# OpenPPL/ppq

Measured on AMD Instinct MI355X. Metric: calibration samples/sec (RuntimeCalibrationPass, KL 2048-bin, ResNet-50 INT8), higher is better.
Workload: dtype f32; 1 GPU; ResNet-50 topology (53 Conv + 1 Gemm, BN folded, seeded He init), RuntimeCalibrationPass kl 2048 bins, per-tensor INT8 activations, per-channel INT8 weights, 279 batches x 32 x 3x224x224 per GPU; samples=8928, batch=32, observed_tensors=72, rccl_ranks=1, async_observe=False, cache_params=False, channels_last=False, fuse_params=True, batch_observations=True, reuse_activations=False, replayed_batches=0, hip_graph=auto, graph_replays=0, miopen_find=False

## Files before the change

### include/ppq_hip.h

```cpp
#ifndef PPQ_HIP_H_
#define PPQ_HIP_H_

#include <stdint.h>

#ifdef __cplusplus
extern "C" {
#endif

typedef enum {
    PPQHIP_OK = 0,
    PPQHIP_ERR_INVALID_VALUE = -1,
    PPQHIP_ERR_UNSUPPORTED = -2,
    PPQHIP_ERR_HIP = -3
} ppqhip_status;

#define PPQHIP_ABI_VERSION 4

const char* ppqhip_last_error(void);
int ppqhip_version(void);
int ppqhip_device_arch(char* buf, int n);

int ppqhip_fq_linear_t(const float* x, const float* scale, const float* offset, float* out,
                       int64_t n, int clip_min, int clip_max, int rounding, void* stream);

int ppqhip_fq_linear_c(const float* x, const float* scale, const float* offset, float* out,
                       int64_t n, int64_t num_channel, int64_t elem_per_channel,
                       int clip_min, int clip_max, int rounding, void* stream);

int ppqhip_to_int_t(const float* x, const float* scale, const float* offset, void* out, int64_t n,
                    int clip_min, int clip_max, int rounding, int out_dtype, void* stream);
int ppqhip_to_int_c(const float* x, const float* scale, const float* offset, void* out, int64_t n,
                    int64_t num_channel, int64_t elem_per_channel, int clip_min, int clip_max,
                    int rounding, int out_dtype, void* stream);

typedef struct ppqhip_fq_job {
    const float* x;
    const float* scale;
    const float* offset;
    float* out;
    int64_t n, num_channel, elem_per_channel;
    int32_t clip_min, clip_max;
} ppqhip_fq_job;
int64_t ppqhip_fq_linear_multi_table_bytes(int num_jobs);
int ppqhip_fq_linear_multi(const ppqhip_fq_job* jobs, int num_jobs, int rounding, void* device_table,
                           int upload, void* stream);

int ppqhip_fq_linear_t_bwd(const float* x, const float* scale, const float* offset,
                           const float* grad_y, float* grad_x, float* grad_s, int64_t n,
                           int clip_min, int clip_max, int rounding, void* stream);

int ppqhip_fq_linear_c_bwd(const float* x, const float* scale, const float* offset,
                           const float* grad_y, float* grad_x, float* grad_s, int64_t n,
                           int64_t num_channel, int64_t elem_per_channel,
                           int clip_min, int clip_max, int rounding, void* stream);

int64_t ppqhip_fq_linear_t_bwd_partials(int64_t n);
int ppqhip_fq_linear_t_bwd_main(const float* x, const float* scale, const float* offset, const float* grad_y, float* grad_x,
                                float* partial, int64_t n, int clip_min, int clip_max, int rounding, void* stream);
typedef struct ppqhip_lsq_finish_job {
    const float* partial;
    float* grad_s;
    int64_t n;
    int32_t clip_min, clip_max;
} ppqhip_lsq_finish_job;
int ppqhip_lsq_finish_multi(const ppqhip_lsq_finish_job* jobs, int num_jobs, void* stream);

typedef struct ppqhip_lsq_job {
    const float* x;
    const float* scale;
    const float* offset;
    const float* grad_y;
    float* grad_x;
    float* grad_s;
    int64_t n, num_channel, elem_per_channel;
    int32_t clip_min, clip_max;
} ppqhip_lsq_job;
int ppqhip_fq_linear_c_bwd_multi(const ppqhip_lsq_job* jobs, int num_jobs, int rounding, void* stream);

int ppqhip_fq_float_t(const float* x, const float* scale, const float* offset, float* out,
                      int64_t n, int exponent, int mantissa, float clip_min, float clip_max,
                      int rounding, void* stream);

int ppqhip_fq_float_c(const float* x, const float* scale, const float* offset, float* out,
                      int64_t n, int64_t num_channel, int64_t elem_per_channel,
                      int exponent, int mantissa, float clip_min, float clip_max,
                      int rounding, void* stream);

typedef struct ppqhip_float_search_job {
    const float* x;
    int64_t rows, row_len;
    int32_t exponent, mantissa;
    float clip_min, clip_max;
} ppqhip_float_search_job;
int64_t ppqhip_float_scale_search_table_bytes(int num_jobs);
int ppqhip_float_scale_search(const ppqhip_float_search_job* jobs, int num_jobs, const float* candidates,
                              int num_candidates, int rounding, void* device_table, double* out, void* stream);

typedef struct ppqhip_fq_float_job {
    const float* x;
    const float* scale;
    const float* offset;
    float* out;
    int64_t n, num_channel, elem_per_channel;
    int32_t exponent, mantissa;
    float clip_min, clip_max;
} ppqhip_fq_float_job;
int64_t ppqhip_fq_float_multi_table_bytes(int num_jobs);
int ppqhip_fq_float_multi(const ppqhip_fq_float_job* jobs, int num_jobs, int rounding, void* device_table,
                          int upload, void* stream);

int ppqhip_fq_float_c_bwd(const float* x, const float* scale, const float* offset,
                          const float* grad_y, float* grad_x, float* grad_s, int64_t n,
                          int64_t num_channel, int64_t elem_per_channel,
                          int exponent, int mantissa, float clip_min, float clip_max,
                          int rounding, void* stream);

int64_t ppqhip_hist_workspace_bytes(int64_t n, int64_t num_bins);
int ppqhip_hist_sym_t(const float* x, int64_t n, float hist_scale, int clip_outliers,
                      int32_t* hist, int64_t num_bins, void* workspace, void* stream);

int ppqhip_hist_asym_t(const float* x, int64_t n, float min_value, float max_value,
                       int clip_outliers, int32_t* hist, int64_t num_bins, void* workspace,
                       void* stream);

int ppqhip_hist_sym_c(const float* x, int64_t n, int64_t num_channel, int64_t elem_per_channel,
                      float hist_scale, int clip_outliers, int32_t* hist, int64_t num_bins,
                      void* stream);

int ppqhip_hist_sym_c_scales(const float* x, int64_t n, int64_t num_channel, int64_t elem_per_channel,
                             const float* hist_scales, int clip_outliers, int32_t* hist,
                             int64_t num_bins, void* stream);
int ppqhip_hist_asym_c_ranges(const float* x, int64_t n, int64_t num_channel, int64_t elem_per_channel,
                              const float* mins, const float* maxs, int clip_outliers, int32_t* hist,
                              int64_t num_bins, void* stream);

int64_t ppqhip_quantile_workspace_bytes(int64_t n);
int ppqhip_quantile_t(const float* x, int64_t n, float q, float* dest, uint32_t* hint, void* workspace,
                      void* stream);

typedef struct ppqhip_quantile_job {
    const float* x;
    float* dest;
    uint32_t* hint;
    int64_t n;
} ppqhip_quantile_job;
int64_t ppqhip_quantile_multi_workspace_bytes(int num_jobs, int64_t total_elems);
int ppqhip_quantile_t_multi(const ppqhip_quantile_job* jobs, int num_jobs, float q, void* workspace,
                            void* stream);
void ppqhip_quantile_debug_layout(int64_t* out);
void ppqhip_quantile_hot_layout(int64_t* out);

int ppqhip_isotone_t(const float* x, int64_t n, float* dest, void* workspace, void* stream);

int64_t ppqhip_minmax_workspace_bytes(int64_t n);
int ppqhip_minmax_t(const float* x, int64_t n, float* minmax, void* workspace, void* stream);

int ppqhip_minmax_c(const float* x, int64_t n, int64_t num_channel, int64_t elem_per_channel,
                    float* mins, float* maxs, void* stream);

typedef struct ppqhip_minmax_c_job {
    const float* x;
    float* mins;
    float* maxs;
    int64_t n, num_channel, elem_per_channel;
    int32_t fresh, reserved;
} ppqhip_minmax_c_job;
int ppqhip_minmax_c_multi(const ppqhip_minmax_c_job* jobs, int num_jobs, void* stream);

int ppqhip_channel_sum(const float* x, int64_t n, int64_t num_channel, int64_t elem_per_channel,
                       double* sums, void* stream);

int64_t ppqhip_hist_rows(void);
int ppqhip_hist_sym_t_rows(const float* x, int64_t n, float hist_scale, int clip_outliers,
                           int32_t* rows, int64_t num_bins, void* stream);
int ppqhip_hist_asym_t_rows(const float* x, int64_t n, float min_value, float max_value,
                            int clip_outliers, int32_t* rows, int64_t num_bins, void* stream);
typedef struct ppqhip_minmax_job {
    const float* x;
    float* slots;
    int64_t n;
} ppqhip_minmax_job;
int ppqhip_minmax_t_slots_multi(const ppqhip_minmax_job* jobs, int num_jobs, void* stream);

typedef struct ppqhip_hist_job {
    const float* x;
    int32_t* rows;
    int64_t n;
    float p0, p1;
} ppqhip_hist_job;
int ppqhip_hist_t_rows_multi(const ppqhip_hist_job* jobs, int num_jobs, int asymmetric,
                             int clip_outliers, int64_t num_bins, void* stream);
int ppqhip_hist_rows_finish(const int32_t* rows, int64_t num_bins, int32_t* hist, void* stream);
int ppqhip_check_bin_rule(const float* x, int64_t n, float min_value, float hist_scale, int asymmetric, uint64_t* out, void* stream);
int64_t ppqhip_minmax_slots(void);
int ppqhip_minmax_t_slots(const float* x, int64_t n, float* slots, void* stream);
int ppqhip_minmax_slots_finish(const float* slots, float* minmax, void* stream);

float ppqhip_mse_loss_host(const int64_t* hist, int64_t num_bins, int start, int step, int end);

int64_t ppqhip_mse_search_workspace_bytes(int64_t num_hist);
int ppqhip_mse_search(const int32_t* hist, int64_t num_hist, int64_t num_bins,
                      const double* hist_scale, const double* min_value,
                      int quant_min, int quant_max, int symmetrical, int32_t* best,
                      void* workspace, void* stream);

int64_t ppqhip_kl_num_candidates(int64_t num_bins, int num_of_bits);
int ppqhip_kl_losses(const int32_t* hist, int64_t num_hist, int64_t num_bins, int num_of_bits,
                     double* losses, void* stream);

int ppqhip_tensor_clip_t(const float* value, const float* reference, const float* limit,
                         float* out, int64_t n, void* stream);
int ppqhip_tensor_clip_c(const float* value, const float* reference, const float* limit,
                         float* out, int64_t n, int64_t num_channel, int64_t elem_per_channel,
                         void* stream);
int ppqhip_rounding_loss(const float* x, const float* scale, const float* offset, float* out,
                         int64_t n, int64_t num_channel, int64_t elem_per_channel,
                         int clip_min, int clip_max, int rounding, void* stream);
int ppqhip_rounding_loss_bwd(const float* x, const float* dy, const float* scale,
                             const float* offset, float* dx, int64_t n, int64_t num_channel,
                             int64_t elem_per_channel, int clip_min, int clip_max, int rounding,
                             void* stream);

int ppqhip_bias_act(float* y, const float* bias, int64_t n, int64_t num_channel, int64_t elem_per_channel,
                    int relu, void* stream);
int ppqhip_bias_add_act(float* a, const float* bias_a, float* b, const float* bias_b, float* out,
                        int64_t n, int64_t num_channel, int64_t elem_per_channel, int relu, void* stream);

typedef struct ppqhip_adaround_job {
    const float* w;
    const float* v;
    const float* scale;
    const float* offset;
    float* out;
    const float* dy;
    int64_t n, num_channel, elem_per_channel;
    int32_t qmin, qmax;
} ppqhip_adaround_job;
int ppqhip_adaround_fwd_multi(const ppqhip_adaround_job* jobs, int num_jobs, void* stream);
int ppqhip_adaround_bwd_multi(const ppqhip_adaround_job* jobs, int num_jobs, const float* reg, void* stream);

typedef struct ppqhip_roundtune_job {
    const float* w;
    const float* r;
    const float* scale;
    const float* offset;
    float* out;
    int64_t n, num_channel, elem_per_channel;
    int32_t qmin, qmax;
} ppqhip_roundtune_job;
int ppqhip_roundtune_fwd_multi(const ppqhip_roundtune_job* jobs, int num_jobs, void* stream);

typedef struct ppqhip_fetch_rows_job {
    const float* x;
    const int32_t* index;
    float* out;
    int64_t rows, row_len, count;
} ppqhip_fetch_rows_job;
int ppqhip_fetch_rows_multi(const ppqhip_fetch_rows_job* jobs, int num_jobs, void* stream);
typedef struct ppqhip_measure_rows_job {
    const float* p;
    const float* r;
    const int32_t* index;
    double* sums;
    int64_t rows, row_len, count;
} ppqhip_measure_rows_job;
int ppqhip_measure_rows_multi(const ppqhip_measure_rows_job* jobs, int num_jobs, void* stream);
enum { PPQHIP_MEASURE_SNR = 0, PPQHIP_MEASURE_MSE = 1, PPQHIP_MEASURE_COSINE = 2 };
enum { PPQHIP_REDUCE_MEAN = 0, PPQHIP_REDUCE_MAX = 1 };
typedef struct ppqhip_measure_finish_job {
    const double* sums;
    double* acc;
    float* row_out;
    int64_t rows, count;
    int32_t method, reduce;
} ppqhip_measure_finish_job;
int ppqhip_measure_finish_multi(const ppqhip_measure_finish_job* jobs, int num_jobs, void* stream);

typedef struct ppqhip_equalize_segment {
    const float* base;
    int64_t extent;
    int64_t div, a, b;
    int64_t outer, stride, run;
    float multiplier;
    int32_t downstream;
} ppqhip_equalize_segment;
typedef struct ppqhip_equalize_scale_job {
    const ppqhip_equalize_segment* segments;
    float* scale;
    int32_t num_segments, num_channel;
    float value_threshold;
    int32_t reserved;
} ppqhip_equalize_scale_job;
int ppqhip_equalize_scale_multi(const ppqhip_equalize_scale_job* jobs, int num_jobs, void* stream);
typedef struct ppqhip_equalize_apply_job {
    float* x;
    const float* scale;
    int64_t n, run, inner, group_out;
    int64_t num_scale;
    int32_t divide, reserved;
} ppqhip_equalize_apply_job;
int ppqhip_equalize_apply_multi(const ppqhip_equalize_apply_job* jobs, int num_jobs, void* stream);

typedef struct ppqhip_split_plan_job {
    const ppqhip_equalize_segment* segments;
    int32_t* src_of;
    int32_t* count;
    int32_t num_segments, num_channel;
    float value_threshold;
    int32_t reserved;
} ppqhip_split_plan_job;
int ppqhip_split_plan_multi(const ppqhip_split_plan_job* jobs, int num_jobs, void* stream);
typedef struct ppqhip_split_apply_job {
    const float* x;
    float* out;
    const int32_t* src_of;
    int64_t n, run;
    int32_t num_channel, count;
} ppqhip_split_apply_job;
int ppqhip_split_apply_multi(const ppqhip_split_apply_job* jobs, int num_jobs, void* stream);

typedef struct ppqhip_ssd_scales_job {
    ppqhip_equalize_segment first, last;
    const float* act_range;
    float* scales;
    float* ranges;
    int32_t num_channel;
    float channel_ratio;
} ppqhip_ssd_scales_job;
int ppqhip_ssd_scales_multi(const ppqhip_ssd_scales_job* jobs, int num_jobs, void* stream);
typedef struct ppqhip_ssd_apply_job {
    const float* x;
    float* out;
    const float* scales;
    int64_t n, run, inner, group_out;
    int64_t num_channel;
    int32_t divide, reserved;
} ppqhip_ssd_apply_job;
int ppqhip_ssd_apply_multi(const ppqhip_ssd_apply_job* jobs, int num_jobs, void* stream);
typedef struct ppqhip_fq_measure_rows_job {
    const float* y;
    const float* r;
    const float* scale;
    const float* offset;
    double* sums;
    int64_t rows, count;
    int64_t num_channel, elem_per_channel;
    int32_t clip_min, clip_max, rounding, reserved;
} ppqhip_fq_measure_rows_job;
int ppqhip_fq_measure_rows_multi(const ppqhip_fq_measure_rows_job* jobs, int num_jobs, void* stream);

typedef struct ppqhip_stat_job {
    const float* p;
    const float* r;
    float* rec;
    int64_t n;
    int32_t bins, reserved;
} ppqhip_stat_job;
int ppqhip_stat_moments_multi(const ppqhip_stat_job* jobs, int num_jobs, void* stream);
int ppqhip_stat_shape_multi(const ppqhip_stat_job* jobs, int num_jobs, void* stream);

#define PPQHIP_PROF_MAX_KERNELS 40
typedef struct {
    char name[48];
    int64_t launches;
    double total_ms;
    double total_bytes;
} ppqhip_prof_entry;
int ppqhip_prof_enable(int on);
int ppqhip_prof_collect(ppqhip_prof_entry* entries, int max_entries);
double ppqhip_prof_event_overhead_us(void* stream, int pairs);

#ifdef __cplusplus
}
#endif
#endif
```

### ppq_amd/_lib.py

```python
import ctypes
import os

_HERE = os.path.dirname(os.path.abspath(__file__))
LIB_PATH = os.path.join(_HERE, 'libppq_hip.so')

c_f32p = ctypes.c_void_p
c_i32p = ctypes.c_void_p
c_f64p = ctypes.c_void_p
c_i64 = ctypes.c_int64
c_int = ctypes.c_int
c_flt = ctypes.c_float
c_vp = ctypes.c_void_p

ABI_VERSION = 4


class ProfEntry(ctypes.Structure):
    _fields_ = [('name', ctypes.c_char * 48), ('launches', ctypes.c_int64),
                ('total_ms', ctypes.c_double), ('total_bytes', ctypes.c_double)]


PROTOTYPES = {
    'ppqhip_last_error': (ctypes.c_char_p, []),
    'ppqhip_version': (c_int, []),
    'ppqhip_device_arch': (c_int, [ctypes.c_char_p, c_int]),
    'ppqhip_fq_linear_t': (c_int, [c_f32p, c_f32p, c_f32p, c_f32p, c_i64, c_int, c_int, c_int, c_vp]),
    'ppqhip_fq_linear_c': (c_int, [c_f32p, c_f32p, c_f32p, c_f32p, c_i64, c_i64, c_i64, c_int, c_int, c_int, c_vp]),
    'ppqhip_to_int_t': (c_int, [c_f32p, c_f32p, c_f32p, c_vp, c_i64, c_int, c_int, c_int, c_int, c_vp]),
    'ppqhip_to_int_c': (c_int, [c_f32p, c_f32p, c_f32p, c_vp, c_i64, c_i64, c_i64, c_int, c_int, c_int, c_int, c_vp]),
    'ppqhip_fq_linear_t_bwd': (c_int, [c_f32p, c_f32p, c_f32p, c_f32p, c_f32p, c_f32p, c_i64, c_int, c_int, c_int,
                                       c_vp]),
    'ppqhip_fq_linear_c_bwd': (c_int, [c_f32p, c_f32p, c_f32p, c_f32p, c_f32p, c_f32p, c_i64, c_i64, c_i64, c_int,
                                       c_int, c_int, c_vp]),
    'ppqhip_fq_linear_c_bwd_multi': (c_int, [c_vp, c_int, c_int, c_vp]),
    'ppqhip_fq_linear_t_bwd_partials': (c_i64, [c_i64]),
    'ppqhip_fq_linear_t_bwd_main': (c_int, [c_f32p, c_f32p, c_f32p, c_f32p, c_f32p, c_f32p, c_i64, c_int, c_int, c_int, c_vp]),
    'ppqhip_lsq_finish_multi': (c_int, [c_vp, c_int, c_vp]),
    'ppqhip_bias_act': (c_int, [c_f32p, c_f32p, c_i64, c_i64, c_i64, c_int, c_vp]),
    'ppqhip_bias_add_act': (c_int, [c_f32p, c_f32p, c_f32p, c_f32p, c_f32p, c_i64, c_i64, c_i64, c_int, c_vp]),
    'ppqhip_fq_float_t': (c_int, [c_f32p, c_f32p, c_f32p, c_f32p, c_i64, c_int, c_int, c_flt, c_flt, c_int, c_vp]),
    'ppqhip_fq_float_c': (c_int, [c_f32p, c_f32p, c_f32p, c_f32p, c_i64, c_i64, c_i64, c_int, c_int, c_flt, c_flt,
                                  c_int, c_vp]),
    'ppqhip_fq_float_c_bwd': (c_int, [c_f32p, c_f32p, c_f32p, c_f32p, c_f32p, c_f32p, c_i64, c_i64, c_i64, c_int,
                                      c_int, c_flt, c_flt, c_int, c_vp]),
    'ppqhip_hist_workspace_bytes': (c_i64, [c_i64, c_i64]),
    'ppqhip_hist_sym_t': (c_int, [c_f32p, c_i64, c_flt, c_int, c_i32p, c_i64, c_vp, c_vp]),
    'ppqhip_hist_asym_t': (c_int, [c_f32p, c_i64, c_flt, c_flt, c_int, c_i32p, c_i64, c_vp, c_vp]),
    'ppqhip_hist_sym_c': (c_int, [c_f32p, c_i64, c_i64, c_i64, c_flt, c_int, c_i32p, c_i64, c_vp]),
    'ppqhip_hist_sym_c_scales': (c_int, [c_f32p, c_i64, c_i64, c_i64, c_f32p, c_int, c_i32p, c_i64, c_vp]),
    'ppqhip_hist_asym_c_ranges': (c_int, [c_f32p, c_i64, c_i64, c_i64, c_f32p, c_f32p, c_int, c_i32p, c_i64, c_vp]),
    'ppqhip_quantile_workspace_bytes': (c_i64, [c_i64]),
    'ppqhip_quantile_t': (c_int, [c_f32p, c_i64, c_flt, c_f32p, c_vp, c_vp, c_vp]),
    'ppqhip_isotone_t': (c_int, [c_f32p, c_i64, c_f32p, c_vp, c_vp]),
    'ppqhip_minmax_workspace_bytes': (c_i64, [c_i64]),
    'ppqhip_minmax_t': (c_int, [c_f32p, c_i64, c_f32p, c_vp, c_vp]),
    'ppqhip_minmax_c': (c_int, [c_f32p, c_i64, c_i64, c_i64, c_f32p, c_f32p, c_vp]),
    'ppqhip_minmax_c_multi': (c_int, [c_vp, c_int, c_vp]),
    'ppqhip_fq_linear_multi_table_bytes': (c_i64, [c_int]),
    'ppqhip_fq_linear_multi': (c_int, [c_vp, c_int, c_int, c_vp, c_int, c_vp]),
    'ppqhip_float_scale_search_table_bytes': (c_i64, [c_int]),
    'ppqhip_float_scale_search': (c_int, [c_vp, c_int, c_vp, c_int, c_int, c_vp, c_vp, c_vp]),
    'ppqhip_fq_float_multi_table_bytes': (c_i64, [c_int]),
    'ppqhip_fq_float_multi': (c_int, [c_vp, c_int, c_int, c_vp, c_int, c_vp]),
    'ppqhip_quantile_multi_workspace_bytes': (c_i64, [c_int, c_i64]),
    'ppqhip_quantile_t_multi': (c_int, [c_vp, c_int, c_flt, c_vp, c_vp]),
    'ppqhip_quantile_debug_layout': (None, [c_vp]),
    'ppqhip_quantile_hot_layout': (None, [c_vp]),
    'ppqhip_minmax_t_slots_multi': (c_int, [c_vp, c_int, c_vp]),
    'ppqhip_hist_t_rows_multi': (c_int, [c_vp, c_int, c_int, c_int, c_i64, c_vp]),
    'ppqhip_channel_sum': (c_int, [c_f32p, c_i64, c_i64, c_i64, c_f64p, c_vp]),
    'ppqhip_hist_rows': (c_i64, []),
    'ppqhip_hist_sym_t_rows': (c_int, [c_f32p, c_i64, c_flt, c_int, c_i32p, c_i64, c_vp]),
    'ppqhip_hist_asym_t_rows': (c_int, [c_f32p, c_i64, c_flt, c_flt, c_int, c_i32p, c_i64, c_vp]),
    'ppqhip_hist_rows_finish': (c_int, [c_i32p, c_i64, c_i32p, c_vp]),
    'ppqhip_check_bin_rule': (c_int, [c_f32p, c_i64, c_flt, c_flt, c_int, c_vp, c_vp]),
    'ppqhip_minmax_slots': (c_i64, []),
    'ppqhip_minmax_t_slots': (c_int, [c_f32p, c_i64, c_f32p, c_vp]),
    'ppqhip_minmax_slots_finish': (c_int, [c_f32p, c_f32p, c_vp]),
    'ppqhip_mse_loss_host': (c_flt, [ctypes.POINTER(ctypes.c_int64), c_i64, c_int, c_int, c_int]),
    'ppqhip_mse_search_workspace_bytes': (c_i64, [c_i64]),
    'ppqhip_mse_search': (c_int, [c_i32p, c_i64, c_i64, c_f64p, c_f64p, c_int, c_int, c_int, c_i32p, c_vp, c_vp]),
    'ppqhip_kl_num_candidates': (c_i64, [c_i64, c_int]),
    'ppqhip_kl_losses': (c_int, [c_i32p, c_i64, c_i64, c_int, c_f64p, c_vp]),
    'ppqhip_tensor_clip_t': (c_int, [c_f32p, c_f32p, c_f32p, c_f32p, c_i64, c_vp]),
    'ppqhip_tensor_clip_c': (c_int, [c_f32p, c_f32p, c_f32p, c_f32p, c_i64, c_i64, c_i64, c_vp]),
    'ppqhip_rounding_loss': (c_int, [c_f32p, c_f32p, c_f32p, c_f32p, c_i64, c_i64, c_i64, c_int, c_int, c_int, c_vp]),
    'ppqhip_rounding_loss_bwd': (c_int, [c_f32p, c_f32p, c_f32p, c_f32p, c_f32p, c_i64, c_i64, c_i64, c_int, c_int,
                                         c_int, c_vp]),
    'ppqhip_adaround_fwd_multi': (c_int, [c_vp, c_int, c_vp]),
    'ppqhip_adaround_bwd_multi': (c_int, [c_vp, c_int, c_f32p, c_vp]),
    'ppqhip_roundtune_fwd_multi': (c_int, [c_vp, c_int, c_vp]),
    'ppqhip_equalize_scale_multi': (c_int, [c_vp, c_int, c_vp]),
    'ppqhip_equalize_apply_multi': (c_int, [c_vp, c_int, c_vp]),
    'ppqhip_split_plan_multi': (c_int, [c_vp, c_int, c_vp]),
    'ppqhip_split_apply_multi': (c_int, [c_vp, c_int, c_vp]),
    'ppqhip_ssd_scales_multi': (c_int, [c_vp, c_int, c_vp]),
    'ppqhip_ssd_apply_multi': (c_int, [c_vp, c_int, c_vp]),
    'ppqhip_fq_measure_rows_multi': (c_int, [c_vp, c_int, c_vp]),
    'ppqhip_fetch_rows_multi': (c_int, [c_vp, c_int, c_vp]),
    'ppqhip_measure_rows_multi': (c_int, [c_vp, c_int, c_vp]),
    'ppqhip_measure_finish_multi': (c_int, [c_vp, c_int, c_vp]),
    'ppqhip_stat_moments_multi': (c_int, [c_vp, c_int, c_vp]),
    'ppqhip_stat_shape_multi': (c_int, [c_vp, c_int, c_vp]),
    'ppqhip_prof_enable': (c_int, [c_int]),
    'ppqhip_prof_collect': (c_int, [ctypes.POINTER(ProfEntry), c_int]),
    'ppqhip_prof_event_overhead_us': (ctypes.c_double, [c_vp, c_int]),
}

if not os.path.exists(LIB_PATH):
    raise ImportError(
        f'{LIB_PATH} is missing: the HIP kernel library has not been built.  Run '
        '`python -c "import __graft_entry__ as g; g.build()"` or `make -C ppq_amd/csrc` (needs hipcc, '
        'targets gfx950).  ppq_amd has no CPU / PyTorch fallback by design.')

import torch

_torch_hip = os.path.join(os.path.dirname(torch.__file__), 'lib', 'libamdhip64.so')
if os.path.exists(_torch_hip):
    ctypes.CDLL(_torch_hip, mode=ctypes.RTLD_GLOBAL)

try:
    lib = ctypes.CDLL(LIB_PATH)
except OSError as e:
    raise ImportError(f'cannot load {LIB_PATH}: {e}') from e

for _name, (_res, _args) in PROTOTYPES.items():
    _fn = getattr(lib, _name)
    _fn.restype = _res
    _fn.argtypes = _args


if lib.ppqhip_version() != ABI_VERSION:
    raise ImportError(f'{LIB_PATH} has ABI version {lib.ppqhip_version()}, this package needs {ABI_VERSION}: rebuild it '
                      '(`make -C ppq_amd/csrc` or `python -c "import __graft_entry__ as g; g.build()"`)')


def last_error() -> str:
    msg = lib.ppqhip_last_error()
    return msg.decode('utf-8', 'replace') if msg else ''
```

### ppq_amd/calibration.py

```python
import time
from math import ceil
from typing import Callable, Dict, Iterable, List

from .core import QuantizationStates, state_value
from .distributed import merge_observers
from .observer import OperationObserver, TorchHistObserver, render_observers


class QuantizationOptimizationPass:
    def __init__(self, name: str = 'Default Quanzation Optim') -> None:
        self.name = name

    def apply(self, graph, **kwargs) -> None:
        self.optimize(graph, **kwargs)

    def optimize(self, graph, **kwargs) -> None:
        raise NotImplementedError('Implement this function first.')

    def __str__(self) -> str:
        return 'QuantizationOptimizationPass[' + self.name + ']'


class RuntimeCalibrationPass(QuantizationOptimizationPass):
    AUTO_GRAPH_ISSUE_FRACTION = 0.7
    AUTO_GRAPH_MIN_STEPS = 12

    def __init__(self, method: str = None, override: bool = False, calib_steps: int = 32,
                 process_group=None, check_steps: bool = True, async_observe: bool = False,
                 use_hip_graph: bool = False, batch_observations: bool = True,
                 reuse_activations: bool = False, reuse_budget_bytes: int = 64 << 30,
                 queue_bytes: int = None) -> None:
        super().__init__(name='PPQ Runtime Calibration Pass')
        self._method = method
        self._observers: Dict[str, OperationObserver] = {}
        self._collate_fn = None
        self._calib_steps = calib_steps
        self._override = override
        self._process_group = process_group
        self._check_steps = check_steps
        self._async_observe = async_observe
        self._use_hip_graph = use_hip_graph
        self._batch_observations = batch_observations
        self._queue = None
        self._reuse_activations = reuse_activations
        self._queue_bytes = queue_bytes
        self._reuse_budget = reuse_budget_bytes
        self._replay: list = []
        self._replay_bytes = 0
        self.replay_peak_bytes = 0
        self.replayed_batches = 0
        self._recording = False
        self.graph_replays = 0
        self.graph_decisions = []
        self.merge_stats = []
        self._side_stream = None

    def _batches(self, dataloader: Iterable) -> list:
        out = []
        for calib_epoch in range(ceil(self._calib_steps / len(dataloader))):
            for data in dataloader:
                if self._collate_fn is not None:
                    data = self._collate_fn(data)
                out.append(data)
                if len(out) >= self._calib_steps: return out
        return out

    def _graph_replayable(self, batches: list, hooks: Dict[str, object]) -> bool:
        import torch
        from .observer import ConstantObserver, TorchHistObserver, TorchMinMaxObserver, TorchMSEObserver
        if not self._use_hip_graph or len(batches) < 4: return False
        if not all(isinstance(b, torch.Tensor) and b.is_cuda and b.shape == batches[0].shape
                   and b.dtype == batches[0].dtype for b in batches): return False
        safe = (TorchMinMaxObserver, TorchHistObserver, TorchMSEObserver, ConstantObserver)
        return all(type(ob) in safe for hook in hooks.values() for ob in hook._observer_table.values())

    @ staticmethod
    def _forward_fn(executor):
        return executor.forward

    def _forward(self, executor, data, hooks, output_names):
        import torch
        recording = self._queue is not None and self._recording
        if recording: self._queue.recorder = []
        with torch.no_grad():
            self._forward_fn(executor)(inputs=data, hooks=hooks, output_names=output_names)
        if self._queue is not None: self._queue.flush()
        if recording:
            rec, self._queue.recorder = self._queue.recorder, None
            size = sum(v.numel() * 4 for _, v in rec)
            if self._replay_bytes + size <= self._reuse_budget:
                self._replay.append(rec); self._replay_bytes += size
                self.replay_peak_bytes = max(self.replay_peak_bytes, self._replay_bytes)
            else: self._recording = False

    def _replay_phase2(self, batches: list) -> int:
        n = min(len(self._replay), len(batches))
        for i in range(n):
            for ob, value in self._replay[i]: ob.observe(value)
            self._queue.flush()
            self._replay[i] = None
        self._replay, self._replay_bytes = [], 0
        self.replayed_batches += n
        return n

    def calibrate(self, desc: str, dataloader: Iterable, executor, hooks: Dict[str, object],
                  output_names: List[str] = None):
        import torch
        batches = self._batches(dataloader)
        if self._replay and not self._recording:
            batches = batches[self._replay_phase2(batches):]
            if not batches: return
        if not self._graph_replayable(batches, hooks):
            for data in batches:
                self._forward(executor, data, hooks, output_names)
            return
        self._forward(executor, batches[0], hooks, output_names)
        first = 1
        if self._use_hip_graph == 'auto':
            torch.cuda.synchronize()
            t0 = time.perf_counter()
            self._forward(executor, batches[1], hooks, output_names)
            t1 = time.perf_counter()
            torch.cuda.synchronize()
            t2 = time.perf_counter()
            first = 2
            launch_bound = (t1 - t0) > self.AUTO_GRAPH_ISSUE_FRACTION * (t2 - t0)
            self.graph_decisions.append({'phase': desc, 'issue_ms': (t1 - t0) * 1e3, 'total_ms': (t2 - t0) * 1e3,
                                         'graph': bool(launch_bound and len(batches) - first >= self.AUTO_GRAPH_MIN_STEPS)})
            if not self.graph_decisions[-1]['graph']:
                for data in batches[first:]:
                    self._forward(executor, data, hooks, output_names)
                return
        self._recording = False
        static_in = torch.empty_like(batches[0])
        torch.cuda.synchronize()
        graph = torch.cuda.CUDAGraph()
        with torch.cuda.graph(graph):
            self._forward(executor, static_in, hooks, output_names)
            if self._side_stream is not None:
                torch.cuda.current_stream().wait_stream(self._side_stream)
        for data in batches[first:]:
            static_in.copy_(data, non_blocking=True)
            graph.replay()
            self.graph_replays += 1

    def _all_tensor_observers(self):
        return [ob for op_ob in self._observers.values() for ob in op_ob.observers()]

    def _render(self):
        observers = self._all_tensor_observers()
        if self._queue is not None: self._queue.flush()
        if self._side_stream is not None:
            import torch
            torch.cuda.current_stream().wait_stream(self._side_stream)
        if merge_observers(observers, group=self._process_group):
            from . import distributed
            self.merge_stats.append(dict(distributed.last_merge_stats))
        render_observers(observers)

    def optimize(self, graph, dataloader: Iterable, executor, calib_steps: int = 32,
                 collate_fn: Callable = None, **kwargs) -> None:
        if collate_fn is not None: self._collate_fn = collate_fn
        if calib_steps is not None: self._calib_steps = calib_steps
        if self._check_steps:
            assert self._calib_steps >= 8, (
                'Insufficient Calibration Detected, to get a better quantization performance, '
                'more calibration steps is required, we strongly recommend you to prepare more calibration data '
                'and more calibration steps is preferred here. (at least 8)')
            assert self._calib_steps <= 512, (
                'Calibration steps is too large, ppq can quantize your network within 8-512 '
                'calibration steps. More calibration steps will greatly delay ppq\'s calibration procedure. '
                'Reset your calib_steps parameter please.')

        if self._override:
            for operation in graph.operations.values():
                if not hasattr(operation, 'config'): continue
                for config, var in operation.config_with_variable:
                    if (not var.is_parameter and state_value(config.state) == QuantizationStates.ACTIVATED.value
                            and config.dominated_by == config):
                        config.state = type(config.state).INITIAL

        self._observers = {}
        hooks = {}
        import torch
        if self._async_observe and torch.cuda.is_available():
            self._side_stream = torch.cuda.Stream()
        for op_name, operation in graph.operations.items():
            if not hasattr(operation, 'config'): continue
            for config, var in operation.config_with_variable:
                if not var.is_parameter and self._method is not None:
                    config.observer_algorithm = self._method
            observer = OperationObserver(operation=executor._graph.operations[op_name], monitor_parameter=False)
            observer.hook.stream = self._side_stream
            self._observers[op_name] = observer
            hooks[op_name] = observer.hook

        self._queue = None
        if self._batch_observations and self._side_stream is None:
            from .observer import ObservationQueue
            self._queue = ObservationQueue() if self._queue_bytes is None else ObservationQueue(self._queue_bytes)
        for ob in self._all_tensor_observers(): ob.queue = self._queue

        self._replay, self._replay_bytes = [], 0
        self._recording = bool(self._reuse_activations and self._queue is not None)
        self.calibrate(desc='Calibration Progress(Phase 1)', dataloader=dataloader, executor=executor,
                       hooks=hooks, output_names=None)
        self._recording = False
        self._render()
        if self._replay:
            for observer in self._observers.values():
                for cfg, ob in observer.hook._observer_table.items():
                    if (not getattr(ob._watch_on, 'is_parameter', False)
                            and QuantizationStates.is_activated(cfg.state)):
                        self._replay, self._replay_bytes = [], 0
                        break
                if not self._replay: break

        pop_list = []
        for op_name, observer in self._observers.items():
            if all([not isinstance(var_observer, TorchHistObserver)
                    for var_observer in observer.observers()]):
                pop_list.append(op_name)
        for op_name in pop_list:
            self._observers.pop(op_name)
            hooks.pop(op_name)

        if len(hooks) > 0:
            self.calibrate(desc='Calibration Progress(Phase 2)', dataloader=dataloader, executor=executor,
                           hooks=hooks, output_names=None)
            self._render()


class PPLDSPTIReCalibrationPass(RuntimeCalibrationPass):
    def __init__(self, method: str = None, override: bool = False) -> None:
        super().__init__(method, override)
        self.name = 'PPQ ReCalibration For Computing Op Pass'

    def optimize(self, graph, dataloader: Iterable, executor, calib_steps: int, collate_fn: Callable = None, **kwargs) -> None:
        from .blocks import COMPUTING_OP, downstream_operations
        from .core import QuantizationPolicy, QuantizationProperty as P, TensorQuantizationConfig
        from .observer import CalibrationHook, TensorObserverFactroy, TorchMinMaxObserver
        self._collate_fn, self._calib_steps = collate_fn, calib_steps
        assert calib_steps >= 8, ('Insufficient Calibration Detected, to better quantize your network, more calibration steps is '
                                  'demonded, we strongly recommend you to prepare more calibration data and more calibration '
                                  'steps is preferred here. (at least 8)')
        assert calib_steps <= 512, ('Calibration steps is too large, ppq is capable for quantizing your network within 32-128 '
                                    'calibration steps. More calibraiton steps will greatly delay ppq\'s calibration procedure. '
                                    'Reset your calib_steps parameter please.')

        def probe(like, per_channel: bool, consumer):
            bits = P.SYMMETRICAL.value + P.LINEAR.value + (P.PER_CHANNEL.value if per_channel else P.PER_TENSOR.value)
            return TensorQuantizationConfig(policy=QuantizationPolicy(bits), rounding=like.rounding, num_of_bits=like.num_of_bits,
                                            quant_min=like.quant_min, quant_max=like.quant_max, scale=None, offset=None,
                                            observer_algorithm='Minmax', state=QuantizationStates.INITIAL,
                                            channel_axis=1 if per_channel else None, detail={'consumer': consumer})
        hooks = {}
        for operation in graph.topological_sort():
            if not hasattr(operation, 'config') or operation.type not in COMPUTING_OP: continue
            output_cfg = operation.config.output_quantization_config[0]
            master_cfg, master_operation, master_var = output_cfg, operation, operation.outputs[0]
            table = {}
            if operation.inputs[0].name in graph.inputs:
                input_cfg = operation.config.input_quantization_config[0]
                table[input_cfg] = TensorObserverFactroy.build_observer(operation.inputs[0], probe(input_cfg, False, input_cfg))
            followers = downstream_operations(operation)
            if len(followers) == 1 and followers[0].type in {'Relu', 'Clip'} and hasattr(followers[0], 'config'):
                if table:
                    hooks[operation.name] = CalibrationHook(operation, table)
                    table = {}
                master_operation = followers[0]
                master_cfg = master_operation.config.output_quantization_config[0]
                master_var = master_operation.outputs[0]
            table[master_cfg] = TensorObserverFactroy.build_observer(master_var, probe(master_cfg, True, output_cfg))
            assert master_operation.name not in hooks, 'register an operation in calibration hooks twice'
            hooks[master_operation.name] = CalibrationHook(master_operation, table)

        self._queue = None
        self.calibrate(desc='ReCalibration For Computing Ops', dataloader=dataloader, executor=executor, hooks=hooks)

        for hook in hooks.values():
            for observer in hook._observer_table.values():
                cfg = observer._quant_cfg.detail['consumer']
                assert isinstance(observer, TorchMinMaxObserver)
                r = observer._range_on_host()
                if observer._quant_cfg.policy.has_property(P.PER_CHANNEL):
                    cfg.detail.update({'range_min': r[0].copy(), 'range_max': r[1].copy()})
                else:
                    cfg.detail.update({'range_min': (float(r[0]),), 'range_max': (float(r[1]),)})


class IsotoneCalibrationPass(RuntimeCalibrationPass):
    def __init__(self, variables: List[str] = None, axis: int = -1, verbose: bool = True, calib_steps: int = 32) -> None:
        super().__init__(calib_steps=calib_steps)
        self.name = 'Isotone Calibration Pass'
        self.variables = variables
        self.axis = axis
        self.verbose = verbose

    @ staticmethod
    def _mark(cfg, axis: int) -> None:
        from .core import OBSERVER_ISOTONE_OBSERVER_AXIS
        cfg.state = type(cfg.state).INITIAL
        cfg.observer_algorithm = 'Isotone'
        cfg.detail[OBSERVER_ISOTONE_OBSERVER_AXIS] = axis

    def optimize(self, graph, **kwargs) -> None:
        if self.variables is None:
            for op in graph.operations.values():
                if op.type != 'Softmax' or not hasattr(op, 'config'): continue
                cfg = op.config.output_quantization_config[0]
                if cfg.dominated_by != cfg: continue
                axis = op.attributes.get('axis', -1)
                self._mark(cfg, axis)
                if self.verbose: print(f'Calibration Method of Op {op.name} has been changed to Isotone[axis={axis}].')
        else:
            if not isinstance(self.variables, list):
                raise TypeError('Isotone Calibration Pass needs a list of variable name as its input.')
            for name in self.variables:
                if not isinstance(name, str):
                    raise TypeError('Isotone Calibration Pass needs a list of variable name as its input.')
                if name not in graph.variables: raise ValueError(f'Variable {name} not in current graph.')
                var = graph.variables[name]
                op = var.source_op
                if op is None or not hasattr(op, 'config'): continue
                self._mark(op.config.output_quantization_config[op.outputs.index(var)], self.axis)
                if self.verbose: print(f'Calibration Method of Variable {var.name} has been changed to Isotone[axis={self.axis}].')
        super().optimize(graph, **kwargs)
```

### ppq_amd/csrc/epilogue.hip

```cpp
#include "common.hpp"

namespace ppqhip {
namespace {

constexpr int kEpTileU = 2;
constexpr int kEpSmallU = 1;
constexpr long long kEpSmallElems = 1ll << 20;

struct EpArgs {
    float* a;
    const float* bias_a;
    float* b;
    const float* bias_b;
    float* out;
    uint32_t nvec;
    uint32_t tail;
    int ntail;
    FastDiv epc;
    FastDiv nc;
};

__device__ __forceinline__ uint32_t channel_of(uint32_t i, const FastDiv& epc, const FastDiv& nc) {
    const uint32_t row = fdiv(i, epc);
    return row - fdiv(row, nc) * nc.d;
}

__device__ __forceinline__ float act(float v, bool relu) {
    return (relu && !__builtin_isnan(v)) ? __builtin_fmaxf(v, 0.f) : v;
}

__device__ __forceinline__ float4 add4(const float4& x, const float4& y) {
    return make_float4(x.x + y.x, x.y + y.y, x.z + y.z, x.w + y.w);
}

template <bool RELU>
__device__ __forceinline__ float4 act4(const float4& v) {
    return make_float4(act(v.x, RELU), act(v.y, RELU), act(v.z, RELU), act(v.w, RELU));
}

template <bool PLANE>
__device__ __forceinline__ float4 bias4(const float* __restrict__ bias, uint32_t v, const FastDiv& epc, const FastDiv& nc) {
    if (PLANE) {
        const float t = bias[channel_of(v, epc, nc)];
        return make_float4(t, t, t, t);
    }
    const uint32_t i = v * 4u;
    return make_float4(bias[channel_of(i, epc, nc)], bias[channel_of(i + 1, epc, nc)], bias[channel_of(i + 2, epc, nc)],
                       bias[channel_of(i + 3, epc, nc)]);
}

template <bool RESID, bool BIAS_B, bool RELU>
__device__ __forceinline__ void epilogue_elem(const EpArgs& p, uint32_t i, const FastDiv& epc) {
    const uint32_t c = channel_of(i, epc, p.nc);
    const float x = p.a[i] + p.bias_a[c];
    if (!RESID) { p.a[i] = act(x, RELU); return; }
    p.a[i] = x;
    float y = p.b[i];
    if (BIAS_B) { y = y + p.bias_b[c]; p.b[i] = y; }
    p.out[i] = act(x + y, RELU);
}

template <int U, bool RESID, bool BIAS_B, bool RELU, bool PLANE>
__global__ __launch_bounds__(kBlock) void epilogue_kernel(EpArgs p) {
    const uint32_t base = blockIdx.x * (kBlock * U) + threadIdx.x;
    float4* a4 = reinterpret_cast<float4*>(p.a);
    float4* b4 = reinterpret_cast<float4*>(p.b);
    float4* o4 = reinterpret_cast<float4*>(p.out);
    float4 a[U], ba[U], b[U], bb[U];
#pragma unroll
    for (int k = 0; k < U; k++) {
        const uint32_t vv = min(base + k * kBlock, p.nvec - 1);
        a[k] = a4[vv];
        ba[k] = bias4<PLANE>(p.bias_a, vv, p.epc, p.nc);
        if (RESID) b[k] = b4[vv];
        if (BIAS_B) bb[k] = bias4<PLANE>(p.bias_b, vv, p.epc, p.nc);
    }
#pragma unroll
    for (int k = 0; k < U; k++) {
        const uint32_t vv = base + k * kBlock;
        if (vv >= p.nvec) continue;
        const float4 x = add4(a[k], ba[k]);
        if (!RESID) { a4[vv] = act4<RELU>(x); continue; }
        a4[vv] = x;
        float4 y = b[k];
        if (BIAS_B) { y = add4(y, bb[k]); b4[vv] = y; }
        o4[vv] = act4<RELU>(add4(x, y));
    }
    if (!PLANE && blockIdx.x == 0 && (int)threadIdx.x < p.ntail)
        epilogue_elem<RESID, BIAS_B, RELU>(p, p.tail + threadIdx.x, p.epc);
}

template <bool RESID, bool BIAS_B, bool RELU>
__global__ __launch_bounds__(kBlock) void epilogue_scalar_kernel(EpArgs p) {
    const uint32_t stride = gridDim.x * kBlock;
    for (uint32_t i = blockIdx.x * kBlock + threadIdx.x; i < (uint32_t)p.ntail; i += stride)
        epilogue_elem<RESID, BIAS_B, RELU>(p, i, p.epc);
}

template <bool RESID, bool BIAS_B, bool RELU>
void launch_epilogue(EpArgs p, int64_t n, int64_t C, int64_t epc, bool aligned, hipStream_t st) {
    p.nc = make_fastdiv((uint32_t)C);
    if (!aligned || n < 4) {
        p.nvec = 0; p.tail = 0; p.ntail = (int)n;
        p.epc = make_fastdiv((uint32_t)epc);
        hipLaunchKernelGGL((epilogue_scalar_kernel<RESID, BIAS_B, RELU>), dim3(stream_grid(n, kBlock)), dim3(kBlock), 0, st, p);
        return;
    }
    p.nvec = (uint32_t)(n >> 2);
    p.tail = p.nvec * 4u;
    p.ntail = (int)(n & 3);
    const bool plane = (epc % 4 == 0);
    p.epc = make_fastdiv((uint32_t)(plane ? epc / 4 : epc));
#define PPQ_LAUNCH_EP(U, PLANE)                                                                                          \
    hipLaunchKernelGGL((epilogue_kernel<U, RESID, BIAS_B, RELU, PLANE>), dim3((p.nvec + kBlock * U - 1) / (kBlock * U)),   \
                       dim3(kBlock), 0, st, p)
    if (n <= kEpSmallElems) {
        if (plane) PPQ_LAUNCH_EP(kEpSmallU, true); else PPQ_LAUNCH_EP(kEpSmallU, false);
    } else {
        if (plane) PPQ_LAUNCH_EP(kEpTileU, true); else PPQ_LAUNCH_EP(kEpTileU, false);
    }
#undef PPQ_LAUNCH_EP
}

int validate(int64_t n, int64_t C, int64_t epc, const char* what) {
    if (n <= 0 || n > 0x7fffffffLL) {
        set_error("%s: n=%lld is empty or has more than 2^31 - 1 elements", what, (long long)n);
        return PPQHIP_ERR_INVALID_VALUE;
    }
    if (C <= 0 || epc <= 0 || C > 0x7fffffffLL || epc > 0x7fffffffLL || n % (C * epc) != 0) {
        set_error("%s: n=%lld is not [outer, %lld channels, %lld elem/channel]", what, (long long)n, (long long)C,
                  (long long)epc);
        return PPQHIP_ERR_INVALID_VALUE;
    }
    return PPQHIP_OK;
}

}
}

using namespace ppqhip;

extern "C" {

int ppqhip_bias_act(float* y, const float* bias, int64_t n, int64_t num_channel, int64_t elem_per_channel, int relu,
                    void* stream) {
    if (int st = validate(n, num_channel, elem_per_channel, "bias_act")) return st;
    if (!y || !bias) { set_error("bias_act: null pointer"); return PPQHIP_ERR_INVALID_VALUE; }
    hipStream_t s = (hipStream_t)stream;
    EpArgs p{};
    p.a = y; p.bias_a = bias;
    const bool aligned = aligned16(y);
    if (relu) launch_epilogue<false, false, true>(p, n, num_channel, elem_per_channel, aligned, s);
    else launch_epilogue<false, false, false>(p, n, num_channel, elem_per_channel, aligned, s);
    return finish_launch("bias_act");
}

int ppqhip_bias_add_act(float* a, const float* bias_a, float* b, const float* bias_b, float* out, int64_t n,
                        int64_t num_channel, int64_t elem_per_channel, int relu, void* stream) {
    if (int st = validate(n, num_channel, elem_per_channel, "bias_add_act")) return st;
    if (!a || !bias_a || !b || !out) { set_error("bias_add_act: null pointer"); return PPQHIP_ERR_INVALID_VALUE; }
    hipStream_t s = (hipStream_t)stream;
    EpArgs p{};
    p.a = a; p.bias_a = bias_a; p.b = b; p.bias_b = bias_b; p.out = out;
    const bool aligned = aligned16(a) && aligned16(b) && aligned16(out);
    if (bias_b) {
        if (relu) launch_epilogue<true, true, true>(p, n, num_channel, elem_per_channel, aligned, s);
        else launch_epilogue<true, true, false>(p, n, num_channel, elem_per_channel, aligned, s);
    } else {
        if (relu) launch_epilogue<true, false, true>(p, n, num_channel, elem_per_channel, aligned, s);
        else launch_epilogue<true, false, false>(p, n, num_channel, elem_per_channel, aligned, s);
    }
    return finish_launch("bias_add_act");
}

}
```

### ppq_amd/csrc/hist.hip

```cpp
#include "common.hpp"

namespace ppqhip {

constexpr int kMaxLdsBins = 16384;
constexpr int kLdsBudgetInts = 2048;
constexpr int kHistBlock = 512;
constexpr int kHistWgPerCu = 2;
constexpr int kHistU = 2;
constexpr int kHistMinTiles = 2;
constexpr int kHistAtomicMaxWg = 128;
constexpr long long kHistNtElems = 48ll << 20;
constexpr int kHistRows = kNumCU * kHistWgPerCu;
constexpr uint32_t kTileVec = (uint32_t)kHistBlock * kHistU;
constexpr uint32_t kTileElems = kTileVec * 4;
static_assert(kHistBlock % 64 == 0 && kHistBlock >= 64 && kHistBlock <= 1024, "histogram workgroup: whole waves");

typedef float v2f __attribute__((ext_vector_type(2)));

struct BinRule {
    float a;
    float hs;
    float rcp;
    int bins;
    int clip;
    int asym;
};
static BinRule make_rule(float a, float hs, int bins, int clip, int asym) {
    BinRule r; r.a = a; r.hs = hs; r.rcp = 1.0f / hs; r.bins = bins; r.clip = clip; r.asym = asym;
    return r;
}

__device__ __forceinline__ bool quotient_is_safe(float t) {
    return __builtin_fabsf(t - __builtin_rintf(t)) >= __builtin_fabsf(t) * 0x1p-22f;
}

__device__ __forceinline__ int f2i_abs(float t) {
    int r;
    asm("v_cvt_i32_f32_e64 %0, |%1|" : "=v"(r) : "v"(t));
    return r;
}
__device__ __forceinline__ int f2i_floor(float t) {
    int r;
    asm("v_cvt_flr_i32_f32 %0, %1" : "=v"(r) : "v"(t));
    return r;
}

template <bool ASYM, bool CLIP, bool HOT>
struct Binner : WaveBinCounter<ASYM, CLIP, HOT> {
    using Base = WaveBinCounter<ASYM, CLIP, HOT>;
    using Base::h; using Base::last; using Base::hot_bin; using Base::hot_cnt;
    float a0, hs, rcp;

    __device__ __forceinline__ void set_rule(float a, float scale) { a0 = a; hs = scale; rcp = 1.0f / scale; }

    __device__ __forceinline__ void bins4(const float4& v, int (&b)[4]) const {
        v2f x01 = {v.x, v.y}, x23 = {v.z, v.w};
        if (ASYM) { x01 = x01 - a0; x23 = x23 - a0; }
        const v2f t01 = x01 * rcp, t23 = x23 * rcp;
        const v2f r01 = {__builtin_rintf(t01.x), __builtin_rintf(t01.y)};
        const v2f r23 = {__builtin_rintf(t23.x), __builtin_rintf(t23.y)};
        const v2f d01 = t01 - r01, d23 = t23 - r23;
        const v2f e01 = t01 * 0x1p-22f, e23 = t23 * 0x1p-22f;
        const bool u0 = !(__builtin_fabsf(d01.x) >= __builtin_fabsf(e01.x));
        const bool u1 = !(__builtin_fabsf(d01.y) >= __builtin_fabsf(e01.y));
        const bool u2 = !(__builtin_fabsf(d23.x) >= __builtin_fabsf(e23.x));
        const bool u3 = !(__builtin_fabsf(d23.y) >= __builtin_fabsf(e23.y));
        b[0] = ASYM ? f2i_floor(t01.x) : f2i_abs(t01.x);
        b[1] = ASYM ? f2i_floor(t01.y) : f2i_abs(t01.y);
        b[2] = ASYM ? f2i_floor(t23.x) : f2i_abs(t23.x);
        b[3] = ASYM ? f2i_floor(t23.y) : f2i_abs(t23.y);
        if (u0 | u1 | u2 | u3) {
            if (u0) b[0] = exact_bin(ASYM ? x01.x : __builtin_fabsf(v.x));
            if (u1) b[1] = exact_bin(ASYM ? x01.y : __builtin_fabsf(v.y));
            if (u2) b[2] = exact_bin(ASYM ? x23.x : __builtin_fabsf(v.z));
            if (u3) b[3] = exact_bin(ASYM ? x23.y : __builtin_fabsf(v.w));
        }
    }
    __device__ __forceinline__ int exact_bin(float a) const { return f2i_sat(__builtin_floorf(a / hs)); }

    __device__ __forceinline__ int bin1(float v) const {
        const float a = ASYM ? (v - a0) : __builtin_fabsf(v);
        const float t = a * rcp;
        if (quotient_is_safe(t)) return ASYM ? f2i_floor(t) : f2i_abs(t);
        return exact_bin(a);
    }

};

constexpr int kReduceBins = 32, kReduceSlices = 32, kReduceBlock = kReduceBins * kReduceSlices;
__global__ __launch_bounds__(kReduceBlock) void hist_reduce_kernel(const int* __restrict__ partial, int count, int bins,
                                                                   int* __restrict__ hist) {
    __shared__ int lds[kReduceSlices][kReduceBins];
    const int lane_bin = threadIdx.x % kReduceBins, slice = threadIdx.x / kReduceBins;
    const int b = blockIdx.x * kReduceBins + lane_bin;
    int total = 0;
    if (b < bins) {
        int i = slice;
        for (; i + 15 * kReduceSlices < count; i += 16 * kReduceSlices) {
            int v[16];
#pragma unroll
            for (int k = 0; k < 16; k++) v[k] = partial[(size_t)(i + k * kReduceSlices) * bins + b];
#pragma unroll
            for (int k = 0; k < 16; k++) total += v[k];
        }
        for (; i < count; i += kReduceSlices) total += partial[(size_t)i * bins + b];
    }
    lds[slice][lane_bin] = total;
    __syncthreads();
    if (slice == 0 && b < bins) {
        int t = 0;
#pragma unroll
        for (int k = 0; k < kReduceSlices; k++) t += lds[k][lane_bin];
        if (t) hist[b] += t;
    }
}

constexpr int kMultiMax = 96;
enum FlushMode : int {
    FLUSH_ROWS_ADD = 0,
    FLUSH_ROWS_STORE = 1,
    FLUSH_ATOMIC = 2
};
struct HistJob {
    const float* x;
    int* rows;
    uint32_t n;
    float a, hs;
    uint32_t first_tile;
};
struct HistJobs {
    HistJob job[kMultiMax];
    uint32_t count;
    uint32_t total_tiles;
    int bins, copies, mode;
};
__host__ __device__ inline uint32_t job_tiles(uint32_t n, bool vec_ok) {
    if (!vec_ok) return (n + kTileElems - 1) / kTileElems;
    const uint32_t full = (n >> 2) / kTileVec;
    return full + (n > full * kTileElems ? 1u : 0u);
}

__device__ __forceinline__ void lds_hist_flush(int* lds, int bins, int copies, int* __restrict__ dst, int mode) {
    asm volatile("s_waitcnt lgkmcnt(0)" ::: "memory");
    __syncthreads();
    for (int b = threadIdx.x; b < bins; b += kHistBlock) {
        int s = 0;
        for (int c = 0; c < copies; c++) { s += lds[c * bins + b]; lds[c * bins + b] = 0; }
        if (mode == FLUSH_ROWS_STORE) dst[b] = s;
        else if (s) {
            if (mode == FLUSH_ROWS_ADD) dst[b] += s;
            else atomicAdd(&dst[b], s);
        }
    }
    __syncthreads();
}

template <bool ASYM, bool CLIP, bool HOT, bool NT>
__global__ __launch_bounds__(kHistBlock, (kHistBlock * kHistWgPerCu + 255) / 256)
void hist_persistent_kernel(const HistJobs jobs) {
    extern __shared__ int lds[];
    const uint32_t G = gridDim.x, g = blockIdx.x;
    uint32_t t, t_end;
    even_split(jobs.total_tiles, G, g, t, t_end);
    const int bins = jobs.bins, copies = jobs.copies;
    bool zeroed = false;
    auto zero_lds = [&]() {
        if (zeroed) return;
        for (int i = threadIdx.x; i < copies * bins; i += kHistBlock) lds[i] = 0;
        asm volatile("s_waitcnt lgkmcnt(0)\n\ts_barrier" ::: "memory");
        zeroed = true;
    };
    if (t >= t_end) {
        if (jobs.mode == FLUSH_ROWS_STORE) for (int b = threadIdx.x; b < bins; b += kHistBlock) jobs.job[0].rows[(size_t)g * bins + b] = 0;
        return;
    }
    uint32_t lo = 0, hi = jobs.count;
    while (hi - lo > 1) {
        const uint32_t mid = (lo + hi) >> 1;
        if (jobs.job[mid].first_tile <= t) lo = mid; else hi = mid;
    }
    Binner<ASYM, CLIP, HOT> acc;
    acc.init(lds + ((threadIdx.x >> 6) % copies) * bins, bins);

    for (uint32_t j = lo; t < t_end; j++) {
        const HistJob& job = jobs.job[j];
        const uint32_t j_end = (j + 1 < jobs.count) ? jobs.job[j + 1].first_tile : jobs.total_tiles;
        uint32_t k = t - job.first_tile;
        const uint32_t k1 = min(t_end, j_end) - job.first_tile;
        t = min(t_end, j_end);
        acc.set_rule(job.a, job.hs);
        const float* __restrict__ x = job.x;
        const uint32_t n = job.n;
        const bool vec_ok = (reinterpret_cast<uintptr_t>(x) & 15u) == 0;
        const uint32_t full = vec_ok ? (n >> 2) / kTileVec : 0u;
        const uint32_t kf = min(k1, full);
        if (k < kf) {
            const float4* xv = reinterpret_cast<const float4*>(x) + threadIdx.x;
            float4 bufa[kHistU], bufb[kHistU];
            auto fetch = [&](float4 (&buf)[kHistU], uint32_t tile) {
                const float4* p = xv + (size_t)tile * kTileVec;
#pragma unroll
                for (int u = 0; u < kHistU; u++) buf[u] = load4<NT>(p + u * kHistBlock);
            };
            auto consume = [&](const float4 (&buf)[kHistU], uint32_t tile) {
#pragma unroll
                for (int u = 0; u < kHistU; u++) {
                    int b[4];
                    acc.bins4(buf[u], b);
                    if (u == 0) acc.elect(b[0], true);
                    if (CLIP && HOT) acc.commit4_exec(b);
                    else {
                        acc.template commit<true>(b[0], true); acc.template commit<true>(b[1], true);
                        acc.template commit<true>(b[2], true); acc.template commit<true>(b[3], true);
                    }
                }
            };
            fetch(bufa, k);
            zero_lds();
            for (;;) {
                fetch(bufb, min(k + 1, kf - 1));
                consume(bufa, k);
                if (++k >= kf) break;
                fetch(bufa, min(k + 1, kf - 1));
                consume(bufb, k);
                if (++k >= kf) break;
            }
        }
        zero_lds();
        for (; k < k1; k++) {
            const uint32_t e0 = k * kTileElems + threadIdx.x;
#pragma unroll 4
            for (int r = 0; r < 4 * kHistU; r++) {
                const uint32_t i = e0 + r * kHistBlock;
                const bool in = i < n;
                const float a = in ? x[i] : 0.f;
                const int b = acc.bin1(a);
                if ((r & 3) == 0) acc.elect(b, in);
                acc.template commit<false>(b, in);
            }
        }
        acc.flush_hot();
        acc.hot_bin = -1;
        int* dst = jobs.mode == FLUSH_ATOMIC ? job.rows : job.rows + (size_t)g * bins;
        lds_hist_flush(lds, bins, copies, dst, jobs.mode);
    }
}

template <bool ASYM, bool CLIP, int kSmallK, bool PING = false, bool NT = false>
__global__ __launch_bounds__(kHistBlock) void hist_small_kernel(const float* __restrict__ x, uint32_t n, float a, float hs, int bins,
                                                                 int copies, int* __restrict__ dst, uint32_t row_mod) {
    extern __shared__ int lds[];
    const uint32_t G = gridDim.x, g = blockIdx.x;
    const uint32_t nvec = n >> 2;
    const uint32_t full_rows = nvec / kHistBlock;
    uint32_t r0, r1;
    even_split(full_rows, G, g, r0, r1);
    const float4* xv = reinterpret_cast<const float4*>(x) + threadIdx.x;
    Binner<ASYM, CLIP, true> acc;
    acc.init(lds + ((threadIdx.x >> 6) % copies) * bins, bins);
    acc.set_rule(a, hs);
    bool zeroed = false;
    auto zero_lds = [&]() {
        if (zeroed) return;
        for (int i = threadIdx.x; i < copies * bins; i += kHistBlock) lds[i] = 0;
        asm volatile("s_waitcnt lgkmcnt(0)\n\ts_barrier" ::: "memory");
        zeroed = true;
    };
    auto fetch = [&](float4 (&buf)[kSmallK], uint32_t r) {
#pragma unroll
        for (int k = 0; k < kSmallK; k++) buf[k] = load4<NT>(xv + (size_t)min(r + (uint32_t)k, r1 - 1) * kHistBlock);
    };
    auto consume = [&](const float4 (&buf)[kSmallK], uint32_t cnt) {
#pragma unroll
        for (int k = 0; k < kSmallK; k++) {
            if ((uint32_t)k < cnt) {
                int b[4];
                acc.bins4(buf[k], b);
                if ((k & 1) == 0) acc.elect(b[0], true);
                if (CLIP) acc.commit4_exec(b);
                else {
                    acc.template commit<true>(b[0], true); acc.template commit<true>(b[1], true);
                    acc.template commit<true>(b[2], true); acc.template commit<true>(b[3], true);
                }
            }
        }
    };
    if (PING) {
        if (r0 < r1) {
            float4 bufa[kSmallK], bufb[kSmallK];
            uint32_t r = r0;
            fetch(bufa, r);
            zero_lds();
            for (;;) {
                fetch(bufb, r + kSmallK);
                consume(bufa, min((uint32_t)kSmallK, r1 - r));
                r += kSmallK;
                if (r >= r1) break;
                fetch(bufa, r + kSmallK);
                consume(bufb, min((uint32_t)kSmallK, r1 - r));
                r += kSmallK;
                if (r >= r1) break;
            }
        }
    } else {
        for (uint32_t r = r0; r < r1; r += kSmallK) {
            float4 buf[kSmallK];
            fetch(buf, r);
            zero_lds();
            consume(buf, min((uint32_t)kSmallK, r1 - r));
        }
    }
    zero_lds();
    if (g == G - 1) {
        const uint32_t e0 = full_rows * kHistBlock * 4;
        const uint32_t trips = (n - e0 + kHistBlock - 1) / kHistBlock;
        for (uint32_t t = 0; t < trips; t++) {
            const uint32_t i = e0 + t * kHistBlock + threadIdx.x;
            const bool in = i < n;
            const float v = in ? x[i] : 0.f;
            const int b = acc.bin1(v);
            if ((t & 3) == 0) acc.elect(b, in);
            acc.template commit<false>(b, in);
        }
    }
    acc.flush_hot();
    int* row = dst + (size_t)(row_mod ? g % row_mod : 0u) * bins;
    asm volatile("s_waitcnt lgkmcnt(0)" ::: "memory");
    __syncthreads();
    for (int b = threadIdx.x; b < bins; b += kHistBlock) {
        int sum = 0;
        for (int c = 0; c < copies; c++) sum += lds[c * bins + b];
        if (sum) atomicAdd(&row[b], sum);
    }
}

template <bool ASYM>
__global__ __launch_bounds__(kBlock) void check_bin_rule_kernel(const float4* __restrict__ x, uint32_t nvec, float a, float hs,
                                                                unsigned long long* __restrict__ out) {
    Binner<ASYM, true, false> acc;
    acc.init(nullptr, 1);
    acc.set_rule(a, hs);
    const uint32_t stride = gridDim.x * kBlock;
    for (uint32_t i = blockIdx.x * kBlock + threadIdx.x; i < nvec; i += stride) {
        const float4 v = x[i];
        int b[4];
        acc.bins4(v, b);
        const float e[4] = {v.x, v.y, v.z, v.w};
#pragma unroll
        for (int k = 0; k < 4; k++) {
            const int want = acc.exact_bin(ASYM ? (e[k] - a) : __builtin_fabsf(e[k]));
            if (b[k] != want) { atomicAdd(&out[0], 1ull); out[2] = __float_as_uint(e[k]); }
            if (acc.bin1(e[k]) != want) { atomicAdd(&out[1], 1ull); out[2] = __float_as_uint(e[k]); }
        }
    }
}

__device__ __forceinline__ bool bin_of(float v, const BinRule& r, int* b_out) {
    const float a = r.asym ? (v - r.a) : __builtin_fabsf(v);
    int b = f2i_sat(__builtin_floorf(a / r.hs));
    const int last = r.bins - 1;
    bool out = b > last;
    if (r.asym) out = out || (b < 0);
    *b_out = b < 0 ? 0 : (b > last ? last : b);
    return !(out && r.clip);
}

__global__ __launch_bounds__(kBlock) void hist_t_global_kernel(const float* __restrict__ x, uint32_t n, BinRule rule,
                                                               int* __restrict__ hist) {
    const uint32_t stride = gridDim.x * kBlock;
    for (uint32_t i = blockIdx.x * kBlock + threadIdx.x; i < n; i += stride) {
        int b;
        if (bin_of(x[i], rule, &b)) atomicAdd(&hist[b], 1);
    }
}

constexpr int kHistCWgPerCu = 1;
template <bool ASYM, bool CLIP, bool NT>
__global__ __launch_bounds__(kHistBlock, (kHistBlock * kHistWgPerCu + 255) / 256)
void hist_c_channel_kernel(const float* __restrict__ x, FastDiv vec_per_row, uint32_t C, uint32_t outer, uint32_t splits,
                           BinRule rule, int copies, int* __restrict__ hist, const float* __restrict__ scales,
                           const float* __restrict__ mins, const float* __restrict__ maxs, int flush_mode) {
    extern __shared__ int lds[];
    const int bins = rule.bins;
    bool zeroed = false;
    auto zero_lds = [&]() {
        if (zeroed) return;
        for (int i = threadIdx.x; i < copies * bins; i += kHistBlock) lds[i] = 0;
        asm volatile("s_waitcnt lgkmcnt(0)\n\ts_barrier" ::: "memory");
        zeroed = true;
    };
// ... 509 lines not shown
```

### ppq_amd/ffi.py

```python
import threading
import weakref
from typing import List

import numpy as np
import torch

from . import _lib
from ._lib import lib

_KERNEL_FAILURE = 'Kernel Failure, '


_raw_stream = torch._C._cuda_getCurrentRawStream
_get_device = torch._C._cuda_getDevice


def _stream() -> int:
    return _raw_stream(_get_device())


def _check(t: torch.Tensor, dtype: torch.dtype, name: str) -> None:
    if not isinstance(t, torch.Tensor):
        raise TypeError(f'{name}: expected a torch.Tensor, got {type(t)}')
    if t.dtype != dtype:
        raise RuntimeError(_KERNEL_FAILURE + 'Invalid dtype of Input tensor: ' + name)
    if t.numel() == 0:
        raise RuntimeError(_KERNEL_FAILURE + 'Tensor is empty: ' + name)
    if not t.is_cuda:
        raise RuntimeError(_KERNEL_FAILURE + f'{name} is not on the GPU (ppq_amd has no CPU path)')


_F32 = torch.float32


def _f32(t, name):
    try:
        if t.dtype is _F32 and t.is_cuda and t.numel() > 0: return
    except AttributeError:
        pass
    _check(t, torch.float32, name + '(Expect to be FP32)')


def _dense(t: torch.Tensor, channel_axis=None) -> torch.Tensor:
    if t.is_contiguous(): return t
    if channel_axis is None or channel_axis % t.dim() == 0:
        if t.dim() == 4 and t.is_contiguous(memory_format=torch.channels_last): return t
        if t.dim() == 5 and t.is_contiguous(memory_format=torch.channels_last_3d): return t
    return t.contiguous()


def _raise(status: int) -> None:
    if status != 0:
        raise RuntimeError(_KERNEL_FAILURE + _lib.last_error())


def _geometry(shape, channel_axis: int):
    ndim = len(shape)
    if channel_axis < 0: channel_axis += ndim
    if not 0 <= channel_axis < ndim:
        raise RuntimeError(_KERNEL_FAILURE + f'channel_axis {channel_axis} out of range for a {ndim}-d tensor')
    epc = 1
    for d in shape[channel_axis + 1:]:
        epc *= int(d)
    return int(shape[channel_axis]), epc


class _DeviceOf:
    __slots__ = ('idx', 'prev')

    def __init__(self, t: torch.Tensor):
        self.idx = t.device.index
        self.prev = None

    def __enter__(self):
        if self.idx is not None and self.idx != _get_device():
            self.prev = _get_device()
            torch.cuda.set_device(self.idx)

    def __exit__(self, *a):
        if self.prev is not None:
            torch.cuda.set_device(self.prev)


_workspaces = {}
_MAX_WORKSPACES = 16


def _workspace(device: torch.device, nbytes: int) -> torch.Tensor:
    key = (device.index, _stream())
    ws = _workspaces.pop(key, None)
    if ws is None or ws.numel() < nbytes:
        ws = torch.empty(max(nbytes, 1 << 16), dtype=torch.uint8, device=device)
    _workspaces[key] = ws
    while len(_workspaces) > _MAX_WORKSPACES:
        _workspaces.pop(next(iter(_workspaces)))
    return ws


_MINMAX_JOB = np.dtype([('x', '<u8'), ('slots', '<u8'), ('n', '<i8')])
_FQ_JOB = np.dtype([('x', '<u8'), ('scale', '<u8'), ('offset', '<u8'), ('out', '<u8'), ('n', '<i8'),
                    ('num_channel', '<i8'), ('elem_per_channel', '<i8'), ('clip_min', '<i4'), ('clip_max', '<i4')])
_FQ_FLOAT_JOB = np.dtype([('x', '<u8'), ('scale', '<u8'), ('offset', '<u8'), ('out', '<u8'), ('n', '<i8'),
                          ('num_channel', '<i8'), ('elem_per_channel', '<i8'), ('exponent', '<i4'), ('mantissa', '<i4'),
                          ('clip_min', '<f4'), ('clip_max', '<f4')])
_FLOAT_SEARCH_JOB = np.dtype([('x', '<u8'), ('rows', '<i8'), ('row_len', '<i8'), ('exponent', '<i4'), ('mantissa', '<i4'),
                              ('clip_min', '<f4'), ('clip_max', '<f4')])
_LSQ_JOB = np.dtype([('x', '<u8'), ('scale', '<u8'), ('offset', '<u8'), ('grad_y', '<u8'), ('grad_x', '<u8'), ('grad_s', '<u8'),
                     ('n', '<i8'), ('num_channel', '<i8'), ('elem_per_channel', '<i8'), ('clip_min', '<i4'), ('clip_max', '<i4')])
_LSQ_FINISH_JOB = np.dtype([('partial', '<u8'), ('grad_s', '<u8'), ('n', '<i8'), ('clip_min', '<i4'), ('clip_max', '<i4')])
_MINMAX_C_JOB = np.dtype([('x', '<u8'), ('mins', '<u8'), ('maxs', '<u8'), ('n', '<i8'), ('num_channel', '<i8'),
                          ('elem_per_channel', '<i8'), ('fresh', '<i4'), ('reserved', '<i4')])
_QUANTILE_JOB = np.dtype([('x', '<u8'), ('dest', '<u8'), ('hint', '<u8'), ('n', '<i8')])

_owner_hints = weakref.WeakKeyDictionary()
_hint_owner = threading.local()


def quantile_hint(device: torch.device) -> torch.Tensor:
    return torch.zeros(8, dtype=torch.int32, device=device)


class quantile_hint_owner:
    __slots__ = ('owner', 'prev')

    def __init__(self, owner):
        self.owner, self.prev = owner, None

    def __enter__(self):
        self.prev = getattr(_hint_owner, 'current', None)
        _hint_owner.current = self.owner
        return self

    def __exit__(self, *a):
        _hint_owner.current = self.prev


def _owner_quantile_hint(device: torch.device, numel: int, q: float):
    owner = getattr(_hint_owner, 'current', None)
    if owner is None: return None
    try: per = _owner_hints.setdefault(owner, {})
    except TypeError: return None
    key = (device.index, int(numel), float(q))
    h = per.get(key)
    if h is None: h = per[key] = quantile_hint(device)
    return h


_HIST_JOB = np.dtype([('x', '<u8'), ('rows', '<u8'), ('n', '<i8'), ('p0', '<f4'), ('p1', '<f4')])


def _epilogue_geometry(ts, bias_list):
    t0 = ts[0]
    if not isinstance(t0, torch.Tensor) or t0.dtype is not _F32 or not t0.is_cuda or t0.dim() != 4 or t0.numel() == 0:
        return None
    shape, strides, dev = t0.shape, t0.stride(), t0.device
    for t in ts[1:]:
        if not isinstance(t, torch.Tensor) or t.dtype is not _F32 or t.device != dev or t.shape != shape or t.stride() != strides:
            return None
    C = int(shape[1])
    for bias in bias_list:
        if (not isinstance(bias, torch.Tensor) or bias.dtype is not _F32 or bias.device != dev or bias.dim() != 1
                or bias.numel() != C or not bias.is_contiguous()):
            return None
    if t0.is_contiguous(): return C, int(shape[2]) * int(shape[3])
    if t0.is_contiguous(memory_format=torch.channels_last): return C, 1
    return None


def bias_act_(y: torch.Tensor, bias: torch.Tensor, relu: bool) -> bool:
    geo = _epilogue_geometry([y], [bias])
    if geo is None: return False
    with _DeviceOf(y):
        _raise(lib.ppqhip_bias_act(y.data_ptr(), bias.data_ptr(), y.numel(), geo[0], geo[1], 1 if relu else 0, _stream()))
    return True


def bias_add_act(a: torch.Tensor, bias_a: torch.Tensor, b: torch.Tensor, bias_b, relu: bool):
    geo = _epilogue_geometry([a, b], [bias_a] if bias_b is None else [bias_a, bias_b])
    if geo is None or a.data_ptr() == b.data_ptr(): return None
    out = torch.empty_like(a)
    with _DeviceOf(a):
        _raise(lib.ppqhip_bias_add_act(a.data_ptr(), bias_a.data_ptr(), b.data_ptr(), 0 if bias_b is None else bias_b.data_ptr(),
                                       out.data_ptr(), a.numel(), geo[0], geo[1], 1 if relu else 0, _stream()))
    return out


_ADAROUND_JOB = np.dtype([('w', '<u8'), ('v', '<u8'), ('scale', '<u8'), ('offset', '<u8'), ('out', '<u8'), ('dy', '<u8'),
                          ('n', '<i8'), ('num_channel', '<i8'), ('elem_per_channel', '<i8'), ('qmin', '<i4'), ('qmax', '<i4')])


def _adaround_table(items, outs, dys=None):
    n = len(items)
    if len(outs) != n or (dys is not None and len(dys) != n):
        raise RuntimeError(_KERNEL_FAILURE + 'AdaRound: argument lists differ in length')
    jobs = np.zeros(n, dtype=_ADAROUND_JOB)
    dev = items[0][0].device
    for k, (w, v, s, o, axis, qmin, qmax) in enumerate(items):
        ts = [('Value', w), ('Rounding', v), ('Scale', s), ('Offset', o), ('Out', outs[k])] + ([('Dy', dys[k])] if dys is not None else [])
        for name, t in ts:
            _f32(t, name)
            if t.device != dev: raise RuntimeError(_KERNEL_FAILURE + f'AdaRound: item {k}: {name} is on another device')
            if not t.is_contiguous(): raise RuntimeError(_KERNEL_FAILURE + f'AdaRound: item {k}: {name} is not contiguous')
        for name, t in ts[1:2] + ts[4:]:
            if t.shape != w.shape: raise RuntimeError(_KERNEL_FAILURE + f'AdaRound: item {k}: {name} is not shaped like the weight')
        C, epc = _geometry(w.shape, axis) if axis is not None else (1, w.numel())
        if s.numel() != C or o.numel() != C:
            raise RuntimeError(_KERNEL_FAILURE + f'AdaRound: item {k}: scale / offset need {C} elements')
        jobs[k] = (w.data_ptr(), v.data_ptr(), s.data_ptr(), o.data_ptr(), outs[k].data_ptr(),
                   dys[k].data_ptr() if dys is not None else 0, w.numel(), C, epc, int(qmin), int(qmax))
    return jobs


def adaround_forward_multi(items, outs=None) -> List[torch.Tensor]:
    if not items: return []
    if outs is None: outs = [torch.empty_like(it[0]) for it in items]
    jobs = _adaround_table(items, outs)
    with _DeviceOf(items[0][0]):
        _raise(lib.ppqhip_adaround_fwd_multi(jobs.ctypes.data, len(items), _stream()))
    return outs


def adaround_backward_multi(items, dys, reg: torch.Tensor, dvs=None) -> List[torch.Tensor]:
    if not items: return []
    _f32(reg, 'Reg')
    if reg.numel() != 3 or not reg.is_contiguous() or reg.device != items[0][0].device:
        raise RuntimeError(_KERNEL_FAILURE + 'AdaRound: reg must be a contiguous float32[3] on the weights\' device')
    if dvs is None: dvs = [torch.empty_like(it[0]) for it in items]
    jobs = _adaround_table(items, dvs, dys)
    with _DeviceOf(items[0][0]):
        _raise(lib.ppqhip_adaround_bwd_multi(jobs.ctypes.data, len(items), reg.data_ptr(), _stream()))
    return dvs


_ROUNDTUNE_JOB = np.dtype([('w', '<u8'), ('r', '<u8'), ('scale', '<u8'), ('offset', '<u8'), ('out', '<u8'),
                           ('n', '<i8'), ('num_channel', '<i8'), ('elem_per_channel', '<i8'), ('qmin', '<i4'), ('qmax', '<i4')])


def _roundtune_table(items, outs):
    n = len(items)
    if len(outs) != n: raise RuntimeError(_KERNEL_FAILURE + 'RoundTuning: argument lists differ in length')
    jobs = np.zeros(n, dtype=_ROUNDTUNE_JOB)
    dev = items[0][0].device
    for k, (w, r, s, o, axis, qmin, qmax) in enumerate(items):
        ts = [('Value', w), ('Rounding', r), ('Scale', s), ('Offset', o), ('Out', outs[k])]
        for name, t in ts:
            _f32(t, name)
            if t.device != dev: raise RuntimeError(_KERNEL_FAILURE + f'RoundTuning: item {k}: {name} is on another device')
            if not t.is_contiguous(): raise RuntimeError(_KERNEL_FAILURE + f'RoundTuning: item {k}: {name} is not contiguous')
        for name, t in ts[1:2] + ts[4:]:
            if t.shape != w.shape: raise RuntimeError(_KERNEL_FAILURE + f'RoundTuning: item {k}: {name} is not shaped like the weight')
        C, epc = _geometry(w.shape, axis) if axis is not None else (1, w.numel())
        if s.numel() != C or o.numel() != C:
            raise RuntimeError(_KERNEL_FAILURE + f'RoundTuning: item {k}: scale / offset need {C} elements')
        jobs[k] = (w.data_ptr(), r.data_ptr(), s.data_ptr(), o.data_ptr(), outs[k].data_ptr(), w.numel(), C, epc, int(qmin), int(qmax))
    return jobs


def roundtune_forward_multi(items, outs=None) -> List[torch.Tensor]:
    if not items: return []
    if outs is None: outs = [torch.empty_like(it[0]) for it in items]
    jobs = _roundtune_table(items, outs)
    with _DeviceOf(items[0][0]):
        _raise(lib.ppqhip_roundtune_fwd_multi(jobs.ctypes.data, len(items), _stream()))
    return outs


_EQ_SEGMENT = np.dtype([('base', '<u8'), ('extent', '<i8'), ('div', '<i8'), ('a', '<i8'), ('b', '<i8'), ('outer', '<i8'),
                        ('stride', '<i8'), ('run', '<i8'), ('multiplier', '<f4'), ('downstream', '<i4')])
_EQ_SCALE_JOB = np.dtype([('segments', '<u8'), ('scale', '<u8'), ('num_segments', '<i4'), ('num_channel', '<i4'),
                          ('value_threshold', '<f4'), ('reserved', '<i4')])
_EQ_APPLY_JOB = np.dtype([('x', '<u8'), ('scale', '<u8'), ('n', '<i8'), ('run', '<i8'), ('inner', '<i8'), ('group_out', '<i8'),
                          ('num_scale', '<i8'), ('divide', '<i4'), ('reserved', '<i4')])


def _eq_tensor(t, what: str, k: int, dev):
    _f32(t, what)
    if t.device != dev: raise RuntimeError(_KERNEL_FAILURE + f'Equalization: item {k}: {what} is on another device')
    if not t.is_contiguous(): raise RuntimeError(_KERNEL_FAILURE + f'Equalization: item {k}: {what} is not contiguous')


class EqualizeTable:
    __slots__ = ('jobs', 'segments', 'keep', 'entry')

    def __init__(self, jobs, segments, keep, entry):
        self.jobs, self.segments, self.keep, self.entry = jobs, segments, keep, entry

    def __len__(self) -> int: return len(self.jobs)

    def run(self) -> None:
        if len(self.jobs) == 0: return
        with _DeviceOf(self.keep[0]):
            _raise(self.entry(self.jobs.ctypes.data, len(self.jobs), _stream()))


def equalize_scale_table(items) -> EqualizeTable:
    jobs = np.zeros(len(items), dtype=_EQ_SCALE_JOB)
    segs = np.zeros(sum(len(it[2]) for it in items), dtype=_EQ_SEGMENT)
    keep, at = [], 0
    dev = items[0][0].device if items else None
    for k, (scale, threshold, segments) in enumerate(items):
        _eq_tensor(scale, 'Scale', k, dev)
        keep.append(scale)
        jobs[k] = (segs.ctypes.data + at * _EQ_SEGMENT.itemsize, scale.data_ptr(), len(segments), scale.numel(), float(threshold), 0)
        for t, div, a, b, outer, stride, run, mult, down in segments:
            _eq_tensor(t, 'Value', k, dev)
            keep.append(t)
            segs[at] = (t.data_ptr(), t.numel(), int(div), int(a), int(b), int(outer), int(stride), int(run), float(mult), 1 if down else 0)
            at += 1
    return EqualizeTable(jobs, segs, keep, lib.ppqhip_equalize_scale_multi)


def equalize_apply_table(items) -> EqualizeTable:
    jobs = np.zeros(len(items), dtype=_EQ_APPLY_JOB)
    keep = []
    dev = items[0][0].device if items else None
    for k, (x, scale, run, inner, group_out, divide) in enumerate(items):
        _eq_tensor(x, 'Value', k, dev); _eq_tensor(scale, 'Scale', k, dev)
        keep += [x, scale]
        jobs[k] = (x.data_ptr(), scale.data_ptr(), x.numel(), int(run), int(inner), int(group_out), scale.numel(), 1 if divide else 0, 0)
    return EqualizeTable(jobs, None, keep, lib.ppqhip_equalize_apply_multi)


def equalize_scale_multi(items) -> None:
    (items if isinstance(items, EqualizeTable) else equalize_scale_table(items)).run()


def equalize_apply_multi(items) -> None:
    (items if isinstance(items, EqualizeTable) else equalize_apply_table(items)).run()


_SPLIT_PLAN_JOB = np.dtype([('segments', '<u8'), ('src_of', '<u8'), ('count', '<u8'), ('num_segments', '<i4'), ('num_channel', '<i4'),
                            ('value_threshold', '<f4'), ('reserved', '<i4')])
_SPLIT_APPLY_JOB = np.dtype([('x', '<u8'), ('out', '<u8'), ('src_of', '<u8'), ('n', '<i8'), ('run', '<i8'), ('num_channel', '<i4'),
                             ('count', '<i4')])
SPLIT_MAX_JOBS, SPLIT_MAX_SEGMENTS = 32, 72
SPLIT_BIT = -0x80000000


def _i32(t, what: str, k: int, dev, numel: int):
    if not (isinstance(t, torch.Tensor) and t.dtype == torch.int32 and t.is_contiguous() and t.numel() == numel):
        raise RuntimeError(_KERNEL_FAILURE + f'Channel split: item {k}: {what} must be a contiguous int32 tensor of {numel}')
    if not t.is_cuda: raise RuntimeError(_KERNEL_FAILURE + f'Channel split: item {k}: {what} is not on the GPU')
    if t.device != dev: raise RuntimeError(_KERNEL_FAILURE + f'Channel split: item {k}: {what} is on another device')


def split_plan_table(items) -> EqualizeTable:
    jobs = np.zeros(len(items), dtype=_SPLIT_PLAN_JOB)
    segs = np.zeros(sum(len(it[3]) for it in items), dtype=_EQ_SEGMENT)
    keep, at = [], 0
    dev = items[0][0].device if items else None
    for k, (src_of, count, threshold, segments) in enumerate(items):
        if src_of.numel() % 2: raise RuntimeError(_KERNEL_FAILURE + f'Channel split: item {k}: SrcOf must hold 2 x C entries')
        _i32(src_of, 'SrcOf', k, dev, src_of.numel()); _i32(count, 'Count', k, dev, 1)
        keep += [src_of, count]
        jobs[k] = (segs.ctypes.data + at * _EQ_SEGMENT.itemsize, src_of.data_ptr(), count.data_ptr(), len(segments), src_of.numel() // 2,
                   float(threshold), 0)
        for t, div, a, b, outer, stride, run, mult, down in segments:
            _eq_tensor(t, 'Value', k, dev)
            keep.append(t)
            segs[at] = (t.data_ptr(), t.numel(), int(div), int(a), int(b), int(outer), int(stride), int(run), float(mult), 1 if down else 0)
            at += 1
    return EqualizeTable(jobs, segs, keep, lib.ppqhip_split_plan_multi)


def split_apply_table(items) -> EqualizeTable:
    jobs = np.zeros(len(items), dtype=_SPLIT_APPLY_JOB)
    keep = []
    dev = items[0][0].device if items else None
    for k, (x, out, src_of, C, count, run) in enumerate(items):
        _eq_tensor(x, 'Value', k, dev); _eq_tensor(out, 'Out', k, dev)
        _i32(src_of, 'SrcOf', k, dev, src_of.numel())
        C, count, run = int(C), int(count), int(run)
        if C > 0 and run > 0 and x.numel() % (C * run) == 0 and C <= count <= 2 * C:
            if out.numel() != x.numel() // C * count or src_of.numel() < count:
                raise RuntimeError(_KERNEL_FAILURE + f'Channel split: item {k}: Out must hold {x.numel() // C * count} floats and SrcOf {count} entries')
        keep += [x, out, src_of]
        jobs[k] = (x.data_ptr(), out.data_ptr(), src_of.data_ptr(), x.numel(), run, C, count)
    return EqualizeTable(jobs, None, keep, lib.ppqhip_split_apply_multi)


def split_plan_launches(items) -> int:
    chunks = jobs = segs = 0
    for it in items:
        n = len(it[3])
        if jobs == 0 or jobs == SPLIT_MAX_JOBS or segs + n > SPLIT_MAX_SEGMENTS: chunks, jobs, segs = chunks + 1, 0, 0
        jobs, segs = jobs + 1, segs + n
    return 2 * chunks


def split_apply_launches(items) -> int:
    return (len(items) + SPLIT_MAX_JOBS - 1) // SPLIT_MAX_JOBS


def split_plan_multi(items) -> None:
    (items if isinstance(items, EqualizeTable) else split_plan_table(items)).run()


def split_apply_multi(items) -> None:
    (items if isinstance(items, EqualizeTable) else split_apply_table(items)).run()


_SSD_SCALES_JOB = np.dtype([('first', _EQ_SEGMENT), ('last', _EQ_SEGMENT), ('act_range', '<u8'), ('scales', '<u8'), ('ranges', '<u8'),
                            ('num_channel', '<i4'), ('channel_ratio', '<f4')])
_SSD_APPLY_JOB = np.dtype([('x', '<u8'), ('out', '<u8'), ('scales', '<u8'), ('n', '<i8'), ('run', '<i8'), ('inner', '<i8'),
                           ('group_out', '<i8'), ('num_channel', '<i8'), ('divide', '<i4'), ('reserved', '<i4')])
_FQ_MEASURE_JOB = np.dtype([('y', '<u8'), ('r', '<u8'), ('scale', '<u8'), ('offset', '<u8'), ('sums', '<u8'), ('rows', '<i8'),
                            ('count', '<i8'), ('num_channel', '<i8'), ('elem_per_channel', '<i8'), ('clip_min', '<i4'),
                            ('clip_max', '<i4'), ('rounding', '<i4'), ('reserved', '<i4')])


def ssd_scales_multi(items) -> None:
    if not items: return
    jobs = np.zeros(len(items), dtype=_SSD_SCALES_JOB)
    dev = items[0][2].device
    for k, (first, last, act, ratio, scales, ranges) in enumerate(items):
        C = act.numel()
        for what, t, n in (('ActRange', act, C), ('Scales', scales, 4 * C), ('Ranges', ranges, 2 * C)):
            _eq_tensor(t, what, k, dev)
            if t.numel() != n: raise RuntimeError(_KERNEL_FAILURE + f'SSD scales: item {k}: {what} must hold {n} floats')
        segs = []
        for what, (t, div, a, b, outer, stride, run) in (('First', first), ('Last', last)):
            _eq_tensor(t, what, k, dev)
            segs.append((t.data_ptr(), t.numel(), int(div), int(a), int(b), int(outer), int(stride), int(run), 1.0, 0))
        jobs[k] = (segs[0], segs[1], act.data_ptr(), scales.data_ptr(), ranges.data_ptr(), C, float(ratio))
    with _DeviceOf(items[0][2]):
        _raise(lib.ppqhip_ssd_scales_multi(jobs.ctypes.data, len(items), _stream()))


def ssd_apply_multi(items) -> None:
    if not items: return
    jobs = np.zeros(len(items), dtype=_SSD_APPLY_JOB)
    dev = items[0][0].device
    for k, (x, out, scales, run, inner, group_out, divide) in enumerate(items):
        _eq_tensor(x, 'Value', k, dev); _eq_tensor(out, 'Out', k, dev); _eq_tensor(scales, 'Scales', k, dev)
        if out.numel() != 4 * x.numel(): raise RuntimeError(_KERNEL_FAILURE + f'SSD apply: item {k}: Out must hold 4 x {x.numel()} floats')
        if scales.numel() % 4: raise RuntimeError(_KERNEL_FAILURE + f'SSD apply: item {k}: Scales must be [4, C]')
        jobs[k] = (x.data_ptr(), out.data_ptr(), scales.data_ptr(), x.numel(), int(run), int(inner), int(group_out),
                   scales.numel() // 4, 1 if divide else 0, 0)
    with _DeviceOf(items[0][0]):
        _raise(lib.ppqhip_ssd_apply_multi(jobs.ctypes.data, len(items), _stream()))


def fq_measure_rows_multi(items, sums=None) -> List[torch.Tensor]:
    if not items: return []
    dev = items[0][0].device
    if sums is None: sums = [torch.empty([it[0].shape[0], 4], dtype=torch.float64, device=dev) for it in items]
    jobs = np.zeros(len(items), dtype=_FQ_MEASURE_JOB)
    for k, ((y, r, scale, offset, axis, qmin, qmax, rounding), out) in enumerate(zip(items, sums)):
        rows, count = _rows_of(y, 'Value')
        if _rows_of(r, 'Real') != (rows, count): raise RuntimeError(_KERNEL_FAILURE + f'fq measure: item {k}: Value {tuple(y.shape)} and Real {tuple(r.shape)} do not match')
        _f32(scale, 'Scale'); _f32(offset, 'Offset')
        if axis is None: C, epc = 1, count
        else:
            if axis % y.dim() != 1: raise RuntimeError(_KERNEL_FAILURE + f'fq measure: item {k}: channel_axis must be 1, {axis} was given')
            C, epc = _geometry(y.shape, 1)
        if scale.numel() != C or offset.numel() != C or not scale.is_contiguous() or not offset.is_contiguous():
            raise RuntimeError(_KERNEL_FAILURE + f'fq measure: item {k}: Scale / Offset must be contiguous with {C} element(s)')
        if any(t.device != dev for t in (y, r, scale, offset, out)): raise RuntimeError(_KERNEL_FAILURE + f'fq measure: item {k} is on another device')
        if out.dtype != torch.float64 or out.numel() != rows * 4 or not out.is_contiguous():
            raise RuntimeError(_KERNEL_FAILURE + f'fq measure: item {k}: Sums must be a contiguous float64 [{rows}, 4]')
        jobs[k] = (y.data_ptr(), r.data_ptr(), scale.data_ptr(), offset.data_ptr(), out.data_ptr(), rows, count, C, epc,
                   int(qmin), int(qmax), int(rounding), 0)
    with _DeviceOf(items[0][0]):
        _raise(lib.ppqhip_fq_measure_rows_multi(jobs.ctypes.data, len(items), _stream()))
    return sums


_FETCH_JOB = np.dtype([('x', '<u8'), ('index', '<u8'), ('out', '<u8'), ('rows', '<i8'), ('row_len', '<i8'), ('count', '<i8')])
_MEASURE_JOB = np.dtype([('p', '<u8'), ('r', '<u8'), ('index', '<u8'), ('sums', '<u8'), ('rows', '<i8'), ('row_len', '<i8'),
                         ('count', '<i8')])
_FINISH_JOB = np.dtype([('sums', '<u8'), ('acc', '<u8'), ('row_out', '<u8'), ('rows', '<i8'), ('count', '<i8'),
                        ('method', '<i4'), ('reduce', '<i4')])
MEASURE_METHODS = {'snr': 0, 'mse': 1, 'cosine': 2}
MEASURE_REDUCES = {'mean': 0, 'max': 1}


def _rows_of(t: torch.Tensor, name: str):
    _f32(t, name)
    if not t.is_contiguous(): raise RuntimeError(_KERNEL_FAILURE + f'{name} is not contiguous')
    if t.dim() < 1: raise RuntimeError(_KERNEL_FAILURE + f'{name} has no batch dimension')
    return t.shape[0], t.numel() // t.shape[0]


def _index_of(index: torch.Tensor, row_len: int, dev) -> int:
    if index.dtype != torch.int32 or not index.is_cuda or not index.is_contiguous() or index.dim() != 1 or index.numel() == 0:
        raise RuntimeError(_KERNEL_FAILURE + 'Index must be a contiguous 1-D int32 tensor on the GPU')
    if index.device != dev: raise RuntimeError(_KERNEL_FAILURE + 'Index is on another device')
# ... 1134 lines not shown
```

### ppq_amd/harness.py

```python
from typing import Callable, Dict, List, Optional

import torch
import torch.nn.functional as F

from .core import LinearQuantizationConfig, QuantizationStates, TensorQuantizationConfig, is_initial
from .core import QuantizationProperty as P
from .qfunction import PPQuantFunction

PASSIVE_OPERATIONS = {'MaxPool', 'GlobalMaxPool', 'Reshape', 'Flatten', 'Identity', 'Dropout', 'Slice', 'Pad', 'Resize',
                      'Split', 'Transpose', 'Interp', 'Squeeze', 'Unsqueeze'}
COMPUTING_OP = {'Conv', 'Gemm', 'ConvTranspose', 'MatMul'}


class Variable:
    def __init__(self, name: str, value: torch.Tensor = None, is_parameter: bool = False):
        self.name = name
        self.value = value
        self.stored_value = None
        self.is_parameter = is_parameter
        self.dest_ops: List['Operation'] = []
        self.source_op: Optional['Operation'] = None

    def __hash__(self): return hash(self.name)
    def __eq__(self, o): return isinstance(o, Variable) and o.name == self.name


class OperationQuantizationConfig:
    def __init__(self, input_quantization_configs, output_quantization_configs):
        self.input_quantization_config: List[TensorQuantizationConfig] = input_quantization_configs
        self.output_quantization_config: List[TensorQuantizationConfig] = output_quantization_configs


class Operation:
    def __init__(self, name: str, op_type: str, attributes: dict = None, inputs=None, outputs=None):
        self.name, self.type = name, op_type
        self.attributes = attributes or {}
        self.inputs: List[Variable] = inputs or []
        self.outputs: List[Variable] = outputs or []

    @ property
    def parameters(self) -> List[Variable]:
        return [v for v in self.inputs if v.is_parameter]

    def __str__(self): return f'{self.name}({self.type})'


class QuantableOperation(Operation):
    def __init__(self, op: Operation, config: OperationQuantizationConfig):
        super().__init__(op.name, op.type, op.attributes, op.inputs, op.outputs)
        self.config = config
        self.store_parameter_value()

    def store_parameter_value(self):
        for var in self.inputs:
            if var.is_parameter and isinstance(var.value, torch.Tensor): var.stored_value = var.value.detach().clone()
        return self

    def _swap_parameters(self) -> None:
        for var in self.inputs:
            if var.is_parameter and isinstance(var.value, torch.Tensor) and var.stored_value is not None:
                parked = var.value
                var.value = var.stored_value.to(parked.device)
                var.stored_value = parked

    @ property
    def config_with_variable(self):
        return list(zip(self.config.input_quantization_config, self.inputs)) + \
            list(zip(self.config.output_quantization_config, self.outputs))

    def dequantize(self):
        if getattr(self, '_dequantized', False): return self
        for cfg, _ in self.config_with_variable:
            cfg.detail['Stored State'] = cfg.state
            cfg.state = QuantizationStates.FP32
        self._swap_parameters()
        self._dequantized = True
        return self

    def restore_quantize_state(self):
        if not getattr(self, '_dequantized', False): return self
        for cfg, _ in self.config_with_variable:
            if 'Stored State' in cfg.detail: cfg.state = cfg.detail.pop('Stored State')
        self._swap_parameters()
        self._dequantized = False
        return self

    def baking_parameters(self, quant_func: Callable):
        for config, var in self.config_with_variable:
            if var.is_parameter and QuantizationStates.is_activated(config.state):
                var.value = quant_func(var.value, config)
                config.state = (QuantizationStates.BAKED if config.state == QuantizationStates.ACTIVATED
                                else QuantizationStates.PASSIVE_BAKED)


class BaseGraph:
    def __init__(self, name: str):
        self.name = name
        self.operations: Dict[str, Operation] = {}
        self.variables: Dict[str, Variable] = {}
        self.inputs: Dict[str, Variable] = {}
        self.outputs: Dict[str, Variable] = {}

    def create_variable(self, name: str, value=None, is_parameter=False) -> Variable:
        v = Variable(name, value, is_parameter)
        self.variables[name] = v
        return v

    def create_operation(self, op_type: str, name: str, inputs: List[Variable], attributes: dict = None) -> Variable:
        out = self.create_variable(name + '_out')
        op = Operation(name, op_type, attributes, list(inputs), [out])
        out.source_op = op
        for v in inputs: v.dest_ops.append(op)
        self.operations[name] = op
        return out

    def topological_sort(self) -> List[Operation]:
        return list(self.operations.values())


def _forward(op: Operation, x: List[torch.Tensor]):
    t, a = op.type, op.attributes
    if t == 'Conv':
        return F.conv2d(x[0], x[1], x[2] if len(x) > 2 else None, stride=a.get('strides', 1),
                        padding=a.get('pads', 0), groups=a.get('group', 1))
    if t == 'Gemm': return F.linear(x[0], x[1], x[2] if len(x) > 2 else None)
    if t == 'MatMul': return torch.matmul(x[0], x[1])
    if t == 'Relu': return F.relu(x[0])
    if t == 'Gelu': return F.gelu(x[0])
    if t == 'Add': return x[0] + x[1]
    if t == 'MaxPool': return F.max_pool2d(x[0], a['kernel_shape'], a.get('strides', 1), a.get('pads', 0))
    if t == 'GlobalAveragePool': return F.adaptive_avg_pool2d(x[0], 1)
    if t == 'Flatten': return torch.flatten(x[0], 1)
    if t == 'LayerNormalization': return F.layer_norm(x[0], x[0].shape[-1:], x[1], x[2])
    if t == 'Softmax': return F.softmax(x[0], dim=a.get('axis', -1))
    if t == 'Mul': return x[0] * (x[1] if len(x) > 1 else a['value'])
    if t == 'Reshape': return x[0].reshape(a['shape'])
    if t == 'Transpose': return x[0].permute(a['perm'])
    if t == 'Concat': return torch.cat([v.expand(x[-1].shape[0], *v.shape[1:]) if v.shape[0] == 1 else v for v in x],
                                       dim=a.get('axis', 1))
    if t == 'Slice': return x[0].narrow(a['axis'], a['start'], a['length'])
    if t == 'Resize': return F.interpolate(x[0], scale_factor=a.get('scale', 2), mode=a.get('mode', 'nearest'))
    raise NotImplementedError(f'Graph op: {op.name}({op.type}) has no backend implementation')


class EpilogueGroup:
    __slots__ = ('kind', 'ops', 'convs', 'add', 'relu')

    def __init__(self, kind, ops, convs, add, relu):
        self.kind, self.ops, self.convs, self.add, self.relu = kind, ops, convs, add, relu

    def __repr__(self): return f'{self.kind}({", ".join(op.name for op in self.ops)})'


def _in_cfg(op, i):
    return op.config.input_quantization_config[i] if isinstance(op, QuantableOperation) else None


def _out_cfg(op, i):
    return op.config.output_quantization_config[i] if isinstance(op, QuantableOperation) else None


def plan_epilogues(operations: List[Operation], hooks: Dict[str, object] = None, keep=(), passes_through: Callable = None,
                   grad_enabled: bool = False) -> List[EpilogueGroup]:
    if grad_enabled: return []
    from .observer import CalibrationHook
    hooks = hooks or {}
    keep = set(keep)
    if passes_through is None:
        def passes_through(c): return not QuantizationStates.is_activated(c.state)

    def through(*cfgs): return all(c is None or passes_through(c) for c in cfgs)

    def hooks_ok(members, unwritten):
        for op in members:
            h = hooks.get(op.name)
            if h is None: continue
            if type(h) is not CalibrationHook: return False
            if any(c is not None and c in h._observer_table for c in unwritten): return False
        return True

    def conv_ok(op):
        return (op.type == 'Conv' and len(op.inputs) == 3 and op.inputs[2].is_parameter and len(op.outputs) == 1
                and op.outputs[0].name not in keep)

    def only_feeds(v, op): return len(v.dest_ops) == 1 and v.dest_ops[0] is op

    def relu_after(op, i):
        if i >= len(operations): return None
        r = operations[i]
        out = op.outputs[0]
        if r.type != 'Relu' or len(r.inputs) != 1 or r.inputs[0] is not out or not only_feeds(out, r) or out.name in keep:
            return None
        return r

    def try_p2(i):
        for n_conv in (2, 1):
            j = i + n_conv
            if j + 1 >= len(operations): continue
            add, convs = operations[j], operations[i:j]
            if add.type != 'Add' or len(add.inputs) != 2 or len(add.outputs) != 1 or not all(conv_ok(c) for c in convs): continue
            by_out = {c.outputs[0].name: c for c in convs}
            x0, x1 = add.inputs
            if x0.name not in by_out or x0 is x1: continue
            if n_conv == 2 and x1.name not in by_out: continue
            ordered = [by_out[x0.name]] + ([by_out[x1.name]] if n_conv == 2 else [])
            if not all(only_feeds(c.outputs[0], add) for c in convs): continue
            relu = relu_after(add, j + 1)
            if relu is None: continue
            unwritten = (_out_cfg(add, 0), _in_cfg(relu, 0))
            between = [_out_cfg(c, 0) for c in convs] + [_in_cfg(add, 0), _in_cfg(add, 1)]
            if not through(*unwritten, *between): return None
            members = list(operations[i:j + 2])
            if not hooks_ok(members, unwritten): return None
            return EpilogueGroup('P2', members, ordered, add, relu)
        return None

    def try_p1(i):
        conv = operations[i]
        if not conv_ok(conv): return None
        relu = relu_after(conv, i + 1)
        if relu is None: return None
        unwritten = (_out_cfg(conv, 0), _in_cfg(relu, 0))
        if not through(*unwritten) or not hooks_ok([conv, relu], unwritten): return None
        return EpilogueGroup('P1', [conv, relu], [conv], None, relu)

    groups, i = [], 0
    while i < len(operations):
        g = try_p2(i) if operations[i].type == 'Conv' else None
        if g is None and operations[i].type == 'Conv': g = try_p1(i)
        if g is None:
            i += 1
            continue
        groups.append(g)
        i += len(g.ops)
    return groups


class TorchExecutor:
    def __init__(self, graph: BaseGraph, device: str = 'cuda'):
        self._graph = graph
        self._device = device
        self._default_quant_fn = PPQuantFunction
        self.cache_parameter_quantization = False
        self._param_cache: Dict[str, tuple] = {}
        self.fuse_parameter_quantization = True
        self._plans: list = []
        self._plan_signature = None
        self._plan_cache: Dict[tuple, list] = {}
        self._fused: Dict[tuple, torch.Tensor] = {}
        self._delegates: Dict[object, Callable] = {}
        self.fuse_epilogues = True
        self._epilogue_cache: Dict[tuple, dict] = {}
        self.channels_last = False
        for v in graph.variables.values():
            if v.is_parameter and v.value is not None: v.value = v.value.to(device)

    def use_channels_last(self) -> 'TorchExecutor':
        self.channels_last = True
        for v in self._graph.variables.values():
            if v.is_parameter and isinstance(v.value, torch.Tensor) and v.value.dim() == 4:
                v.value = v.value.contiguous(memory_format=torch.channels_last)
        return self

    def _place(self, value: torch.Tensor) -> torch.Tensor:
        value = value.to(self._device)
        if self.channels_last and value.dim() == 4: value = value.contiguous(memory_format=torch.channels_last)
        return value

    def register_quantize_delegate(self, config, delegator: Callable) -> None:
        self._delegates[config] = delegator

    def remove_quantize_delegate(self, config) -> None:
        self._delegates.pop(config, None)

    def quantize_function(self, tensor: torch.Tensor, config=None) -> torch.Tensor:
        if self._delegates and config in self._delegates:
            return self._delegates[config](tensor, config)
        return self._default_quant_fn(tensor, config)

    def forward_with_gradient(self, inputs, output_names: List[str] = None, hooks=None):
        return TorchExecutor.forward.__wrapped__(self, inputs, output_names, hooks)

    def partial_graph_forward(self, operations: List[Operation], feed_dict: Dict[str, torch.Tensor],
                              output_names: List[str], with_gradient: bool = False) -> List[torch.Tensor]:
        if not with_gradient:
            with torch.no_grad(): return self._partial_graph_forward(operations, feed_dict, output_names)
        return self._partial_graph_forward(operations, feed_dict, output_names)

    def _partial_graph_forward(self, operations, feed_dict, output_names):
        g = self._graph
        for name, value in feed_dict.items(): g.variables[name].value = self._place(value)
        results = [None] * len(output_names)
        self._fused_parameters(operations)
        plan, fused_done = self._epilogue_plan(operations, None, output_names), set()
        for op in operations:
            if op.name in fused_done: continue
            grp = plan.get(op.name)
            vals = self._run_epilogue(grp, lambda v: v.value, None) if grp is not None else None
            if vals is not None:
                for m in grp.ops:
                    fused_done.add(m.name)
                    for v in m.outputs:
                        v.value = vals[v.name]
                        if v.name in output_names: results[output_names.index(v.name)] = v.value
                continue
            raw_in = [v.value for v in op.inputs]
            if any(x is None for x in raw_in):
                raise ValueError(f'partial_graph_forward: input of {op.name} was not fed')
            if isinstance(op, QuantableOperation):
                qin = [self._quantize_parameter(v, c) if v.is_parameter else self.quantize_function(x, c)
                       for v, x, c in zip(op.inputs, raw_in, op.config.input_quantization_config)]
            else: qin = raw_in
            outs = _forward(op, qin)
            outs = list(outs) if isinstance(outs, (list, tuple)) else [outs]
            if isinstance(op, QuantableOperation):
                outs = [self.quantize_function(y, c) for y, c in zip(outs, op.config.output_quantization_config)]
            for v, y in zip(op.outputs, outs):
                v.value = y
                if v.name in output_names: results[output_names.index(v.name)] = y
        for v in g.variables.values():
            if not v.is_parameter: v.value = None
        return results

    def _fused_parameters(self, operations=None) -> None:
        self._fused = {}
        if not self.fuse_parameter_quantization or self._default_quant_fn is not PPQuantFunction: return
        from .ffi import FloatingQuantizePlan, LinearQuantizePlan
        todo, sig = [], []
        for op in (self._graph.operations.values() if operations is None else operations):
            if not isinstance(op, QuantableOperation): continue
            for v, c in zip(op.inputs, op.config.input_quantization_config):
                if not (v.is_parameter and isinstance(v.value, torch.Tensor) and v.value.is_cuda): continue
                if not QuantizationStates.is_activated(c.state) or c in self._delegates: continue
                pol = c.policy
                floating = pol.has_property(P.FLOATING)
                if not (pol.has_property(P.LINEAR) or floating) or pol.has_property(P.DYNAMIC): continue
                if v.value.dtype != torch.float32 or v.value.requires_grad or v.value.numel() == 0: continue
                if not (isinstance(c.scale, torch.Tensor) and isinstance(c.offset, torch.Tensor)): continue
                axis = c.channel_axis if pol.has_property(P.PER_CHANNEL) else None
                if not LinearQuantizePlan.accepts(v.value, c.scale, c.offset, axis): continue
                rnd = int(getattr(c.rounding, 'value', c.rounding))
                todo.append((v, c, axis, rnd, floating))
                sig.append((v.name, id(c), v.value.data_ptr(), c.scale.data_ptr(), c.offset.data_ptr(), tuple(v.value.shape), c.scale.numel(),
                            axis, c.quant_min, c.quant_max, rnd, floating,
                            (c.exponent_bits, c.mantissa_bits) if floating else None))
        if not todo:
            self._plans, self._plan_signature = [], None
            return
        cached = self._plan_cache.get(tuple(sig))
        if cached is not None:
            self._plan_cache[tuple(sig)] = self._plan_cache.pop(tuple(sig))
            self._plans, self._plan_signature = cached, sig
        if sig != self._plan_signature:
            groups: Dict[tuple, list] = {}
            for item in todo: groups.setdefault((item[3], item[4]), []).append(item)
            self._plans = []
            for (rnd, floating), items in groups.items():
                if floating:
                    plan = FloatingQuantizePlan([(v.value, c.scale, c.offset, axis, c.exponent_bits, c.mantissa_bits,
                                                  c.quant_min, c.quant_max) for v, c, axis, _, _ in items], rounding=rnd)
                else:
                    plan = LinearQuantizePlan([(v.value, c.scale, c.offset, axis, c.quant_min, c.quant_max)
                                               for v, c, axis, _, _ in items], rounding=rnd)
                self._plans.append((plan, [(v.name, id(c)) for v, c, _, _, _ in items]))
            self._plan_signature = sig
            if len(self._plan_cache) >= 8: self._plan_cache.pop(next(iter(self._plan_cache)))
            self._plan_cache[tuple(sig)] = self._plans
        for plan, keys in self._plans:
            for key, out in zip(keys, plan.run()): self._fused[key] = out

    def _epilogue_plan(self, operations: List[Operation], hooks, output_names) -> Dict[str, EpilogueGroup]:
        if not self.fuse_epilogues or torch.is_grad_enabled() or self._default_quant_fn is not PPQuantFunction: return {}
        states = tuple(c.state for op in operations if isinstance(op, QuantableOperation)
                       for c in (*op.config.input_quantization_config, *op.config.output_quantization_config))
        sig = (tuple(op.name for op in operations), tuple((k, id(h)) for k, h in hooks.items()) if hooks else (),
               tuple(output_names or ()), tuple(id(c) for c in self._delegates), states)
        plan = self._epilogue_cache.get(sig)
        if plan is None:
            delegates = self._delegates

            def passes_through(c): return not QuantizationStates.is_activated(c.state) and c not in delegates
            groups = plan_epilogues(operations, hooks, set(self._graph.outputs) | set(output_names or ()), passes_through)
            plan = {g.ops[0].name: g for g in groups}
            if len(self._epilogue_cache) >= 8: self._epilogue_cache.pop(next(iter(self._epilogue_cache)))
            self._epilogue_cache[sig] = plan
        return plan

    def _run_epilogue(self, grp: EpilogueGroup, raw_of: Callable, hooks) -> Optional[Dict[str, torch.Tensor]]:
        from .ffi import bias_act_, bias_add_act
        for conv in grp.convs:
            x, w = raw_of(conv.inputs[0]), conv.inputs[1].value
            if not (isinstance(x, torch.Tensor) and x.is_cuda and x.dtype == torch.float32 and x.dim() == 4
                    and isinstance(w, torch.Tensor) and w.dim() == 4): return None
            fmt = torch.channels_last if self.channels_last else torch.contiguous_format
            if not (x.is_contiguous(memory_format=fmt) and w.is_contiguous(memory_format=fmt)): return None
        if grp.add is not None:
            b_var = grp.add.inputs[1]
            if b_var.source_op not in grp.convs:
                b = raw_of(b_var)
                if not (isinstance(b, torch.Tensor) and b.is_cuda and b.dtype == torch.float32): return None
        hooks = hooks or {}
        ys, biases, qins = {}, {}, {}
        for conv in grp.ops[:len(grp.convs)]:
            raw_in = [raw_of(v) for v in conv.inputs]
            qin, in_cfgs = raw_in, None
            if isinstance(conv, QuantableOperation):
                in_cfgs = list(conv.config.input_quantization_config)
                qin = [self._quantize_parameter(v, c) if v.is_parameter else self.quantize_function(x, c)
                       for v, x, c in zip(conv.inputs, raw_in, in_cfgs)]
            hook = hooks.get(conv.name)
            if hook is not None: qin = hook.pre_forward_hook(inputs=raw_in, quant_inputs=qin, quant_configs=in_cfgs)
            a = conv.attributes
            ys[conv.name] = F.conv2d(qin[0], qin[1], None, stride=a.get('strides', 1), padding=a.get('pads', 0),
                                     groups=a.get('group', 1))
            biases[conv.name] = qin[2]
            qins[conv.name] = qin
        if grp.kind == 'P1':
            conv = grp.convs[0]
            y = ys[conv.name]
            if not bias_act_(y, biases[conv.name], relu=True):
                y.add_(biases[conv.name].view(1, -1, 1, 1)).relu_()
            tail = {conv.name: y, grp.relu.name: y}
        else:
            conv_a = grp.convs[0]
            a = ys[conv_a.name]
            conv_b = grp.convs[1] if len(grp.convs) > 1 else None
            b = ys[conv_b.name] if conv_b is not None else raw_of(grp.add.inputs[1])
            out = bias_add_act(a, biases[conv_a.name], b, biases[conv_b.name] if conv_b is not None else None, relu=True)
            if out is None:
                a.add_(biases[conv_a.name].view(1, -1, 1, 1))
                if conv_b is not None: b.add_(biases[conv_b.name].view(1, -1, 1, 1))
                out = F.relu(a + b)
            tail = {conv_a.name: a, grp.add.name: out, grp.relu.name: out}
            if conv_b is not None: tail[conv_b.name] = b
        values: Dict[str, torch.Tensor] = {}
        for op in grp.ops:
            hook = hooks.get(op.name)
            quantable = isinstance(op, QuantableOperation)
            if op.type != 'Conv':
                raw_in = [values[v.name] if v.name in values else raw_of(v) for v in op.inputs]
                qin, in_cfgs = raw_in, None
                if quantable:
                    in_cfgs = list(op.config.input_quantization_config)
                    qin = [self.quantize_function(x, c) for x, c in zip(raw_in, in_cfgs)]
                if hook is not None: hook.pre_forward_hook(inputs=raw_in, quant_inputs=qin, quant_configs=in_cfgs)
            outs = fp_outs = [tail[op.name]]
            out_cfgs = None
            if quantable:
                out_cfgs = list(op.config.output_quantization_config)
                outs = [self.quantize_function(y, c) for y, c in zip(outs, out_cfgs)]
            if hook is not None:
                outs = hook.post_forward_hook(outputs=fp_outs, quant_outputs=outs, quant_configs=out_cfgs)
            for v, y in zip(op.outputs, outs): values[v.name] = y
        return values

    def _quantize_parameter(self, var: Variable, config) -> torch.Tensor:
        hit = self._fused.get((var.name, id(config)))
        if hit is not None: return hit
        """A parameter and its scale do not change between calibration forwards, so its fake-quantised
        value is computed once and kept resident (the reference recomputes it every forward until
        ParameterBakingPass; same values, ppq/executor/torch.py:516-518).  The cache entry is keyed on
        the identity + version of value, scale and offset and on the config state."""
        if not self.cache_parameter_quantization or not QuantizationStates.is_activated(config.state):
            return self.quantize_function(var.value, config)
        key = (var.value.data_ptr(), var.value._version, id(config.scale), config.scale._version,
               id(config.offset), config.offset._version, int(getattr(config.state, 'value', config.state)))
        hit = self._param_cache.get(var.name)
        if hit is not None and hit[0] == key: return hit[1]
        q = self.quantize_function(var.value, config)
        self._param_cache[var.name] = (key, q)
        return q

    @ torch.no_grad()
    def forward_cached(self, inputs, output_names: List[str], cache: Dict[str, torch.Tensor]) -> List[torch.Tensor]:
        g = self._graph
        if isinstance(inputs, torch.Tensor): inputs = {next(iter(g.inputs)): inputs}
        elif isinstance(inputs, (list, tuple)): inputs = {k: v for k, v in zip(g.inputs, inputs)}
        for name, value in inputs.items():
            if name not in cache: cache[name] = self._place(value)
        need, stack = set(), [g.variables[n] for n in output_names]
        while stack:
            v = stack.pop()
            if v.name in cache or v.is_parameter: continue
            op = v.source_op
            if op is None: raise ValueError(f'forward_cached: graph input {v.name} was not fed')
            if op.name in need: continue
            need.add(op.name)
            stack.extend(op.inputs)
        ops = [op for op in g.topological_sort() if op.name in need]
        if ops: self._fused_parameters(ops)
        plan, fused_done = (self._epilogue_plan(ops, None, output_names) if ops else {}), set()
        for op in ops:
            if op.name in fused_done: continue
            grp = plan.get(op.name)
            vals = (self._run_epilogue(grp, lambda v: v.value if v.is_parameter else cache[v.name], None)
                    if grp is not None else None)
            if vals is not None:
                hidden = grp.relu.inputs[0].name
                for m in grp.ops:
                    fused_done.add(m.name)
                    for v in m.outputs:
                        if v.name != hidden: cache[v.name] = vals[v.name]
                continue
            raw_in = [v.value if v.is_parameter else cache[v.name] for v in op.inputs]
            if isinstance(op, QuantableOperation):
                qin = [self._quantize_parameter(v, c) if v.is_parameter else self.quantize_function(x, c)
                       for v, x, c in zip(op.inputs, raw_in, op.config.input_quantization_config)]
            else: qin = raw_in
            outs = _forward(op, qin)
            outs = list(outs) if isinstance(outs, (list, tuple)) else [outs]
            if isinstance(op, QuantableOperation):
                outs = [self.quantize_function(y, c) for y, c in zip(outs, op.config.output_quantization_config)]
            for v, y in zip(op.outputs, outs): cache[v.name] = y
        return [cache[n] for n in output_names]

    @ torch.no_grad()
    def forward(self, inputs, output_names: List[str] = None, hooks: Dict[str, object] = None) -> List[torch.Tensor]:
        g = self._graph
        if isinstance(inputs, torch.Tensor): inputs = {next(iter(g.inputs)): inputs}
        elif isinstance(inputs, (list, tuple)): inputs = {k: v for k, v in zip(g.inputs, inputs)}
        for name, value in inputs.items(): g.variables[name].value = self._place(value)
        stop_early = output_names is not None and not hooks
        if output_names is None: output_names = list(g.outputs)
        results = [None] * len(output_names)
        visited = set()
        self._fused_parameters()
        ops = g.topological_sort()
        plan, fused_done = self._epilogue_plan(ops, hooks, output_names), set()

        def finish(op, outs):
            for v, y in zip(op.outputs, outs):
                v.value = y
                if v.name in output_names: results[output_names.index(v.name)] = y
            visited.add(op.name)
            for v in op.inputs:
                if not v.is_parameter and all(d.name in visited for d in v.dest_ops): v.value = None

        for op in ops:
            if op.name in fused_done: continue
            grp = plan.get(op.name)
            vals = self._run_epilogue(grp, lambda v: v.value, hooks) if grp is not None else None
            if vals is not None:
                for m in grp.ops:
                    fused_done.add(m.name)
                    finish(m, [vals[v.name] for v in m.outputs])
                if stop_early and all(r is not None for r in results): break
                continue
            hook = hooks.get(op.name) if hooks else None
            raw_in = [v.value for v in op.inputs]
            qin = raw_in
            quantable = isinstance(op, QuantableOperation)
            if quantable:
                in_cfgs = list(op.config.input_quantization_config)
                qin = [self._quantize_parameter(v, c) if v.is_parameter else self.quantize_function(x, c)
                       for v, x, c in zip(op.inputs, raw_in, in_cfgs)]
            if hook is not None:
                qin = hook.pre_forward_hook(inputs=raw_in, quant_inputs=qin, quant_configs=in_cfgs)
            outs = _forward(op, qin)
            outs = list(outs) if isinstance(outs, (list, tuple)) else [outs]
            fp_outs = outs
            if quantable:
                out_cfgs = list(op.config.output_quantization_config)
                outs = [self.quantize_function(y, c) for y, c in zip(outs, out_cfgs)]
            if hook is not None:
                outs = hook.post_forward_hook(outputs=fp_outs, quant_outputs=outs, quant_configs=out_cfgs)
            finish(op, outs)
            if stop_early and all(r is not None for r in results): break
        for v in g.variables.values():
            if not v.is_parameter: v.value = None
        return results


def quantize_graph(graph: BaseGraph, activation_algorithm: str = 'kl', per_channel_weight: bool = True,
                   symmetrical: bool = True, weight_symmetrical: bool = True, num_of_bits: int = 8,
                   hist_bins: int = None, fp8: bool = False, passive_bias: bool = False) -> None:
    qmin, qmax = (-(2 ** (num_of_bits - 1)), 2 ** (num_of_bits - 1) - 1) if symmetrical else (0, 2 ** num_of_bits - 1)
    wmin, wmax = (-(2 ** (num_of_bits - 1)), 2 ** (num_of_bits - 1) - 1) if weight_symmetrical else (0, 2 ** num_of_bits - 1)

    def act_cfg():
        if fp8:
            from .core import FloatingQuantizationConfig
            return FloatingQuantizationConfig(calibration='floating')
        c = LinearQuantizationConfig(symmetrical=symmetrical, quant_min=qmin, quant_max=qmax, num_of_bits=num_of_bits,
                                     calibration=activation_algorithm)
        if hist_bins is not None: c.detail['OBSERVER_KL_HIST_BINS_MANUL_OVERRIDE'] = hist_bins
        return c

    for name, op in list(graph.operations.items()):
        in_cfgs = []
        for i, v in enumerate(op.inputs):
            if v.is_parameter and op.type in COMPUTING_OP and i == 1:
                in_cfgs.append(LinearQuantizationConfig(symmetrical=weight_symmetrical, quant_min=wmin, quant_max=wmax,
                                                        num_of_bits=num_of_bits, calibration='minmax',
                                                        channel_axis=0 if per_channel_weight else None))
            elif v.is_parameter and passive_bias and not fp8 and op.type in COMPUTING_OP and i == 2:
                in_cfgs.append(LinearQuantizationConfig(symmetrical=True, quant_min=-(2 ** 31 - 1), quant_max=2 ** 31 - 1, num_of_bits=32,
                                                        calibration=None, channel_axis=0 if per_channel_weight else None))
                in_cfgs[-1].state = QuantizationStates.PASSIVE_INIT
            elif v.is_parameter:
                c = act_cfg(); c.state = QuantizationStates.FP32
                in_cfgs.append(c)
            else:
                in_cfgs.append(act_cfg())
        qop = QuantableOperation(op, OperationQuantizationConfig(in_cfgs, [act_cfg() for _ in op.outputs]))
        for v in qop.inputs: v.dest_ops[v.dest_ops.index(op)] = qop
        for v in qop.outputs: v.source_op = qop
        graph.operations[name] = qop
    ops = list(graph.operations.values())
    for op in ops:
        for v, c in zip(op.inputs, op.config.input_quantization_config):
            if v.source_op is not None and is_initial(c):
                src = v.source_op
                c.dominated_by = src.config.output_quantization_config[src.outputs.index(v)]
    for op in ops:
        out = op.outputs[0]
        if op.type in COMPUTING_OP | {'Add'} and len(out.dest_ops) == 1 and out.dest_ops[0].type in {'Relu', 'Gelu'}:
            op.config.output_quantization_config[0].dominated_by = out.dest_ops[0].config.output_quantization_config[0]
        if op.type in PASSIVE_OPERATIONS:
            first = op.config.input_quantization_config[0]
            if first.dominated_by is not op.config.output_quantization_config[0].dominated_by:
                op.config.output_quantization_config[0].dominated_by = first
            else: op.config.output_quantization_config[0].state = QuantizationStates.OVERLAPPED


from .parameters import ParameterBakingPass, ParameterQuantizePass


def _he(shape, gen) -> torch.Tensor:
    fan_in = shape[1] * (shape[2] * shape[3] if len(shape) == 4 else 1)
    return torch.randn(shape, generator=gen) * (2.0 / fan_in) ** 0.5


def resnet50_graph(seed: int = 0, num_classes: int = 1000) -> BaseGraph:
    gen = torch.Generator().manual_seed(seed)
    g = BaseGraph('resnet50')
    x = g.create_variable('input')
    g.inputs['input'] = x
    n = [0]

    def conv(inp, cin, cout, k, stride=1, pad=0, relu=True, tag='conv'):
        n[0] += 1
        w = g.create_variable(f'{tag}{n[0]}_w', _he([cout, cin, k, k], gen), True)
        b = g.create_variable(f'{tag}{n[0]}_b', torch.randn(cout, generator=gen) * 0.05, True)
        y = g.create_operation('Conv', f'{tag}{n[0]}', [inp, w, b], {'strides': stride, 'pads': pad})
        if relu: y = g.create_operation('Relu', f'relu{n[0]}', [y])
        return y

    y = conv(x, 3, 64, 7, 2, 3)
    y = g.create_operation('MaxPool', 'maxpool', [y], {'kernel_shape': 3, 'strides': 2, 'pads': 1})
    cin = 64
    for stage, (blocks, width) in enumerate(zip([3, 4, 6, 3], [64, 128, 256, 512])):
        for blk in range(blocks):
            stride = 2 if (blk == 0 and stage > 0) else 1
            identity = y
            z = conv(y, cin, width, 1)
            z = conv(z, width, width, 3, stride, 1)
            z = conv(z, width, width * 4, 1, relu=False)
            if blk == 0:
                identity = conv(y, cin, width * 4, 1, stride, 0, relu=False, tag='down')
            n[0] += 1
            z = g.create_operation('Add', f'add{n[0]}', [z, identity])
            y = g.create_operation('Relu', f'relu{n[0]}', [z])
            cin = width * 4
    y = g.create_operation('GlobalAveragePool', 'gap', [y])
    y = g.create_operation('Flatten', 'flatten', [y])
    w = g.create_variable('fc_w', torch.randn([num_classes, 2048], generator=gen) * (1.0 / 2048) ** 0.5, True)
    b = g.create_variable('fc_b', torch.zeros(num_classes), True)
    y = g.create_operation('Gemm', 'fc', [y, w, b])
    g.outputs[y.name] = y
    return g


def yolov6s_graph(seed: int = 0, num_classes: int = 80) -> BaseGraph:
    gen = torch.Generator().manual_seed(seed)
    g = BaseGraph('yolov6s')
    x = g.create_variable('input')
    g.inputs['input'] = x
    n = [0]

    def conv(inp, cin, cout, k=3, stride=1, relu=True, tag='conv'):
        n[0] += 1
        a = (6.0 / (cin * k * k)) ** 0.5
        w = g.create_variable(f'{tag}{n[0]}_w', (torch.rand([cout, cin, k, k], generator=gen) * 2 - 1) * a, True)
        b = g.create_variable(f'{tag}{n[0]}_b', torch.randn(cout, generator=gen) * 0.05, True)
        y = g.create_operation('Conv', f'{tag}{n[0]}', [inp, w, b], {'strides': stride, 'pads': k // 2})
        if relu: y = g.create_operation('Relu', f'relu{n[0]}', [y])
        return y

    def rep(inp, c, repeats):
        for _ in range(repeats): inp = conv(inp, c, c, 3, tag='rep')
        return inp

    def cat(name, vs): return g.create_operation('Concat', name, vs, {'axis': 1})

    y = conv(x, 3, 32, 3, 2, tag='stem')
    feats, cin = [], 32
    for stage, (c, r) in enumerate(zip([64, 128, 256, 512], [2, 4, 6, 2])):
        y = conv(y, cin, c, 3, 2, tag=f's{stage}_down')
        y = rep(y, c, r)
        cin = c
        feats.append(y)
    p = conv(feats[3], 512, 256, 1, tag='sppf_in')
    m1 = g.create_operation('MaxPool', 'sppf_pool1', [p], {'kernel_shape': 5, 'strides': 1, 'pads': 2})
    m2 = g.create_operation('MaxPool', 'sppf_pool2', [m1], {'kernel_shape': 5, 'strides': 1, 'pads': 2})
    m3 = g.create_operation('MaxPool', 'sppf_pool3', [m2], {'kernel_shape': 5, 'strides': 1, 'pads': 2})
    c5 = conv(cat('sppf_cat', [p, m1, m2, m3]), 1024, 512, 1, tag='sppf_out')
    c3, c4 = feats[1], feats[2]
    r5 = conv(c5, 512, 128, 1, tag='reduce5')
    u5 = g.create_operation('Resize', 'up5', [r5], {'scale': 2})
    p4 = rep(conv(cat('cat_p4', [u5, c4]), 128 + 256, 128, 3, tag='p4_in'), 128, 3)
    r4 = conv(p4, 128, 64, 1, tag='reduce4')
    u4 = g.create_operation('Resize', 'up4', [r4], {'scale': 2})
    p3 = rep(conv(cat('cat_p3', [u4, c3]), 64 + 128, 64, 3, tag='p3_in'), 64, 3)
    d3 = conv(p3, 64, 64, 3, 2, tag='down3')
    n4 = rep(conv(cat('cat_n4', [d3, r4]), 64 + 64, 128, 3, tag='n4_in'), 128, 3)
    d4 = conv(n4, 128, 128, 3, 2, tag='down4')
    n5 = rep(conv(cat('cat_n5', [d4, r5]), 128 + 128, 256, 3, tag='n5_in'), 256, 3)
    for name, f, c in (('s8', p3, 64), ('s16', n4, 128), ('s32', n5, 256)):
        stem = conv(f, c, c, 1, tag=f'head_{name}_stem')
        cls = conv(conv(stem, c, c, 3, tag=f'head_{name}_cls'), c, num_classes, 1, relu=False, tag=f'head_{name}_cls_out')
        box = conv(conv(stem, c, c, 3, tag=f'head_{name}_box'), c, 4, 1, relu=False, tag=f'head_{name}_box_out')
        g.outputs[cls.name] = cls
        g.outputs[box.name] = box
    _unit_variance_init(g, torch.rand(2, 3, 96, 96, generator=gen))
    return g


@ torch.no_grad()
def _unit_variance_init(g: BaseGraph, sample: torch.Tensor) -> None:
    values = {next(iter(g.inputs)): sample}
    for op in g.operations.values():
        xs = [v.value if v.is_parameter else values[v.name] for v in op.inputs]
        y = _forward(op, xs)
        if op.type == 'Conv':
            std = float(y.std())
            if std > 0:
                op.inputs[1].value = op.inputs[1].value / std
# ... 121 lines not shown
```

### ppq_amd/observer.py

```python
from typing import Dict, List, Optional, Sequence, Tuple

import weakref

import numpy as np
import torch

from .core import (OBSERVER_FLOATING_MSE_FETCHES, OBSERVER_ISOTONE_OBSERVER_AXIS, OBSERVER_KL_HIST_BINS, OBSERVER_KL_HIST_BINS_MANUL_OVERRIDE,
                   OBSERVER_MIN_SCALE, OBSERVER_MIN_SCALE_MANUL_OVERRIDE, OBSERVER_MSE_HIST_BINS,
                   OBSERVER_PERCENTILE, OBSERVER_PERCENTILE_MANUL_OVERRIDE, is_initial, set_activated)
from .core import QuantizationProperty as P
from .core import RoundingPolicy
from .ffi import CUDA, quantile_hint
from .round import ppq_numerical_round, ppq_round_to_power_of_2


def minmax_to_scale_offset(min_val: float, max_val: float, config,
                           scale_threshold: float = OBSERVER_MIN_SCALE) -> Tuple[float, float]:
    if OBSERVER_MIN_SCALE_MANUL_OVERRIDE in config.detail:
        scale_threshold = config.detail[OBSERVER_MIN_SCALE_MANUL_OVERRIDE]
    scale, offset = 1, 0
    if min_val > 0: min_val = 0
    if max_val < 0: max_val = 0
    if config.policy.has_property(P.ASYMMETRICAL):
        range = float(max_val - min_val)
        scale = range / (config.quant_max - config.quant_min)
        scale = max(scale, scale_threshold)
        offset = ppq_numerical_round(float(-min_val / scale))
    elif config.policy.has_property(P.SYMMETRICAL):
        range = 2 * float(max(abs(max_val), abs(min_val)))
        scale = range / (config.quant_max - config.quant_min)
        scale = max(scale, scale_threshold)
        offset = 0
    else:
        raise TypeError('Tensor Min Max Observer Excepts either ASYMMETRICAL or SYMMETRICAL quantization config.')
    if config.policy.has_property(P.POWER_OF_2):
        scale = ppq_round_to_power_of_2(scale, policy=RoundingPolicy.ROUND_UP)
    return scale, offset


def minmax_to_scale_offset_channels(mins: np.ndarray, maxs: np.ndarray, config,
                                    scale_threshold: float = OBSERVER_MIN_SCALE) -> Tuple[list, list]:
    if config.policy.has_property(P.POWER_OF_2) or mins.dtype != np.float32 or maxs.dtype != np.float32:
        pairs = [minmax_to_scale_offset(a, b, config, scale_threshold) for a, b in zip(mins, maxs)]
        return [p[0] for p in pairs], [p[1] for p in pairs]
    if OBSERVER_MIN_SCALE_MANUL_OVERRIDE in config.detail:
        scale_threshold = config.detail[OBSERVER_MIN_SCALE_MANUL_OVERRIDE]
    zero = np.float32(0)
    lo = np.where(mins > 0, zero, mins)
    hi = np.where(maxs < 0, zero, maxs)
    levels = config.quant_max - config.quant_min
    if config.policy.has_property(P.ASYMMETRICAL):
        with np.errstate(over='ignore', divide='ignore', invalid='ignore'):
            scale = (hi - lo).astype(np.float64) / levels
            scale = np.where(scale_threshold > scale, scale_threshold, scale)
            offset = np.rint(((-lo) / scale.astype(np.float32)).astype(np.float64))
        return scale.tolist(), [int(v) for v in offset.tolist()]
    if config.policy.has_property(P.SYMMETRICAL):
        a, b = np.abs(hi), np.abs(lo)
        m = np.where(b > a, b, a)
        scale = 2 * m.astype(np.float64) / levels
        scale = np.where(scale_threshold > scale, scale_threshold, scale)
        return scale.tolist(), [0] * int(scale.size)
    raise TypeError('Tensor Min Max Observer Excepts either ASYMMETRICAL or SYMMETRICAL quantization config.')


_DEFERRED_SETS: Optional[list] = None


def _set_per_tensor(config, scale: float, offset: float, device) -> None:
    if _DEFERRED_SETS is not None:
        _DEFERRED_SETS.append((config, scale, offset, device))
        return
    config.scale = torch.tensor([scale], dtype=torch.float32, device=device).squeeze(0)
    config.offset = torch.tensor([offset], dtype=torch.float32, device=device).squeeze(0)
    set_activated(config)


def _flush_deferred_sets(pending: list) -> None:
    by_dev: Dict[object, list] = {}
    for item in pending: by_dev.setdefault(torch.device(item[3]), []).append(item)
    for dev, items in by_dev.items():
        chunks = [np.asarray(v, dtype=np.float32).reshape(-1) for _, s, o, _ in items for v in (s, o)]
        flat = torch.from_numpy(np.concatenate(chunks)).to(dev)
        pos = 0
        for k, (config, s, _, _) in enumerate(items):
            if isinstance(s, (list, tuple)):
                C = len(s)
                config.scale, config.offset = flat[pos: pos + C], flat[pos + C: pos + 2 * C]
                pos += 2 * C
            else:
                config.scale, config.offset = flat[pos], flat[pos + 1]
                pos += 2
            set_activated(config)


class ObservationQueue:
    def __init__(self, max_pending_bytes: int = 4 << 30):
        self._minmax = []
        self._minmax_c = []
        self._hist = {}
        self._quantile = {}
        self._bytes = 0
        self._max = max_pending_bytes
        self.launches = 0
        self.recorder: Optional[list] = None

    def __len__(self):
        return (len(self._minmax) + len(self._minmax_c) + sum(len(v) for v in self._hist.values())
                + sum(len(v) for v in self._quantile.values()))

    def _grow(self, value) -> None:
        self._bytes += value.numel() * 4
        if self._bytes > self._max: self.flush()

    def add_minmax(self, value: torch.Tensor, slots: torch.Tensor) -> None:
        self._minmax.append((value, slots))
        self._grow(value)

    def add_minmax_c(self, value: torch.Tensor, channel_axis: int, mins: torch.Tensor, maxs: torch.Tensor, fresh: bool) -> None:
        if any(m.data_ptr() == mins.data_ptr() for _, _, m, _, _ in self._minmax_c): self.flush()
        self._minmax_c.append((value, channel_axis, mins, maxs, bool(fresh)))
        self._grow(value)

    def add_hist(self, value: torch.Tensor, rows: torch.Tensor, asymmetric: bool, p0: float, p1: float = 0.0) -> None:
        self._hist.setdefault((bool(asymmetric), rows.shape[1], value.device), []).append((value, rows, p0, p1))
        self._grow(value)

    def add_quantile(self, value: torch.Tensor, q: float, hint: Optional[torch.Tensor] = None) -> torch.Tensor:
        dest = torch.empty(2, dtype=torch.float32, device=value.device)
        self._quantile.setdefault((float(q), value.device), []).append((value, dest, hint))
        self._grow(value)
        return dest

    def flush(self) -> None:
        if self._quantile:
            pending, self._quantile = self._quantile, {}
            for (q, _), items in pending.items():
                hints, seen = [h for _, _, h in items], set()
                for k in range(len(hints) - 1, -1, -1):
                    if hints[k] is None: continue
                    key = hints[k].data_ptr()
                    if key in seen: hints[k] = None
                    else: seen.add(key)
                CUDA.Quantile_Multi([v for v, _, _ in items], q, [d for _, d, _ in items], hints)
                self.launches += 1
        if self._minmax:
            by_dev = {}
            for v, sl in self._minmax: by_dev.setdefault(v.device, []).append((v, sl))
            self._minmax = []
            for items in by_dev.values():
                CUDA.MinMax_T_Slots_Multi([v for v, _ in items], [sl for _, sl in items])
                self.launches += 1
        if self._minmax_c:
            by_dev = {}
            for it in self._minmax_c: by_dev.setdefault(it[0].device, []).append(it)
            self._minmax_c = []
            for dev, items in by_dev.items():
                CUDA.MinMax_C_Multi([i[0] for i in items], [i[1] for i in items], [i[2] for i in items],
                                    [i[3] for i in items], [i[4] for i in items])
                self.launches += 1
        if self._hist:
            pending, self._hist = self._hist, {}
            for (asym, _, _), items in pending.items():
                vs, rows = [i[0] for i in items], [i[1] for i in items]
                if asym:
                    CUDA.Histogram_Asymmetric_T_Rows_Multi([i[2] for i in items], [i[3] for i in items], vs, rows)
                else:
                    CUDA.Histogram_T_Rows_Multi(vs, rows, [i[2] for i in items])
                self.launches += 1
        self._bytes = 0


SIBLING_PREFETCH = False
_LIVE_OBSERVERS: "weakref.WeakSet" = weakref.WeakSet()
_PREFETCHING = False


def _prefetch_siblings(ob) -> None:
    global _PREFETCHING
    if not SIBLING_PREFETCH or _PREFETCHING: return
    _PREFETCHING = True
    try:
        def device_of(o):
            t = getattr(o, '_hist', None) if getattr(o, '_hist', None) is not None else getattr(o, '_range', None)
            return None if t is None else t.device
        dev = device_of(ob)
        sibs = [o for o in list(_LIVE_OBSERVERS) if isinstance(o, TorchMinMaxObserver) and is_initial(o._quant_cfg) and device_of(o) == dev]
        if ob not in sibs: sibs.append(ob)
        _prefetch(sibs)
    finally:
        _PREFETCHING = False


class BaseTensorObserver:
    queue: Optional[ObservationQueue] = None

    def __init__(self, watch_on, quant_cfg):
        self._watch_on = watch_on
        self._quant_cfg = quant_cfg
        _LIVE_OBSERVERS.add(self)

    def _drain(self) -> None:
        if self.queue is not None and len(self.queue): self.queue.flush()

    def observe(self, value):
        raise NotImplementedError('Implement this function first.')

    def render_quantization_config(self):
        raise NotImplementedError('Implement this function first.')

    def __str__(self) -> str:
        return ('PPQ Tensor Observer (' + self.__class__.__name__ + ') mount on variable ' +
                getattr(self._watch_on, 'name', str(self._watch_on)) + ' observing algorithm: ' +
                str(self._quant_cfg.observer_algorithm))

    def report(self) -> str:
        return ''

    def pending_range(self) -> Optional[torch.Tensor]:
        return None

    def take_range(self, host: np.ndarray) -> None:
        """Receive the host copy of ``pending_range()`` (fetched for all observers at once)."""

    def reducible(self) -> List[Tuple[torch.Tensor, str]]:
        return []

    def gatherable(self) -> List[torch.Tensor]:
        return []

    def take_gathered(self, merged: List[torch.Tensor]) -> None:
        pass


_RANGE_SEEDS: Dict[object, tuple] = {}


def _range_seed(device) -> tuple:
    hit = _RANGE_SEEDS.get(device)
    if hit is None:
        one = torch.tensor([float('inf'), float('-inf')], dtype=torch.float32, device=device)
        hit = _RANGE_SEEDS[device] = (one, one.repeat(CUDA.minmax_slots(), 1).contiguous())
    return hit


class TorchMinMaxObserver(BaseTensorObserver):
    def __init__(self, watch_on, quant_cfg):
        super().__init__(watch_on, quant_cfg)
        self._range: Optional[torch.Tensor] = None
        self._slots: Optional[torch.Tensor] = None
        self._slots_dirty = False
        self._queued_c = False
        self._host_range: Optional[np.ndarray] = None
        self._observed = False

    @ torch.no_grad()
    def observe(self, value: torch.Tensor):
        assert isinstance(value, torch.Tensor), 'TorchMinMaxObserver can only deal with torch Tensor values'
        assert value.numel() > 0, (f'You are observing an empty tensor({getattr(self._watch_on, "name", "")}).')
        if not is_initial(self._quant_cfg): return
        cfg = self._quant_cfg
        if cfg.policy.has_property(P.PER_TENSOR):
            if self._range is None:
                seed = _range_seed(value.device)
                self._range = seed[0].clone()
                self._slots = seed[1].clone()
            if self.queue is not None and value.is_cuda: self.queue.add_minmax(value, self._slots)
            else: CUDA.MinMax_T_Slots(value, self._slots)
            self._slots_dirty = True
        elif cfg.policy.has_property(P.PER_CHANNEL):
            queued = (self.queue is not None and value.is_cuda and CUDA.minmax_c_outer_is_one(value, cfg.channel_axis))
            fresh = False
            if self._range is None:
                C = value.shape[cfg.channel_axis]
                self._range = torch.empty((2, C), dtype=torch.float32, device=value.device)
                fresh = queued and CUDA.minmax_c_fresh_ok(value, cfg.channel_axis)
                if not fresh: self._range[0].fill_(float('inf')); self._range[1].fill_(float('-inf'))
            if queued:
                self.queue.add_minmax_c(value, cfg.channel_axis, self._range[0], self._range[1], fresh)
                self._queued_c = True
            else: CUDA.MinMax_C(value, cfg.channel_axis, self._range[0], self._range[1])
        else:
            raise TypeError('Min-max Observer only work with per-tensor or per-channel quantize policy.')
        self._observed = True
        self._host_range = None

    def _fold(self) -> None:
        if self._queued_c:
            self._drain()
            self._queued_c = False
        if self._slots_dirty:
            self._drain()
            CUDA.MinMax_Slots_Finish(self._slots, self._range)
            self._slots_dirty = False

    def pending_range(self):
        if not (is_initial(self._quant_cfg) and self._observed): return None
        self._fold()
        return self._range

    def take_range(self, host: np.ndarray) -> None:
        self._host_range = host

    def reducible(self):
        if self._range is None: return []
        self._fold()
        if self._range.ndim == 1: return [(self._range[0:1], 'min'), (self._range[1:2], 'max')]
        return [(self._range[0], 'min'), (self._range[1], 'max')]

    def _range_on_host(self) -> np.ndarray:
        if not self._observed:
            raise ValueError('Can not render quantization config yet, Observer data collator is empty. '
                             'Invoke observe() function before render config.')
        if self._host_range is None: _prefetch_siblings(self)
        if self._host_range is None:
            self._fold()
            self._host_range = self._range.cpu().numpy()
        return self._host_range

    def render_quantization_config(self):
        if not is_initial(self._quant_cfg): return
        cfg = self._quant_cfg
        r = self._range_on_host()
        device = self._range.device
        if cfg.policy.has_property(P.PER_TENSOR):
            scale, offset = minmax_to_scale_offset(min_val=float(r[0]), max_val=float(r[1]), config=cfg)
            _set_per_tensor(cfg, scale, offset, device)
        elif cfg.policy.has_property(P.PER_CHANNEL):
            scales, offsets = minmax_to_scale_offset_channels(np.ascontiguousarray(r[0]), np.ascontiguousarray(r[1]), cfg)
            if _DEFERRED_SETS is not None:
                _DEFERRED_SETS.append((cfg, scales, offsets, device))
                return
            cfg.scale = torch.tensor(scales, dtype=torch.float32, device=device)
            cfg.offset = torch.tensor(offsets, dtype=torch.float32, device=device)
            set_activated(cfg)
        else:
            raise TypeError('Min-max Observer only work with per-tensor or per-channel quantize policy.')


class TorchHistObserver(TorchMinMaxObserver):
    def __init__(self, watch_on, quant_cfg, hist_bins: int = OBSERVER_KL_HIST_BINS):
        self._phase = 'Detecting Minmax'
        self._hist = None
        self._rows = None
        self._rows_dirty = False
        self._hist_scale = None
        self._min = None
        self._max = None
        self._losses: Optional[np.ndarray] = None
        if OBSERVER_KL_HIST_BINS_MANUL_OVERRIDE in quant_cfg.detail:
            hist_bins = quant_cfg.detail[OBSERVER_KL_HIST_BINS_MANUL_OVERRIDE]
        self._hist_bins = hist_bins
        super().__init__(watch_on, quant_cfg)

    def observe(self, value: torch.Tensor):
        if not is_initial(self._quant_cfg): return
        assert value.numel() > 0, (f'You are observing an empty tensor({getattr(self._watch_on, "name", "")}).')
        if self._phase == 'Detecting Minmax':
            if self.queue is not None and self.queue.recorder is not None and value.is_cuda:
                self.queue.recorder.append((self, value))
            return super().observe(value)
        elif self._phase == 'Collating Hist':
            self._losses = None
            if getattr(self, '_best', None) is not None: self._best = None
            if self._hist is None:
                self._hist = torch.zeros(size=(self._hist_bins,), dtype=torch.int32, device=value.device)
                if self._hist_bins <= 16384:
                    self._rows = torch.zeros(size=(CUDA.hist_rows(), self._hist_bins), dtype=torch.int32,
                                             device=value.device)
            if self._quant_cfg.policy.has_property(P.ASYMMETRICAL):
                if self._rows is not None:
                    if self.queue is not None: self.queue.add_hist(value, self._rows, True, self._min, self._max)
                    else: CUDA.Histogram_Asymmetric_T_Rows(self._min, self._max, tensor=value, rows=self._rows)
                    self._rows_dirty = True
                else:
                    CUDA.Histogram_Asymmetric_T(self._min, self._max, tensor=value, histogram=self._hist)
            elif self._quant_cfg.policy.has_property(P.SYMMETRICAL):
                if self._rows is not None:
                    if self.queue is not None: self.queue.add_hist(value, self._rows, False, self._hist_scale)
                    else: CUDA.Histogram_T_Rows(tensor=value, rows=self._rows, scale=self._hist_scale)
                    self._rows_dirty = True
                else:
                    CUDA.Histogram_T(tensor=value, histogram=self._hist, scale=self._hist_scale)
            else:
                raise TypeError('Quantization Property is invalid, expect either ASYMMETRICAL or SYMMETRICAL config here.')

    def pending_range(self):
        return super().pending_range() if self._phase == 'Detecting Minmax' else None

    def _fold_hist(self) -> None:
        if self._rows_dirty:
            self._drain()
            CUDA.Histogram_Rows_Finish(self._rows, self._hist)
            self._rows_dirty = False
            if self._rows.is_cuda: self._rows.record_stream(torch.cuda.current_stream(self._rows.device))
            self._rows = None

    def histogram(self) -> Optional[torch.Tensor]:
        self._fold_hist()
        return self._hist

    def reducible(self):
        if self._phase == 'Detecting Minmax': return super().reducible()
        return [(self.histogram(), 'sum')] if self._hist is not None else []

    search_kind = 'kl'

    def search_key(self):
        return ('kl', self._hist_bins, self._quant_cfg.num_of_bits)

    def take_losses(self, losses: np.ndarray) -> None:
        self._losses = losses

    def hist_to_scale_offset(self, histogram: torch.Tensor, hist_bins: int, hist_scale: float, config,
                             scale_threshold: float = OBSERVER_MIN_SCALE) -> Tuple[float, int]:
        if config.policy.has_property(P.ASYMMETRICAL):
            raise PermissionError('KL observer is not designed for ASYMMETRICAL quantization')
        if OBSERVER_MIN_SCALE_MANUL_OVERRIDE in config.detail:
            scale_threshold = config.detail[OBSERVER_MIN_SCALE_MANUL_OVERRIDE]
        quant_bins = 2 ** (config.num_of_bits - 1)
        if self._losses is None: _prefetch_siblings(self)
        if self._losses is None:
            self._losses = CUDA.KLLosses(histogram, config.num_of_bits).cpu().numpy()[0]
        losses = [{'kl': float(kl), 'bin_range': (j + 1) * quant_bins} for j, kl in enumerate(self._losses)]
        best_bin_range = sorted(losses, key=lambda x: x['kl'])[0]['bin_range']
        scale, offset = (best_bin_range / self._hist_bins) * hist_scale * (self._hist_bins / quant_bins), 0
        scale = max(scale, scale_threshold)
        if config.policy.has_property(P.POWER_OF_2):
            scale = ppq_round_to_power_of_2(scale, policy=RoundingPolicy.ROUND_HALF_UP)
        return scale, offset

    def render_quantization_config(self):
        if not is_initial(self._quant_cfg): return
        if not self._quant_cfg.policy.has_property(P.PER_TENSOR):
            raise ValueError('Hist observer can only apply with per-tensor quantization config.')
        if self._phase == 'Detecting Minmax':
            r = self._range_on_host()
            min_val, max_val = float(r[0]), float(r[1])
            if self._quant_cfg.policy.has_property(P.SYMMETRICAL):
                hist_range = float(max(abs(max_val), abs(min_val)))
            else:
                hist_range = max_val - min_val
            self._min = min_val
            self._max = max_val
            self._hist_scale = hist_range / self._hist_bins
            self._phase = 'Collating Hist'
        elif self._phase == 'Collating Hist':
            if self._hist is None:
                raise ValueError('Can not render quantization config yet, histogram is empty. '
                                 'Invoke observe() function before render config.')
            scale, offset = self.hist_to_scale_offset(histogram=self.histogram(), hist_bins=self._hist_bins,
                                                      hist_scale=self._hist_scale, config=self._quant_cfg)
            _set_per_tensor(self._quant_cfg, scale, offset, self._hist.device)


class ChannelwiseKLObserver(TorchHistObserver):
    def __init__(self, watch_on, quant_cfg, hist_bins: int = OBSERVER_KL_HIST_BINS):
        super().__init__(watch_on, quant_cfg, hist_bins)
        if not quant_cfg.policy.has_property(P.PER_CHANNEL) or not quant_cfg.policy.has_property(P.SYMMETRICAL):
            raise TypeError('ChannelwiseKLObserver needs a symmetrical per-channel config.')
        self._scales_dev: Optional[torch.Tensor] = None

    def observe(self, value: torch.Tensor):
        if not is_initial(self._quant_cfg): return
        assert value.numel() > 0, (f'You are observing an empty tensor({getattr(self._watch_on, "name", "")}).')
        if self._phase == 'Detecting Minmax':
            return TorchMinMaxObserver.observe(self, value)
        C = value.shape[self._quant_cfg.channel_axis]
        if self._hist is None:
            self._hist = torch.zeros(size=(C, self._hist_bins), dtype=torch.int32, device=value.device)
        CUDA.Histogram_C_Scales(value, self._quant_cfg.channel_axis, self._hist, self._scales_dev)

    def histogram(self): return self._hist

    def render_quantization_config(self):
        cfg = self._quant_cfg
        if not is_initial(cfg): return
        if self._phase == 'Detecting Minmax':
            r = self._range_on_host()
            hs = [float(max(abs(float(hi)), abs(float(lo)))) / self._hist_bins for lo, hi in zip(r[0], r[1])]
            self._hist_scale = hs
            self._scales_dev = torch.tensor(hs, dtype=torch.float32, device=self._range.device)
            self._phase = 'Collating Hist'
            return
        if self._hist is None:
            raise ValueError('Can not render quantization config yet, histogram is empty. '
                             'Invoke observe() function before render config.')
        losses = CUDA.KLLosses(self._hist, cfg.num_of_bits).cpu().numpy()
        scales = []
        for c in range(self._hist.shape[0]):
            self._losses = losses[c]
            scale, _ = self.hist_to_scale_offset(self._hist[c], self._hist_bins, self._hist_scale[c], cfg)
            scales.append(scale)
        self._losses = None
        cfg.scale = torch.tensor(scales, dtype=torch.float32, device=self._hist.device)
        cfg.offset = torch.zeros(len(scales), dtype=torch.float32, device=self._hist.device)
        set_activated(cfg)


class TorchPercentileObserver(BaseTensorObserver):
    def __init__(self, watch_on, quant_cfg):
        super().__init__(watch_on, quant_cfg)
        if OBSERVER_PERCENTILE_MANUL_OVERRIDE not in quant_cfg.detail:
            self._percentile = OBSERVER_PERCENTILE
        else: self._percentile = quant_cfg.detail[OBSERVER_PERCENTILE_MANUL_OVERRIDE]
        self._percentile_collector = []
        self._sum: Optional[torch.Tensor] = None
        self._hint: Optional[torch.Tensor] = None

    @ torch.no_grad()
    def observe(self, value: torch.Tensor):
        if not is_initial(self._quant_cfg): return
        assert value is not None, ('You are observing an Empty Tensor. '
                                   '(This Error is usually due to you have a wrong Quantizer configuration.)')
        assert value.numel() > 0, (f'You are observing an empty tensor({getattr(self._watch_on, "name", "")}).')
        assert isinstance(value, torch.Tensor), 'TorchMinMaxObserver can only deal with torch Tensor values'
        if self._quant_cfg.policy.has_property(P.PER_TENSOR):
            if value.is_cuda and (self._hint is None or self._hint.device != value.device):
                self._hint = quantile_hint(value.device)
            if self.queue is not None and value.is_cuda:
                self._percentile_collector.append(self.queue.add_quantile(value, self._percentile, self._hint).view(1, -1))
            else:
                self._percentile_collector.append(CUDA.Quantile_Hinted(value, self._percentile, self._hint).view(1, -1))
        elif self._quant_cfg.policy.has_property(P.PER_CHANNEL):
            raise PermissionError('Percentile observer can not deal with per channel quantization.')
        else:
            raise TypeError('Min-max Observer only work with per-tensor or per-channel quantize policy.')

    def _fold(self):
        self._drain()
        if self._percentile_collector:
            stacked = torch.cat(self._percentile_collector, dim=0).float()
            part = torch.cat([stacked.sum(dim=0), stacked.new_tensor([float(stacked.shape[0])])])
            self._sum = part if self._sum is None else self._sum + part
            self._percentile_collector = []

    def reducible(self):
        self._fold()
        return [(self._sum, 'sum')] if self._sum is not None else []

    def render_quantization_config(self):
        if not is_initial(self._quant_cfg): return
        if self._quant_cfg.policy.has_property(P.PER_TENSOR):
            single_shard = self._sum is None
            if single_shard and len(self._percentile_collector) == 0:
                raise ValueError('Can not render quantization config yet, Observer data collator is empty. '
                                 'Invoke observe() function before render config.')
            self._drain()
            if single_shard:
                device = self._percentile_collector[-1].device
                mean = torch.cat(self._percentile_collector, dim=0).float().mean(dim=0).cpu()
            else:
                self._fold()
                device = self._sum.device
                mean = (self._sum[:2] / self._sum[2]).cpu()
            scale, offset = minmax_to_scale_offset(min_val=mean[1].item(), max_val=mean[0].item(),
                                                   config=self._quant_cfg)
            _set_per_tensor(self._quant_cfg, scale, offset, device)
        elif self._quant_cfg.policy.has_property(P.PER_CHANNEL):
            raise PermissionError('Percentile observer can not deal with per channel quantization.')
        else:
            raise TypeError('Min-max Observer only work with per-tensor or per-channel quantize policy.')


class TorchMSEObserver(TorchHistObserver):
    search_kind = 'mse'

    def __init__(self, watch_on, quant_cfg, bins: int = OBSERVER_MSE_HIST_BINS):
        super().__init__(watch_on, quant_cfg)
        self._hist_bins = bins
        self._best: Optional[np.ndarray] = None

    def search_key(self):
        cfg = self._quant_cfg
        return ('mse', self._hist_bins, cfg.quant_min, cfg.quant_max, cfg.policy.has_property(P.SYMMETRICAL))

    def take_best(self, best: np.ndarray) -> None:
        self._best = best

    def compute_mse_loss(self, histogram: list, start: int, step: int, end: int) -> float:
        return CUDA.compute_mse_loss(histogram=histogram, start=start, step=step, end=end)

    def hist_to_scale_offset(self, histogram: torch.Tensor, hist_bins: int, hist_scale: float, config,
                             scale_threshold: float = OBSERVER_MIN_SCALE) -> Tuple[float, int]:
        if OBSERVER_MIN_SCALE_MANUL_OVERRIDE in config.detail:
            scale_threshold = config.detail[OBSERVER_MIN_SCALE_MANUL_OVERRIDE]
        if config.policy.has_property(P.PER_CHANNEL):
            raise PermissionError('Torch Mse observer do not support PER_CHANNEL policy now, please wait.')
        symmetrical = config.policy.has_property(P.SYMMETRICAL)
        if self._best is None: _prefetch_siblings(self)
        if self._best is None:
            dev = histogram.device
            self._best = CUDA.MseSearch(histogram.reshape(1, -1),
                                        torch.tensor([hist_scale], dtype=torch.float64, device=dev),
                                        torch.tensor([self._min], dtype=torch.float64, device=dev),
                                        config.quant_min, config.quant_max, symmetrical).cpu().numpy()[0]
        best_start, best_end = int(self._best[0]), int(self._best[1])
        if not symmetrical:
            range_min, range_max = (best_start * hist_scale) + self._min, (best_end * hist_scale) + self._min
        else:
            range_min, range_max = -(best_end * hist_scale), (best_end * hist_scale)
        return minmax_to_scale_offset(range_min, range_max, config, scale_threshold)


class ChannelwiseMSEObserver(TorchMSEObserver):
    def __init__(self, watch_on, quant_cfg, bins: int = OBSERVER_MSE_HIST_BINS):
        super().__init__(watch_on, quant_cfg, bins)
        if not quant_cfg.policy.has_property(P.PER_CHANNEL):
            raise TypeError('ChannelwiseMSEObserver needs a per-channel config.')
        self._mins_dev = self._maxs_dev = self._scales_dev = None

    def observe(self, value: torch.Tensor):
        if not is_initial(self._quant_cfg): return
        assert value.numel() > 0, (f'You are observing an empty tensor({getattr(self._watch_on, "name", "")}).')
        if self._phase == 'Detecting Minmax':
            return TorchMinMaxObserver.observe(self, value)
        cfg = self._quant_cfg
        C = value.shape[cfg.channel_axis]
        if self._hist is None:
            self._hist = torch.zeros(size=(C, self._hist_bins), dtype=torch.int32, device=value.device)
        if cfg.policy.has_property(P.ASYMMETRICAL):
            CUDA.Histogram_Asymmetric_C_Ranges(value, cfg.channel_axis, self._hist, self._mins_dev, self._maxs_dev)
        else:
            CUDA.Histogram_C_Scales(value, cfg.channel_axis, self._hist, self._scales_dev)

    def histogram(self): return self._hist

    def reducible(self):
        if self._phase == 'Detecting Minmax': return TorchMinMaxObserver.reducible(self)
        return [(self._hist, 'sum')] if self._hist is not None else []

    def render_quantization_config(self):
        cfg = self._quant_cfg
        if not is_initial(cfg): return
        sym = cfg.policy.has_property(P.SYMMETRICAL)
        if self._phase == 'Detecting Minmax':
            r = self._range_on_host()
            self._min = [float(v) for v in r[0]]
            self._max = [float(v) for v in r[1]]
            self._hist_scale = [(float(max(abs(hi), abs(lo))) if sym else (hi - lo)) / self._hist_bins
                                for lo, hi in zip(self._min, self._max)]
            dev = self._range.device
            self._mins_dev = torch.tensor(self._min, dtype=torch.float32, device=dev)
            self._maxs_dev = torch.tensor(self._max, dtype=torch.float32, device=dev)
            self._scales_dev = torch.tensor(self._hist_scale, dtype=torch.float32, device=dev)
            self._phase = 'Collating Hist'
            return
        if self._hist is None:
            raise ValueError('Can not render quantization config yet, histogram is empty. '
                             'Invoke observe() function before render config.')
        dev = self._hist.device
        best = CUDA.MseSearch(self._hist, torch.tensor(self._hist_scale, dtype=torch.float64, device=dev),
                              torch.tensor(self._min, dtype=torch.float64, device=dev), cfg.quant_min, cfg.quant_max,
                              sym).cpu().numpy()
        scale_threshold = cfg.detail.get(OBSERVER_MIN_SCALE_MANUL_OVERRIDE, OBSERVER_MIN_SCALE)
        scales, offsets = [], []
        for c in range(self._hist.shape[0]):
            start, end, hs = int(best[c][0]), int(best[c][1]), self._hist_scale[c]
            if sym: range_min, range_max = -(end * hs), (end * hs)
            else: range_min, range_max = (start * hs) + self._min[c], (end * hs) + self._min[c]
            s_, o_ = minmax_to_scale_offset(range_min, range_max, cfg, scale_threshold)
            scales.append(s_); offsets.append(o_)
        cfg.scale = torch.tensor(scales, dtype=torch.float32, device=dev)
        cfg.offset = torch.tensor(offsets, dtype=torch.float32, device=dev)
        set_activated(cfg)


class ConstantObserver(BaseTensorObserver):
    def __init__(self, watch_on, quant_cfg):
        super().__init__(watch_on, quant_cfg)
        self._value_shape = None
        self._value_device = None
# ... 370 lines not shown
```

Before: 3528 samples/s.

## Fuse per-tensor minmax and histogram observation into bias/add/ReLU epilogue kernels

Adds epilogue kernels that apply bias, residual add and ReLU and, in the same pass, accumulate per-tensor min/max slots or KL histogram rows for the observed outputs. Observers receive these results directly and skip their separate observation when the fused path has already consumed the tensor. This removes an extra full read of each activation and separate statistic launches for conv epilogue outputs. In exchange the epilogue kernel grows more complex, uses LDS for up to three histograms and may run at lower occupancy, and the observers gain new state handling around the fused path.

```diff
diff --git a/include/ppq_hip.h b/include/ppq_hip.h
--- a/include/ppq_hip.h
+++ b/include/ppq_hip.h
@@ -225,6 +225,22 @@
                     int relu, void* stream);
 int ppqhip_bias_add_act(float* a, const float* bias_a, float* b, const float* bias_b, float* out,
                         int64_t n, int64_t num_channel, int64_t elem_per_channel, int relu, void* stream);
+
+int64_t ppqhip_epilogue_hist_max_bins(void);
+int ppqhip_bias_act_minmax(float* y, const float* bias, int64_t n, int64_t num_channel, int64_t elem_per_channel,
+                           int relu, float* slots, void* stream);
+int ppqhip_bias_add_act_minmax(float* a, const float* bias_a, float* b, const float* bias_b, float* out,
+                               int64_t n, int64_t num_channel, int64_t elem_per_channel, int relu,
+                               int store_a, int store_b, float* slots_a, float* slots_b, float* slots_out,
+                               void* stream);
+int ppqhip_bias_act_hist(float* y, const float* bias, int64_t n, int64_t num_channel, int64_t elem_per_channel,
+                         int relu, int32_t* rows, float p0, float p1, int asymmetric, int clip_outliers,
+                         int64_t num_bins, void* stream);
+int ppqhip_bias_add_act_hist(float* a, const float* bias_a, float* b, const float* bias_b, float* out,
+                             int64_t n, int64_t num_channel, int64_t elem_per_channel, int relu,
+                             int store_a, int store_b, int32_t* rows_a, float p0_a, float p1_a,
+                             int32_t* rows_b, float p0_b, float p1_b, int32_t* rows_out, float p0_out, float p1_out,
+                             int asymmetric, int clip_outliers, int64_t num_bins, void* stream);
 
 typedef struct ppqhip_adaround_job {
     const float* w;
diff --git a/ppq_amd/_lib.py b/ppq_amd/_lib.py
--- a/ppq_amd/_lib.py
+++ b/ppq_amd/_lib.py
@@ -38,6 +38,15 @@
     'ppqhip_lsq_finish_multi': (c_int, [c_vp, c_int, c_vp]),
     'ppqhip_bias_act': (c_int, [c_f32p, c_f32p, c_i64, c_i64, c_i64, c_int, c_vp]),
     'ppqhip_bias_add_act': (c_int, [c_f32p, c_f32p, c_f32p, c_f32p, c_f32p, c_i64, c_i64, c_i64, c_int, c_vp]),
+    'ppqhip_epilogue_hist_max_bins': (c_i64, []),
+    'ppqhip_bias_act_minmax': (c_int, [c_f32p, c_f32p, c_i64, c_i64, c_i64, c_int, c_f32p, c_vp]),
+    'ppqhip_bias_add_act_minmax': (c_int, [c_f32p, c_f32p, c_f32p, c_f32p, c_f32p, c_i64, c_i64, c_i64, c_int, c_int, c_int,
+                                           c_f32p, c_f32p, c_f32p, c_vp]),
+    'ppqhip_bias_act_hist': (c_int, [c_f32p, c_f32p, c_i64, c_i64, c_i64, c_int, c_i32p, c_flt, c_flt, c_int, c_int, c_i64,
+                                     c_vp]),
+    'ppqhip_bias_add_act_hist': (c_int, [c_f32p, c_f32p, c_f32p, c_f32p, c_f32p, c_i64, c_i64, c_i64, c_int, c_int, c_int,
+                                         c_i32p, c_flt, c_flt, c_i32p, c_flt, c_flt, c_i32p, c_flt, c_flt, c_int, c_int,
+                                         c_i64, c_vp]),
     'ppqhip_fq_float_t': (c_int, [c_f32p, c_f32p, c_f32p, c_f32p, c_i64, c_int, c_int, c_flt, c_flt, c_int, c_vp]),
     'ppqhip_fq_float_c': (c_int, [c_f32p, c_f32p, c_f32p, c_f32p, c_i64, c_i64, c_i64, c_int, c_int, c_flt, c_flt,
                                   c_int, c_vp]),
diff --git a/ppq_amd/calibration.py b/ppq_amd/calibration.py
--- a/ppq_amd/calibration.py
+++ b/ppq_amd/calibration.py
@@ -29,7 +29,7 @@
                  process_group=None, check_steps: bool = True, async_observe: bool = False,
                  use_hip_graph: bool = False, batch_observations: bool = True,
                  reuse_activations: bool = False, reuse_budget_bytes: int = 64 << 30,
-                 queue_bytes: int = None) -> None:
+                 queue_bytes: int = None, fuse_epilogue_stats: bool = True) -> None:
         super().__init__(name='PPQ Runtime Calibration Pass')
         self._method = method
         self._observers: Dict[str, OperationObserver] = {}
@@ -44,6 +44,7 @@
         self._queue = None
         self._reuse_activations = reuse_activations
         self._queue_bytes = queue_bytes
+        self._fuse_epilogue_stats = fuse_epilogue_stats
         self._reuse_budget = reuse_budget_bytes
         self._replay: list = []
         self._replay_bytes = 0
@@ -199,6 +200,7 @@
         if self._batch_observations and self._side_stream is None:
             from .observer import ObservationQueue
             self._queue = ObservationQueue() if self._queue_bytes is None else ObservationQueue(self._queue_bytes)
+            self._queue.fuse_epilogue_stats = bool(self._fuse_epilogue_stats)
         for ob in self._all_tensor_observers(): ob.queue = self._queue
 
         self._replay, self._replay_bytes = [], 0
diff --git a/ppq_amd/csrc/binner.hpp b/ppq_amd/csrc/binner.hpp
--- /dev/null
+++ b/ppq_amd/csrc/binner.hpp
@@ -0,0 +1,66 @@
+#pragma once
+
+#include "common.hpp"
+
+namespace ppqhip {
+
+typedef float v2f __attribute__((ext_vector_type(2)));
+
+__device__ __forceinline__ bool quotient_is_safe(float t) {
+    return __builtin_fabsf(t - __builtin_rintf(t)) >= __builtin_fabsf(t) * 0x1p-22f;
+}
+
+__device__ __forceinline__ int f2i_abs(float t) {
+    int r;
+    asm("v_cvt_i32_f32_e64 %0, |%1|" : "=v"(r) : "v"(t));
+    return r;
+}
+__device__ __forceinline__ int f2i_floor(float t) {
+    int r;
+    asm("v_cvt_flr_i32_f32 %0, %1" : "=v"(r) : "v"(t));
+    return r;
+}
+
+template <bool ASYM, bool CLIP, bool HOT>
+struct Binner : WaveBinCounter<ASYM, CLIP, HOT> {
+    using Base = WaveBinCounter<ASYM, CLIP, HOT>;
+    using Base::h; using Base::last; using Base::hot_bin; using Base::hot_cnt;
+    float a0, hs, rcp;
+
+    __device__ __forceinline__ void set_rule(float a, float scale) { a0 = a; hs = scale; rcp = 1.0f / scale; }
+
+    __device__ __forceinline__ void bins4(const float4& v, int (&b)[4]) const {
+        v2f x01 = {v.x, v.y}, x23 = {v.z, v.w};
+        if (ASYM) { x01 = x01 - a0; x23 = x23 - a0; }
+        const v2f t01 = x01 * rcp, t23 = x23 * rcp;
+        const v2f r01 = {__builtin_rintf(t01.x), __builtin_rintf(t01.y)};
+        const v2f r23 = {__builtin_rintf(t23.x), __builtin_rintf(t23.y)};
+        const v2f d01 = t01 - r01, d23 = t23 - r23;
+        const v2f e01 = t01 * 0x1p-22f, e23 = t23 * 0x1p-22f;
+        const bool u0 = !(__builtin_fabsf(d01.x) >= __builtin_fabsf(e01.x));
+        const bool u1 = !(__builtin_fabsf(d01.y) >= __builtin_fabsf(e01.y));
+        const bool u2 = !(__builtin_fabsf(d23.x) >= __builtin_fabsf(e23.x));
+        const bool u3 = !(__builtin_fabsf(d23.y) >= __builtin_fabsf(e23.y));
+        b[0] = ASYM ? f2i_floor(t01.x) : f2i_abs(t01.x);
+        b[1] = ASYM ? f2i_floor(t01.y) : f2i_abs(t01.y);
+        b[2] = ASYM ? f2i_floor(t23.x) : f2i_abs(t23.x);
+        b[3] = ASYM ? f2i_floor(t23.y) : f2i_abs(t23.y);
+        if (u0 | u1 | u2 | u3) {
+            if (u0) b[0] = exact_bin(ASYM ? x01.x : __builtin_fabsf(v.x));
+            if (u1) b[1] = exact_bin(ASYM ? x01.y : __builtin_fabsf(v.y));
+            if (u2) b[2] = exact_bin(ASYM ? x23.x : __builtin_fabsf(v.z));
+            if (u3) b[3] = exact_bin(ASYM ? x23.y : __builtin_fabsf(v.w));
+        }
+    }
+    __device__ __forceinline__ int exact_bin(float a) const { return f2i_sat(__builtin_floorf(a / hs)); }
+
+    __device__ __forceinline__ int bin1(float v) const {
+        const float a = ASYM ? (v - a0) : __builtin_fabsf(v);
+        const float t = a * rcp;
+        if (quotient_is_safe(t)) return ASYM ? f2i_floor(t) : f2i_abs(t);
+        return exact_bin(a);
+    }
+
+};
+
+}
diff --git a/ppq_amd/csrc/epilogue.hip b/ppq_amd/csrc/epilogue.hip
--- a/ppq_amd/csrc/epilogue.hip
+++ b/ppq_amd/csrc/epilogue.hip
@@ -1,4 +1,4 @@
-#include "common.hpp"
+#include "epilogue.hpp"
 
 namespace ppqhip {
 namespace {
@@ -20,33 +20,9 @@
     FastDiv nc;
 };
 
-__device__ __forceinline__ uint32_t channel_of(uint32_t i, const FastDiv& epc, const FastDiv& nc) {
-    const uint32_t row = fdiv(i, epc);
-    return row - fdiv(row, nc) * nc.d;
-}
-
-__device__ __forceinline__ float act(float v, bool relu) {
-    return (relu && !__builtin_isnan(v)) ? __builtin_fmaxf(v, 0.f) : v;
-}
-
-__device__ __forceinline__ float4 add4(const float4& x, const float4& y) {
-    return make_float4(x.x + y.x, x.y + y.y, x.z + y.z, x.w + y.w);
-}
-
 template <bool RELU>
 __device__ __forceinline__ float4 act4(const float4& v) {
     return make_float4(act(v.x, RELU), act(v.y, RELU), act(v.z, RELU), act(v.w, RELU));
-}
-
-template <bool PLANE>
-__device__ __forceinline__ float4 bias4(const float* __restrict__ bias, uint32_t v, const FastDiv& epc, const FastDiv& nc) {
-    if (PLANE) {
-        const float t = bias[channel_of(v, epc, nc)];
-        return make_float4(t, t, t, t);
-    }
-    const uint32_t i = v * 4u;
-    return make_float4(bias[channel_of(i, epc, nc)], bias[channel_of(i + 1, epc, nc)], bias[channel_of(i + 2, epc, nc)],
-                       bias[channel_of(i + 3, epc, nc)]);
 }
 
 template <bool RESID, bool BIAS_B, bool RELU>
@@ -122,19 +98,6 @@
 #undef PPQ_LAUNCH_EP
 }
 
-int validate(int64_t n, int64_t C, int64_t epc, const char* what) {
-    if (n <= 0 || n > 0x7fffffffLL) {
-        set_error("%s: n=%lld is empty or has more than 2^31 - 1 elements", what, (long long)n);
-        return PPQHIP_ERR_INVALID_VALUE;
-    }
-    if (C <= 0 || epc <= 0 || C > 0x7fffffffLL || epc > 0x7fffffffLL || n % (C * epc) != 0) {
-        set_error("%s: n=%lld is not [outer, %lld channels, %lld elem/channel]", what, (long long)n, (long long)C,
-                  (long long)epc);
-        return PPQHIP_ERR_INVALID_VALUE;
-    }
-    return PPQHIP_OK;
-}
-
 }
 }
 
@@ -144,7 +107,7 @@
 
 int ppqhip_bias_act(float* y, const float* bias, int64_t n, int64_t num_channel, int64_t elem_per_channel, int relu,
                     void* stream) {
-    if (int st = validate(n, num_channel, elem_per_channel, "bias_act")) return st;
+    if (int st = validate_epilogue(n, num_channel, elem_per_channel, "bias_act")) return st;
     if (!y || !bias) { set_error("bias_act: null pointer"); return PPQHIP_ERR_INVALID_VALUE; }
     hipStream_t s = (hipStream_t)stream;
     EpArgs p{};
@@ -157,7 +120,7 @@
 
 int ppqhip_bias_add_act(float* a, const float* bias_a, float* b, const float* bias_b, float* out, int64_t n,
                         int64_t num_channel, int64_t elem_per_channel, int relu, void* stream) {
-    if (int st = validate(n, num_channel, elem_per_channel, "bias_add_act")) return st;
+    if (int st = validate_epilogue(n, num_channel, elem_per_channel, "bias_add_act")) return st;
     if (!a || !bias_a || !b || !out) { set_error("bias_add_act: null pointer"); return PPQHIP_ERR_INVALID_VALUE; }
     hipStream_t s = (hipStream_t)stream;
     EpArgs p{};
diff --git a/ppq_amd/csrc/epilogue.hpp b/ppq_amd/csrc/epilogue.hpp
--- /dev/null
+++ b/ppq_amd/csrc/epilogue.hpp
@@ -0,0 +1,44 @@
+#pragma once
+
+#include "common.hpp"
+
+namespace ppqhip {
+
+__device__ __forceinline__ uint32_t channel_of(uint32_t i, const FastDiv& epc, const FastDiv& nc) {
+    const uint32_t row = fdiv(i, epc);
+    return row - fdiv(row, nc) * nc.d;
+}
+
+__device__ __forceinline__ float act(float v, bool relu) {
+    return (relu && !__builtin_isnan(v)) ? __builtin_fmaxf(v, 0.f) : v;
+}
+
+__device__ __forceinline__ float4 add4(const float4& x, const float4& y) {
+    return make_float4(x.x + y.x, x.y + y.y, x.z + y.z, x.w + y.w);
+}
+
+template <bool PLANE>
+__device__ __forceinline__ float4 bias4(const float* __restrict__ bias, uint32_t v, const FastDiv& epc, const FastDiv& nc) {
+    if (PLANE) {
+        const float t = bias[channel_of(v, epc, nc)];
+        return make_float4(t, t, t, t);
+    }
+    const uint32_t i = v * 4u;
+    return make_float4(bias[channel_of(i, epc, nc)], bias[channel_of(i + 1, epc, nc)], bias[channel_of(i + 2, epc, nc)],
+                       bias[channel_of(i + 3, epc, nc)]);
+}
+
+inline int validate_epilogue(int64_t n, int64_t C, int64_t epc, const char* what) {
+    if (n <= 0 || n > 0x7fffffffLL) {
+        set_error("%s: n=%lld is empty or has more than 2^31 - 1 elements", what, (long long)n);
+        return PPQHIP_ERR_INVALID_VALUE;
+    }
+    if (C <= 0 || epc <= 0 || C > 0x7fffffffLL || epc > 0x7fffffffLL || n % (C * epc) != 0) {
+        set_error("%s: n=%lld is not [outer, %lld channels, %lld elem/channel]", what, (long long)n, (long long)C,
+                  (long long)epc);
+        return PPQHIP_ERR_INVALID_VALUE;
+    }
+    return PPQHIP_OK;
+}
+
+}
diff --git a/ppq_amd/csrc/epilogue_stats.hip b/ppq_amd/csrc/epilogue_stats.hip
--- /dev/null
+++ b/ppq_amd/csrc/epilogue_stats.hip
@@ -0,0 +1,360 @@
+#include "binner.hpp"
+#include "epilogue.hpp"
+
+#include <cmath>
+
+namespace ppqhip {
+namespace {
+
+constexpr int kEsBlock = 512;
+constexpr int kEsWgPerCu = 2;
+constexpr int kEsU = 2;
+constexpr uint32_t kEsTileVec = (uint32_t)kEsBlock * kEsU;
+constexpr int kEsMaxHist = 3;
+constexpr int kEsLdsBudget = 48 << 10;
+constexpr int kEsMaxBins = kEsLdsBudget / (kEsMaxHist * (int)sizeof(int));
+constexpr uint32_t kEsMinTilesHist = 4;
+constexpr uint32_t kEsMinTilesMinMax = 2;
+constexpr int kEsWgPerCuMinMax = 4;
+
+struct EsArgs {
+    float* a;
+    const float* bias_a;
+    float* b;
+    const float* bias_b;
+    float* out;
+    uint32_t nvec;
+    uint32_t tail;
+    int ntail;
+    FastDiv epc;
+    FastDiv nc;
+    int relu, store_a, store_b;
+    float* slots[kEsMaxHist];
+    int* rows[kEsMaxHist];
+    float ra[kEsMaxHist];
+    float hs[kEsMaxHist];
+    int bins;
+};
+
+__device__ __forceinline__ float4 act4r(const float4& v, bool relu) {
+    return make_float4(act(v.x, relu), act(v.y, relu), act(v.z, relu), act(v.w, relu));
+}
+
+template <bool HIST, bool ASYM, bool CLIP>
+struct Taker {
+    Binner<ASYM, CLIP, true> acc;
+    float mn, mx;
+    bool on;
+
+    __device__ __forceinline__ void init(bool enabled, int* copy, int bins, float a, float hs) {
+        on = enabled; mn = INFINITY; mx = -INFINITY;
+        acc.init(copy, bins);
+        acc.set_rule(a, hs);
+    }
+    template <bool FULL>
+    __device__ __forceinline__ void take4(const float4& v, bool in, bool elect) {
+        if (!on) return;
+        if (HIST) {
+            int b[4];
+            acc.bins4(v, b);
+            if (elect) acc.elect(b[0], FULL ? true : in);
+            if (FULL && CLIP) acc.commit4_exec(b);
+            else {
+                acc.template commit<FULL>(b[0], in); acc.template commit<FULL>(b[1], in);
+                acc.template commit<FULL>(b[2], in); acc.template commit<FULL>(b[3], in);
+            }
+        } else if (FULL || in) {
+            mn = fminf(fminf(mn, v.x), fminf(v.y, fminf(v.z, v.w)));
+            mx = fmaxf(fmaxf(mx, v.x), fmaxf(v.y, fmaxf(v.z, v.w)));
+        }
+    }
+    __device__ __forceinline__ void take1(float v, bool in) {
+        if (!on) return;
+        if (HIST) {
+            const int b = acc.bin1(v);
+            acc.elect(b, in);
+            acc.template commit<false>(b, in);
+        } else if (in) { mn = fminf(mn, v); mx = fmaxf(mx, v); }
+    }
+};
+
+template <bool HIST, bool RESID, bool BIAS_B, bool PLANE, bool ASYM, bool CLIP>
+__global__ __launch_bounds__(kEsBlock, (kEsBlock * kEsWgPerCu + 255) / 256)
+void epilogue_stats_kernel(const EsArgs p) {
+    extern __shared__ int lds[];
+    const uint32_t G = gridDim.x, g = blockIdx.x;
+    const uint32_t tiles = (p.nvec + kEsTileVec - 1) / kEsTileVec;
+    uint32_t t, t_end;
+    even_split(tiles, G, g, t, t_end);
+    if (t >= t_end) return;
+
+    float4* a4 = reinterpret_cast<float4*>(p.a);
+    float4* b4 = reinterpret_cast<float4*>(p.b);
+    float4* o4 = reinterpret_cast<float4*>(p.out);
+    const bool relu = p.relu != 0, store_a = p.store_a != 0, store_b = p.store_b != 0;
+    const int bins = p.bins;
+
+    const bool on_a = HIST ? p.rows[0] != nullptr : p.slots[0] != nullptr;
+    const bool on_b = BIAS_B && (HIST ? p.rows[1] != nullptr : p.slots[1] != nullptr);
+    const bool on_o = RESID && (HIST ? p.rows[2] != nullptr : p.slots[2] != nullptr);
+    const int off_b = on_a ? bins : 0, off_o = off_b + (on_b ? bins : 0);
+    const int lds_ints = off_o + (on_o ? bins : 0);
+    Taker<HIST, ASYM, CLIP> ta, tb, to;
+    ta.init(on_a, lds, bins, p.ra[0], p.hs[0]);
+    tb.init(on_b, lds + off_b, bins, p.ra[1], p.hs[1]);
+    to.init(on_o, lds + off_o, bins, p.ra[2], p.hs[2]);
+
+    struct Tile { float4 a[kEsU], ba[kEsU], b[kEsU], bb[kEsU]; };
+    auto fetch = [&](Tile& T, uint32_t tile) {
+        const uint32_t base = tile * kEsTileVec + threadIdx.x;
+#pragma unroll
+        for (int k = 0; k < kEsU; k++) {
+            const uint32_t vv = min(base + k * kEsBlock, p.nvec - 1);
+            T.a[k] = a4[vv];
+            T.ba[k] = bias4<PLANE>(p.bias_a, vv, p.epc, p.nc);
+            if (RESID) T.b[k] = b4[vv];
+            if (BIAS_B) T.bb[k] = bias4<PLANE>(p.bias_b, vv, p.epc, p.nc);
+        }
+    };
+    auto consume_t = [&](const Tile& T, uint32_t tile, auto full_tag) {
+        constexpr bool FULL = decltype(full_tag)::value;
+        const uint32_t base = tile * kEsTileVec + threadIdx.x;
+#pragma unroll
+        for (int k = 0; k < kEsU; k++) {
+            const uint32_t vv = base + k * kEsBlock;
+            const bool in = FULL || vv < p.nvec;
+            const float4 x = add4(T.a[k], T.ba[k]);
+            if (!RESID) {
+                const float4 y = act4r(x, relu);
+                if (in) a4[vv] = y;
+                ta.template take4<FULL>(y, in, k == 0);
+                continue;
+            }
+            if (in && store_a) a4[vv] = x;
+            ta.template take4<FULL>(x, in, k == 0);
+            float4 y = T.b[k];
+            if (BIAS_B) {
+                y = add4(y, T.bb[k]);
+                if (in && store_b) b4[vv] = y;
+                tb.template take4<FULL>(y, in, k == 0);
+            }
+            const float4 o = act4r(add4(x, y), relu);
+            if (in) o4[vv] = o;
+            to.template take4<FULL>(o, in, k == 0);
+        }
+    };
+    auto consume = [&](const Tile& T, uint32_t tile) {
+        if ((tile + 1) * kEsTileVec <= p.nvec) consume_t(T, tile, std::true_type{});
+        else consume_t(T, tile, std::false_type{});
+    };
+
+    Tile bufa, bufb;
+    fetch(bufa, t);
+    if (HIST) {
+        for (int i = threadIdx.x; i < lds_ints; i += kEsBlock) lds[i] = 0;
+        asm volatile("s_waitcnt lgkmcnt(0)\n\ts_barrier" ::: "memory");
+    }
+    for (uint32_t k = t;;) {
+        if (k + 1 >= t_end) { consume(bufa, k); break; }
+        fetch(bufb, k + 1);
+        consume(bufa, k);
+        ++k;
+        if (k + 1 >= t_end) { consume(bufb, k); break; }
+        fetch(bufa, k + 1);
+        consume(bufb, k);
+        ++k;
+    }
+
+    if (!PLANE && g == 0 && p.ntail > 0) {
+        const bool in = (int)threadIdx.x < p.ntail;
+        const uint32_t i = p.tail + (in ? threadIdx.x : 0u);
+        const uint32_t c = channel_of(i, p.epc, p.nc);
+        const float x = p.a[i] + p.bias_a[c];
+        if (!RESID) {
+            const float y = act(x, relu);
+            if (in) p.a[i] = y;
+            ta.take1(y, in);
+        } else {
+            if (in && store_a) p.a[i] = x;
+            ta.take1(x, in);
+            float y = p.b[i];
+            if (BIAS_B) {
+                y = y + p.bias_b[c];
+                if (in && store_b) p.b[i] = y;
+                tb.take1(y, in);
+            }
+            const float o = act(x + y, relu);
+            if (in) p.out[i] = o;
+            to.take1(o, in);
+        }
+    }
+
+    if (HIST) {
+        if (on_a) ta.acc.flush_hot();
+        if (on_b) tb.acc.flush_hot();
+        if (on_o) to.acc.flush_hot();
+        asm volatile("s_waitcnt lgkmcnt(0)" ::: "memory");
+        __syncthreads();
+        auto add_row = [&](bool on, const int* copy, int* rows) {
+            if (!on) return;
+            int* __restrict__ row = rows + (size_t)g * bins;
+            for (int b = threadIdx.x; b < bins; b += kEsBlock) {
+                const int s = copy[b];
+                if (s) row[b] += s;
+            }
+        };
+        add_row(on_a, lds, p.rows[0]);
+        add_row(on_b, lds + off_b, p.rows[1]);
+        add_row(on_o, lds + off_o, p.rows[2]);
+    } else {
+        float* red = reinterpret_cast<float*>(lds);
+        constexpr int W = kEsBlock / kWave;
+        const int wid = threadIdx.x >> 6, lane = threadIdx.x & 63;
+        auto wave_fold = [&](bool on, Taker<HIST, ASYM, CLIP>& tk, int k) {
+            if (!on) return;
+            const float mn = wave_min(tk.mn), mx = wave_max(tk.mx);
+            if (lane == 0) { red[(2 * k) * W + wid] = mn; red[(2 * k + 1) * W + wid] = mx; }
+        };
+        wave_fold(on_a, ta, 0);
+        wave_fold(on_b, tb, 1);
+        wave_fold(on_o, to, 2);
+        __syncthreads();
+        auto slot_fold = [&](bool on, int k, float* slots) {
+            if (!on || (int)threadIdx.x != k) return;
+            float mn = red[(2 * k) * W], mx = red[(2 * k + 1) * W];
+            for (int w = 1; w < W; w++) { mn = fminf(mn, red[(2 * k) * W + w]); mx = fmaxf(mx, red[(2 * k + 1) * W + w]); }
+            slots[2 * g] = fminf(mn, slots[2 * g]);
+            slots[2 * g + 1] = fmaxf(mx, slots[2 * g + 1]);
+        };
+        slot_fold(on_a, 0, p.slots[0]);
+        slot_fold(on_b, 1, p.slots[1]);
+        slot_fold(on_o, 2, p.slots[2]);
+    }
+}
+
+int es_grid(uint32_t tiles, bool hist) {
+    uint32_t g = tiles / (hist ? kEsMinTilesHist : kEsMinTilesMinMax);
+    uint32_t cap = (uint32_t)(num_cu() * (hist ? kEsWgPerCu : kEsWgPerCuMinMax));
+    const uint32_t acc = (uint32_t)(hist ? ppqhip_hist_rows() : ppqhip_minmax_slots());
+    if (cap > acc) cap = acc;
+    if (g > cap) g = cap;
+    if (g < 1) g = 1;
+    return (int)g;
+}
+
+template <bool HIST, bool ASYM, bool CLIP>
+void launch_es(const EsArgs& p, bool resid, bool bias_b, bool plane, int grid, size_t lds, hipStream_t st) {
+#define PPQ_LAUNCH_ES(R, BB, PL)                                                                                       \
+    hipLaunchKernelGGL((epilogue_stats_kernel<HIST, R, BB, PL, ASYM, CLIP>), dim3(grid), dim3(kEsBlock), lds, st, p)
+    switch ((resid ? 4 : 0) | (bias_b ? 2 : 0) | (plane ? 1 : 0)) {
+        case 0: PPQ_LAUNCH_ES(false, false, false); break;
+        case 1: PPQ_LAUNCH_ES(false, false, true); break;
+        case 4: PPQ_LAUNCH_ES(true, false, false); break;
+        case 5: PPQ_LAUNCH_ES(true, false, true); break;
+        case 6: PPQ_LAUNCH_ES(true, true, false); break;
+        default: PPQ_LAUNCH_ES(true, true, true); break;
+    }
+#undef PPQ_LAUNCH_ES
+}
+
+int run_es(EsArgs p, int64_t n, int64_t C, int64_t epc, int relu, int store_a, int store_b, bool hist, int asym, int clip,
+           int64_t num_bins, hipStream_t st, const char* what) {
+    if (int s = validate_epilogue(n, C, epc, what)) return s;
+    const bool resid = p.b != nullptr;
+    if (!p.a || !p.bias_a || (resid && !p.out)) { set_error("%s: null pointer", what); return PPQHIP_ERR_INVALID_VALUE; }
+    if (!p.bias_b && (p.slots[1] || p.rows[1])) {
+        set_error("%s: a statistic of b needs bias_b (the launch does not write b otherwise)", what);
+        return PPQHIP_ERR_INVALID_VALUE;
+    }
+    const bool aligned = aligned16(p.a) && (!resid || (aligned16(p.b) && aligned16(p.out)));
+    if (!aligned || n < 4) { set_error("%s: operands are not 16-B aligned (or n < 4)", what); return PPQHIP_ERR_UNSUPPORTED; }
+    int nh = 0;
+    if (hist) {
+        if (num_bins <= 0 || num_bins > kEsMaxBins) {
+            set_error("%s: 1..%d bins (LDS holds up to %d histograms of a launch)", what, kEsMaxBins, kEsMaxHist);
+            return PPQHIP_ERR_UNSUPPORTED;
+        }
+        for (int k = 0; k < kEsMaxHist; k++) nh += p.rows[k] != nullptr;
+    }
+    p.relu = relu ? 1 : 0; p.store_a = store_a ? 1 : 0; p.store_b = store_b ? 1 : 0;
+    p.bins = (int)num_bins;
+    p.nc = make_fastdiv((uint32_t)C);
+    p.nvec = (uint32_t)(n >> 2);
+    p.tail = p.nvec * 4u;
+    p.ntail = (int)(n & 3);
+    const bool plane = (epc % 4 == 0);
+    p.epc = make_fastdiv((uint32_t)(plane ? epc / 4 : epc));
+    const uint32_t tiles = (p.nvec + kEsTileVec - 1) / kEsTileVec;
+    const int grid = es_grid(tiles, hist);
+    const bool bias_b = p.bias_b != nullptr;
+    if (!hist) launch_es<false, false, false>(p, resid, bias_b, plane, grid, sizeof(float) * 2 * kEsMaxHist * (kEsBlock / kWave), st);
+    else {
+        const size_t lds = sizeof(int) * (size_t)(nh > 0 ? nh : 1) * (size_t)num_bins;
+        switch ((asym ? 2 : 0) | (clip ? 1 : 0)) {
+            case 0: launch_es<true, false, false>(p, resid, bias_b, plane, grid, lds, st); break;
+            case 1: launch_es<true, false, true>(p, resid, bias_b, plane, grid, lds, st); break;
+            case 2: launch_es<true, true, false>(p, resid, bias_b, plane, grid, lds, st); break;
+            default: launch_es<true, true, true>(p, resid, bias_b, plane, grid, lds, st); break;
+        }
+    }
+    return finish_launch(what);
+}
+
+void set_rule(EsArgs& p, int k, int32_t* rows, float p0, float p1, int asym, int64_t bins) {
+    p.rows[k] = rows;
+    if (asym) { p.ra[k] = p0; p.hs[k] = (p1 - p0) / (float)bins; }
+    else { p.ra[k] = 0.f; p.hs[k] = p0; }
+}
+
+}
+}
+
+using namespace ppqhip;
+
+extern "C" {
+
+int64_t ppqhip_epilogue_hist_max_bins(void) { return (int64_t)kEsMaxBins; }
+
+int ppqhip_bias_act_minmax(float* y, const float* bias, int64_t n, int64_t num_channel, int64_t elem_per_channel, int relu,
+                           float* slots, void* stream) {
+    EsArgs p{};
+    p.a = y; p.bias_a = bias; p.slots[0] = slots;
+    return run_es(p, n, num_channel, elem_per_channel, relu, 1, 1, false, 0, 0, 0, (hipStream_t)stream, "bias_act_minmax");
+}
+
+int ppqhip_bias_add_act_minmax(float* a, const float* bias_a, float* b, const float* bias_b, float* out, int64_t n,
+                               int64_t num_channel, int64_t elem_per_channel, int relu, int store_a, int store_b,
+                               float* slots_a, float* slots_b, float* slots_out, void* stream) {
+    if (!b) { set_error("bias_add_act_minmax: null pointer"); return PPQHIP_ERR_INVALID_VALUE; }
+    EsArgs p{};
+    p.a = a; p.bias_a = bias_a; p.b = b; p.bias_b = bias_b; p.out = out;
+    p.slots[0] = slots_a; p.slots[1] = slots_b; p.slots[2] = slots_out;
+    return run_es(p, n, num_channel, elem_per_channel, relu, store_a, store_b, false, 0, 0, 0, (hipStream_t)stream,
+                  "bias_add_act_minmax");
+}
+
+int ppqhip_bias_act_hist(float* y, const float* bias, int64_t n, int64_t num_channel, int64_t elem_per_channel, int relu,
+                         int32_t* rows, float p0, float p1, int asymmetric, int clip_outliers, int64_t num_bins, void* stream) {
+    EsArgs p{};
+    p.a = y; p.bias_a = bias;
+    set_rule(p, 0, rows, p0, p1, asymmetric, num_bins);
+    return run_es(p, n, num_channel, elem_per_channel, relu, 1, 1, true, asymmetric, clip_outliers, num_bins,
+                  (hipStream_t)stream, "bias_act_hist");
+}
+
+int ppqhip_bias_add_act_hist(float* a, const float* bias_a, float* b, const float* bias_b, float* out, int64_t n,
+                             int64_t num_channel, int64_t elem_per_channel, int relu, int store_a, int store_b,
+                             int32_t* rows_a, float p0_a, float p1_a, int32_t* rows_b, float p0_b, float p1_b,
+                             int32_t* rows_out, float p0_out, float p1_out, int asymmetric, int clip_outliers,
+                             int64_t num_bins, void* stream) {
+    if (!b) { set_error("bias_add_act_hist: null pointer"); return PPQHIP_ERR_INVALID_VALUE; }
+    EsArgs p{};
+    p.a = a; p.bias_a = bias_a; p.b = b; p.bias_b = bias_b; p.out = out;
+    set_rule(p, 0, rows_a, p0_a, p1_a, asymmetric, num_bins);
+    set_rule(p, 1, rows_b, p0_b, p1_b, asymmetric, num_bins);
+    set_rule(p, 2, rows_out, p0_out, p1_out, asymmetric, num_bins);
+    return run_es(p, n, num_channel, elem_per_channel, relu, store_a, store_b, true, asymmetric, clip_outliers, num_bins,
+                  (hipStream_t)stream, "bias_add_act_hist");
+}
+
+}
diff --git a/ppq_amd/csrc/hist.hip b/ppq_amd/csrc/hist.hip
--- a/ppq_amd/csrc/hist.hip
+++ b/ppq_amd/csrc/hist.hip
@@ -1,4 +1,4 @@
-#include "common.hpp"
+#include "binner.hpp"
 
 namespace ppqhip {
 
@@ -15,8 +15,6 @@
 constexpr uint32_t kTileElems = kTileVec * 4;
 static_assert(kHistBlock % 64 == 0 && kHistBlock >= 64 && kHistBlock <= 1024, "histogram workgroup: whole waves");
 
-typedef float v2f __attribute__((ext_vector_type(2)));
-
 struct BinRule {
     float a;
     float hs;
@@ -29,63 +27,6 @@
     BinRule r; r.a = a; r.hs = hs; r.rcp = 1.0f / hs; r.bins = bins; r.clip = clip; r.asym = asym;
     return r;
 }
-
-__device__ __forceinline__ bool quotient_is_safe(float t) {
-    return __builtin_fabsf(t - __builtin_rintf(t)) >= __builtin_fabsf(t) * 0x1p-22f;
-}
-
-__device__ __forceinline__ int f2i_abs(float t) {
-    int r;
-    asm("v_cvt_i32_f32_e64 %0, |%1|" : "=v"(r) : "v"(t));
-    return r;
-}
-__device__ __forceinline__ int f2i_floor(float t) {
-    int r;
-    asm("v_cvt_flr_i32_f32 %0, %1" : "=v"(r) : "v"(t));
-    return r;
-}
-
-template <bool ASYM, bool CLIP, bool HOT>
-struct Binner : WaveBinCounter<ASYM, CLIP, HOT> {
-    using Base = WaveBinCounter<ASYM, CLIP, HOT>;
-    using Base::h; using Base::last; using Base::hot_bin; using Base::hot_cnt;
-    float a0, hs, rcp;
-
-    __device__ __forceinline__ void set_rule(float a, float scale) { a0 = a; hs = scale; rcp = 1.0f / scale; }
-
-    __device__ __forceinline__ void bins4(const float4& v, int (&b)[4]) const {
-        v2f x01 = {v.x, v.y}, x23 = {v.z, v.w};
-        if (ASYM) { x01 = x01 - a0; x23 = x23 - a0; }
-        const v2f t01 = x01 * rcp, t23 = x23 * rcp;
-        const v2f r01 = {__builtin_rintf(t01.x), __builtin_rintf(t01.y)};
-        const v2f r23 = {__builtin_rintf(t23.x), __builtin_rintf(t23.y)};
-        const v2f d01 = t01 - r01, d23 = t23 - r23;
-        const v2f e01 = t01 * 0x1p-22f, e23 = t23 * 0x1p-22f;
-        const bool u0 = !(__builtin_fabsf(d01.x) >= __builtin_fabsf(e01.x));
-        const bool u1 = !(__builtin_fabsf(d01.y) >= __builtin_fabsf(e01.y));
-        const bool u2 = !(__builtin_fabsf(d23.x) >= __builtin_fabsf(e23.x));
-        const bool u3 = !(__builtin_fabsf(d23.y) >= __builtin_fabsf(e23.y));
-        b[0] = ASYM ? f2i_floor(t01.x) : f2i_abs(t01.x);
-        b[1] = ASYM ? f2i_floor(t01.y) : f2i_abs(t01.y);
-        b[2] = ASYM ? f2i_floor(t23.x) : f2i_abs(t23.x);
-        b[3] = ASYM ? f2i_floor(t23.y) : f2i_abs(t23.y);
-        if (u0 | u1 | u2 | u3) {
-            if (u0) b[0] = exact_bin(ASYM ? x01.x : __builtin_fabsf(v.x));
-            if (u1) b[1] = exact_bin(ASYM ? x01.y : __builtin_fabsf(v.y));
-            if (u2) b[2] = exact_bin(ASYM ? x23.x : __builtin_fabsf(v.z));
-            if (u3) b[3] = exact_bin(ASYM ? x23.y : __builtin_fabsf(v.w));
-        }
-    }
-    __device__ __forceinline__ int exact_bin(float a) const { return f2i_sat(__builtin_floorf(a / hs)); }
-
-    __device__ __forceinline__ int bin1(float v) const {
-        const float a = ASYM ? (v - a0) : __builtin_fabsf(v);
-        const float t = a * rcp;
-        if (quotient_is_safe(t)) return ASYM ? f2i_floor(t) : f2i_abs(t);
-        return exact_bin(a);
-    }
-
-};
 
 constexpr int kReduceBins = 32, kReduceSlices = 32, kReduceBlock = kReduceBins * kReduceSlices;
 __global__ __launch_bounds__(kReduceBlock) void hist_reduce_kernel(const int* __restrict__ partial, int count, int bins,
diff --git a/ppq_amd/ffi.py b/ppq_amd/ffi.py
--- a/ppq_amd/ffi.py
+++ b/ppq_amd/ffi.py
@@ -183,6 +183,68 @@
         _raise(lib.ppqhip_bias_add_act(a.data_ptr(), bias_a.data_ptr(), b.data_ptr(), 0 if bias_b is None else bias_b.data_ptr(),
                                        out.data_ptr(), a.numel(), geo[0], geo[1], 1 if relu else 0, _stream()))
     return out
+
+
+_UNSUPPORTED = -2
+
+
+def epilogue_hist_max_bins() -> int:
+    return int(lib.ppqhip_epilogue_hist_max_bins())
+
+
+def _stat_slots(slots, dev):
+    if slots is None: return 0
+    if (not isinstance(slots, torch.Tensor) or slots.dtype is not _F32 or slots.device != dev or not slots.is_contiguous()
+            or slots.numel() != 2 * lib.ppqhip_minmax_slots()):
+        raise RuntimeError(_KERNEL_FAILURE + 'slots must be a contiguous float32 [minmax_slots(), 2] tensor on the operands\' device')
+    return slots.data_ptr()
+
+
+def _stat_rows(target, dev, bins):
+    if target is None: return 0, 0.0, 0.0
+    rows, p0, p1 = target
+    if (not isinstance(rows, torch.Tensor) or rows.dtype is not torch.int32 or rows.device != dev or not rows.is_contiguous()
+            or rows.ndim != 2 or rows.shape[0] != lib.ppqhip_hist_rows() or rows.shape[1] != bins):
+        raise RuntimeError(_KERNEL_FAILURE + f'rows must be a contiguous int32 [hist_rows(), {bins}] tensor on the operands\' device')
+    return rows.data_ptr(), float(p0), float(p1)
+
+
+def _launched(status: int) -> bool:
+    if status == _UNSUPPORTED: return False
+    _raise(status)
+    return True
+
+
+def bias_act_stats_(y: torch.Tensor, bias: torch.Tensor, relu: bool, kind: str, target, bins: int = 0,
+                    asymmetric: bool = False, clip_outliers: bool = True) -> bool:
+    geo = _epilogue_geometry([y], [bias])
+    if geo is None: return False
+    with _DeviceOf(y):
+        if kind == 'minmax':
+            return _launched(lib.ppqhip_bias_act_minmax(y.data_ptr(), bias.data_ptr(), y.numel(), geo[0], geo[1], 1 if relu else 0,
+                                                        _stat_slots(target, y.device), _stream()))
+        rows, p0, p1 = _stat_rows(target, y.device, bins)
+        return _launched(lib.ppqhip_bias_act_hist(y.data_ptr(), bias.data_ptr(), y.numel(), geo[0], geo[1], 1 if relu else 0, rows,
+                                                  p0, p1, int(bool(asymmetric)), int(bool(clip_outliers)), int(bins), _stream()))
+
+
+def bias_add_act_stats(a: torch.Tensor, bias_a: torch.Tensor, b: torch.Tensor, bias_b, relu: bool, kind: str, targets,
+                       bins: int = 0, asymmetric: bool = False, clip_outliers: bool = True, store_a: bool = True,
+                       store_b: bool = True, out: torch.Tensor = None):
+    geo = _epilogue_geometry([a, b], [bias_a] if bias_b is None else [bias_a, bias_b])
+    if geo is None or a.data_ptr() == b.data_ptr(): return None
+    if out is None: out = torch.empty_like(a)
+    dev = a.device
+    head = (a.data_ptr(), bias_a.data_ptr(), b.data_ptr(), 0 if bias_b is None else bias_b.data_ptr(), out.data_ptr(), a.numel(),
+            geo[0], geo[1], 1 if relu else 0, int(bool(store_a)), int(bool(store_b)))
+    with _DeviceOf(a):
+        if kind == 'minmax':
+            ok = _launched(lib.ppqhip_bias_add_act_minmax(*head, *[_stat_slots(t, dev) for t in targets], _stream()))
+        else:
+            flat = [x for t in targets for x in _stat_rows(t, dev, bins)]
+            ok = _launched(lib.ppqhip_bias_add_act_hist(*head, *flat, int(bool(asymmetric)), int(bool(clip_outliers)), int(bins),
+                                                        _stream()))
+    return out if ok else None
 
 
 _ADAROUND_JOB = np.dtype([('w', '<u8'), ('v', '<u8'), ('scale', '<u8'), ('offset', '<u8'), ('out', '<u8'), ('dy', '<u8'),
diff --git a/ppq_amd/harness.py b/ppq_amd/harness.py
--- a/ppq_amd/harness.py
+++ b/ppq_amd/harness.py
@@ -251,6 +251,7 @@
         self._delegates: Dict[object, Callable] = {}
         self.fuse_epilogues = True
         self._epilogue_cache: Dict[tuple, dict] = {}
+        self.epilogue_stat_launches = 0
         self.channels_last = False
         for v in graph.variables.values():
             if v.is_parameter and v.value is not None: v.value = v.value.to(device)
@@ -386,8 +387,39 @@
             self._epilogue_cache[sig] = plan
         return plan
 
+    @ staticmethod
+    def _epilogue_observers(grp: EpilogueGroup, hooks) -> Optional[dict]:
+        from .observer import fused_statistic
+        if not hooks: return None
+        if grp.kind == 'P1': key_of = {grp.convs[0].name: 'a', grp.relu.name: 'a'}
+        else:
+            key_of = {grp.convs[0].name: 'a', grp.add.name: 'out', grp.relu.name: 'out'}
+            if len(grp.convs) > 1: key_of[grp.convs[1].name] = 'b'
+        seen, written = [], {}
+        for op in grp.ops:
+            hook = hooks.get(op.name)
+            table = hook._observer_table if hook is not None and isinstance(op, QuantableOperation) else None
+            if table:
+                if hook.stream is not None: return None
+                if op.type != 'Conv':
+                    seen += [(written.get(v.name), table[c]) for v, c in zip(op.inputs, op.config.input_quantization_config)
+                             if c in table]
+                seen += [(key_of[op.name], table[c]) for c in op.config.output_quantization_config if c in table]
+            for v in op.outputs: written[v.name] = key_of[op.name]
+        observers, kinds = {}, set()
+        for key, ob in seen:
+            if key is None: continue
+            kind = fused_statistic(ob)
+            if kind is None or key in observers: return None
+            observers[key] = ob
+            kinds.add((kind, ob._hist_bins if kind == 'hist' else 0,
+                       kind == 'hist' and ob._quant_cfg.policy.has_property(P.ASYMMETRICAL)))
+        if not observers or len(kinds) != 1: return None
+        kind, bins, asym = next(iter(kinds))
+        return {'kind': kind, 'bins': bins, 'asymmetric': bool(asym), 'observers': observers}
+
     def _run_epilogue(self, grp: EpilogueGroup, raw_of: Callable, hooks) -> Optional[Dict[str, torch.Tensor]]:
-        from .ffi import bias_act_, bias_add_act
+        from .ffi import bias_act_, bias_add_act, bias_act_stats_, bias_add_act_stats
         for conv in grp.convs:
             x, w = raw_of(conv.inputs[0]), conv.inputs[1].value
             if not (isinstance(x, torch.Tensor) and x.is_cuda and x.dtype == torch.float32 and x.dim() == 4
@@ -415,10 +447,19 @@
                                      groups=a.get('group', 1))
             biases[conv.name] = qin[2]
             qins[conv.name] = qin
+        fused = self._epilogue_observers(grp, hooks)
+        stat = {}
+        if fused is not None:
+            dev = next(iter(ys.values())).device
+            stat = dict(kind=fused['kind'], bins=fused['bins'], asymmetric=fused['asymmetric'])
+            targets = {k: ob.fused_target(dev) for k, ob in fused['observers'].items()}
         if grp.kind == 'P1':
             conv = grp.convs[0]
             y = ys[conv.name]
-            if not bias_act_(y, biases[conv.name], relu=True):
+            if fused is not None and bias_act_stats_(y, biases[conv.name], True, target=targets['a'], **stat):
+                fused['observers']['a'].fused_taken(y)
+                self.epilogue_stat_launches += 1
+            elif not bias_act_(y, biases[conv.name], relu=True):
                 y.add_(biases[conv.name].view(1, -1, 1, 1)).relu_()
             tail = {conv.name: y, grp.relu.name: y}
         else:
@@ -426,13 +467,29 @@
             a = ys[conv_a.name]
             conv_b = grp.convs[1] if len(grp.convs) > 1 else None
             b = ys[conv_b.name] if conv_b is not None else raw_of(grp.add.inputs[1])
-            out = bias_add_act(a, biases[conv_a.name], b, biases[conv_b.name] if conv_b is not None else None, relu=True)
+            out = None
+            if fused is not None:
+                out = bias_add_act_stats(a, biases[conv_a.name], b, biases[conv_b.name] if conv_b is not None else None, True,
+                                         targets=[targets.get(k) for k in ('a', 'b', 'out')], **stat)
+                if out is not None:
+                    for k, t in (('a', a), ('b', b), ('out', out)):
+                        if k in fused['observers']: fused['observers'][k].fused_taken(t)
+                    self.epilogue_stat_launches += 1
+            if out is None:
+                out = bias_add_act(a, biases[conv_a.name], b, biases[conv_b.name] if conv_b is not None else None, relu=True)
             if out is None:
                 a.add_(biases[conv_a.name].view(1, -1, 1, 1))
                 if conv_b is not None: b.add_(biases[conv_b.name].view(1, -1, 1, 1))
                 out = F.relu(a + b)
             tail = {conv_a.name: a, grp.add.name: out, grp.relu.name: out}
             if conv_b is not None: tail[conv_b.name] = b
+        try:
+            return self._epilogue_hooks(grp, raw_of, hooks, tail)
+        finally:
+            if fused is not None:
+                for ob in fused['observers'].values(): ob.fused_release()
+
+    def _epilogue_hooks(self, grp: EpilogueGroup, raw_of: Callable, hooks, tail) -> Dict[str, torch.Tensor]:
         values: Dict[str, torch.Tensor] = {}
         for op in grp.ops:
             hook = hooks.get(op.name)
diff --git a/ppq_amd/observer.py b/ppq_amd/observer.py
--- a/ppq_amd/observer.py
+++ b/ppq_amd/observer.py
@@ -104,6 +104,7 @@
         self._max = max_pending_bytes
         self.launches = 0
         self.recorder: Optional[list] = None
+        self.fuse_epilogue_stats = False
 
     def __len__(self):
         return (len(self._minmax) + len(self._minmax_c) + sum(len(v) for v in self._hist.values())
@@ -233,6 +234,20 @@
         pass
 
 
+def fused_statistic(ob) -> Optional[str]:
+    if type(ob) not in (TorchMinMaxObserver, TorchHistObserver, TorchMSEObserver): return None
+    q = ob.queue
+    if q is None or not q.fuse_epilogue_stats or q.recorder is not None: return None
+    cfg = ob._quant_cfg
+    if not is_initial(cfg) or not cfg.policy.has_property(P.PER_TENSOR): return None
+    if type(ob) is TorchMinMaxObserver: return 'minmax'
+    if ob._phase == 'Detecting Minmax': return 'minmax'
+    if ob._phase != 'Collating Hist': return None
+    if not (cfg.policy.has_property(P.ASYMMETRICAL) or cfg.policy.has_property(P.SYMMETRICAL)): return None
+    if ob._hist_bins > 16384 or (ob._hist is not None and ob._rows is None): return None
+    return 'hist'
+
+
 _RANGE_SEEDS: Dict[object, tuple] = {}
 
 
@@ -253,12 +268,35 @@
         self._queued_c = False
         self._host_range: Optional[np.ndarray] = None
         self._observed = False
+        self._fused: Optional[torch.Tensor] = None
+
+    def fused_target(self, device):
+        if self._range is None:
+            seed = _range_seed(device)
+            self._range = seed[0].clone()
+            self._slots = seed[1].clone()
+        return self._slots
+
+    def fused_taken(self, value: torch.Tensor) -> None:
+        self._fused = value
+        self._slots_dirty = True
+        self._observed = True
+        self._host_range = None
+
+    def fused_release(self) -> None:
+        self._fused = None
+
+    def _swallow_fused(self, value) -> bool:
+        if self._fused is None: return False
+        fused, self._fused = self._fused, None
+        return fused is value
 
     @ torch.no_grad()
     def observe(self, value: torch.Tensor):
         assert isinstance(value, torch.Tensor), 'TorchMinMaxObserver can only deal with torch Tensor values'
         assert value.numel() > 0, (f'You are observing an empty tensor({getattr(self._watch_on, "name", "")}).')
         if not is_initial(self._quant_cfg): return
+        if self._swallow_fused(value): return
         cfg = self._quant_cfg
         if cfg.policy.has_property(P.PER_TENSOR):
             if self._range is None:
@@ -353,6 +391,25 @@
         self._hist_bins = hist_bins
         super().__init__(watch_on, quant_cfg)
 
+    def _alloc_hist(self, device) -> None:
+        if self._hist is None:
+            self._hist = torch.zeros(size=(self._hist_bins,), dtype=torch.int32, device=device)
+            if self._hist_bins <= 16384:
+                self._rows = torch.zeros(size=(CUDA.hist_rows(), self._hist_bins), dtype=torch.int32, device=device)
+
+    def fused_target(self, device):
+        if self._phase == 'Detecting Minmax': return super().fused_target(device)
+        self._alloc_hist(device)
+        if self._quant_cfg.policy.has_property(P.ASYMMETRICAL): return self._rows, self._min, self._max
+        return self._rows, self._hist_scale, 0.0
+
+    def fused_taken(self, value: torch.Tensor) -> None:
+        if self._phase == 'Detecting Minmax': return super().fused_taken(value)
+        self._fused = value
+        self._losses = None
+        if getattr(self, '_best', None) is not None: self._best = None
+        self._rows_dirty = True
+
     def observe(self, value: torch.Tensor):
         if not is_initial(self._quant_cfg): return
         assert value.numel() > 0, (f'You are observing an empty tensor({getattr(self._watch_on, "name", "")}).')
@@ -361,13 +418,10 @@
                 self.queue.recorder.append((self, value))
             return super().observe(value)
         elif self._phase == 'Collating Hist':
+            if self._swallow_fused(value): return
             self._losses = None
             if getattr(self, '_best', None) is not None: self._best = None
-            if self._hist is None:
-                self._hist = torch.zeros(size=(self._hist_bins,), dtype=torch.int32, device=value.device)
-                if self._hist_bins <= 16384:
-                    self._rows = torch.zeros(size=(CUDA.hist_rows(), self._hist_bins), dtype=torch.int32,
-                                             device=value.device)
+            self._alloc_hist(value.device)
             if self._quant_cfg.policy.has_property(P.ASYMMETRICAL):
                 if self._rows is not None:
                     if self.queue is not None: self.queue.add_hist(value, self._rows, True, self._min, self._max)
```

Result: faster. 3608 samples/s (median of 6 runs) (+2.3%).
